# amazon-science/instruct-video-to-video

Hardware: AMD Instinct MI355X
Metric: denoised video-frames/sec (16f@256x384, 50 DDIM steps) (higher is better)
Workload: dtype fp16; 1 GPU; C2: 1 clip/step = VAE-encode + 50 DDIM steps (3-way CFG, text 7.5 / video 1.5) + VAE-decode, 16 frames @ 256x384, random-init full-width UNet+VAE; 5 independent clips in flight per GPU (stacked into every UNet launch, B = 3 x clips); frames=16, height=256, width=384, ddim_steps=50, clips_per_gpu=5, parallelism=clip-parallel x1, one all_gather, hip_graph=True, cfg_branch_streams=False, concurrent_clips=5, clip_mode=stacked, driver_mode=False, full=False

## Files before the change

### include/insv2v_hip.h

```cpp
#ifndef INSV2V_HIP_H
#define INSV2V_HIP_H

#include <stdint.h>

#ifdef __cplusplus
extern "C" {
#endif

typedef void* insv2v_stream_t;

#define INSV2V_OK 0
#define INSV2V_EINVAL (-1)
#define INSV2V_EUNSUPPORTED (-2)

#define INSV2V_ACT_NONE 0
#define INSV2V_ACT_SILU 1
#define INSV2V_ACT_GEGLU 2
#define INSV2V_ACT_QUICK_GELU 3

#define INSV2V_ACT_RELU 4
#define INSV2V_ACT_SIGMOID 5
#define INSV2V_ACT_TANH 6

#define INSV2V_MODE_LINEAR 0
#define INSV2V_MODE_CONV3X3 1

int insv2v_abi_version(void);
int insv2v_init(void);

typedef struct insv2v_gemm_desc {
    const void* a;
    const void* a2;
    const void* w;
    void* c;
    const float* bias;
    const float* row_bias;
    const void* residual;
    const float* row_stats;
    const float* col_sum;
    int64_t lda, lda2, ldw, ldc, ldr, ld_rb;
    int64_t a_bs, w_bs, c_bs, r_bs;
    void* workspace;
    int64_t workspace_bytes;
    int32_t M, N, K;
    int32_t k_split;
    int32_t rows_per_group;
    int32_t rb_mod;
    int32_t act;
    int32_t c_fp32;
    int32_t mode;
    int32_t NB, IH, IW, OH, OW, Cin;
    int32_t stride, pad_t, pad_l, upsample;
    int32_t batch;
    int32_t tile;
    int32_t split_k;
    float alpha;
    const float* gn_ab;
    int32_t gn_images_per_sample;
    int32_t gn_silu;
    float* stats_out;
    float* stats_scratch;
    int32_t stats_parts;
    float ln_eps;
    int64_t w_group_stride;
    int32_t w_group_rows;
    int32_t reserved0;
} insv2v_gemm_desc;
int insv2v_gemm(const insv2v_gemm_desc* d, insv2v_stream_t stream);
int64_t insv2v_set_operand_window(int64_t bytes);
int insv2v_gemm_stats_parts(const insv2v_gemm_desc* d);
int insv2v_conv3x3_fuses_groupnorm(const insv2v_gemm_desc* d);
#define INSV2V_PLAN_NONE 0
#define INSV2V_PLAN_TILE 1
#define INSV2V_PLAN_HALO 2
#define INSV2V_PLAN_Q8 3
#define INSV2V_PLAN_R8 4
#define INSV2V_PLAN_W4 5
typedef struct insv2v_gemm_plan_t {
    int32_t rc;
    int32_t family;
    int32_t variant;
    int32_t ring;
    int32_t tw_shift;
    int32_t cim;
    int32_t split_k;
    int32_t ln_finalize;
    int32_t splitk_reduce;
    int32_t stats_width;
    int32_t gn_fuse;
    int32_t parts;
    int32_t units_per_part;
    int32_t forced_tile;
} insv2v_gemm_plan_t;
int insv2v_gemm_plan(const insv2v_gemm_desc* d, int cus, insv2v_gemm_plan_t* out);

typedef struct insv2v_winograd_in_desc {
    const void* x;
    const void* x2;
    const float* gn_ab;
    void* v;
    int64_t ldx, ldx2;
    int64_t v_group_rows;
    int32_t NB, H, W, C, C1;
    int32_t gn_images_per_sample;
    int32_t gn_silu;
    int32_t upsample;
} insv2v_winograd_in_desc;
int insv2v_winograd_input(const insv2v_winograd_in_desc* d, insv2v_stream_t stream);
typedef struct insv2v_winograd_out_desc {
    const void* m;
    const float* bias;
    const float* row_bias;
    const void* residual;
    void* y;
    int64_t m_group_rows;
    int64_t ldr, ldy, ld_rb;
    int32_t NB, H, W, Cout;
    int32_t rows_per_group;
    int32_t upsample;
} insv2v_winograd_out_desc;
int insv2v_winograd_output(const insv2v_winograd_out_desc* d, insv2v_stream_t stream);

typedef struct insv2v_ffn_desc {
    const void* x;
    void* out;
    const void* wstream;
    int64_t ldx, ldo;
    int32_t M, C, hidden;
    float eps;
    const void* post_residual;
    int64_t ld_post;
    int32_t post;
} insv2v_ffn_desc;
int insv2v_ffn_fused(const insv2v_ffn_desc* d, insv2v_stream_t stream);
int64_t insv2v_ffn_stream_elems(int32_t C, int32_t hidden, int32_t post);

typedef struct insv2v_rowlin_desc {
    const void* x;
    void* out;
    const void* residual;
    const void* wstream;
    int64_t ldx, ldo, ldr;
    int32_t M, N, K;
    int32_t layernorm, frame_bias, rows_per_frame, frames;
    float eps;
    float* stats_out;
    float stats_eps;
    const float* gn_ab;
    int32_t gn_rows;
} insv2v_rowlin_desc;
int insv2v_rowlin(const insv2v_rowlin_desc* d, insv2v_stream_t stream);
int64_t insv2v_rowlin_stream_elems(int32_t N, int32_t K);

typedef struct insv2v_tattn_desc {
    const void* x;
    void* out;
    const void* wstream;
    int64_t ldx, ldo;
    int32_t samples, HW, C, heads, frames;
    float eps;
    float scale;
} insv2v_tattn_desc;
int insv2v_tattn_fused(const insv2v_tattn_desc* d, insv2v_stream_t stream);
int64_t insv2v_tattn_stream_elems(int32_t C, int32_t heads, int32_t frames);
int insv2v_tattn_attn(const insv2v_tattn_desc* d, insv2v_stream_t stream);
int64_t insv2v_tattn_attn_stream_elems(int32_t C, int32_t heads, int32_t frames);

typedef struct insv2v_xattn_desc {
    const void* x;
    void* out;
    const void* wstream;
    const void* kvstream;
    int64_t ldx, ldo;
    int32_t M, rows_per_sample, C, heads, ctx_len;
    float eps;
    float scale;
    const void* pre_residual;
    int64_t ld_pre;
} insv2v_xattn_desc;
int insv2v_xattn_fused(const insv2v_xattn_desc* d, insv2v_stream_t stream);
int64_t insv2v_xattn_stream_elems(int32_t C, int32_t heads, int32_t per_sample_kv);
int insv2v_xattn_attn(const insv2v_xattn_desc* d, insv2v_stream_t stream);
int64_t insv2v_xattn_attn_stream_elems(int32_t C, int32_t heads, int32_t per_sample_kv);

typedef struct insv2v_groupnorm_desc {
    const void* x;
    const void* x2;
    void* y;
    const float* gamma;
    const float* beta;
    float* partials;
    int64_t ldx, ldx2, ldy;
    int32_t nsamples, rows_per_sample, C, C1, G;
    int32_t nchunks;
    int32_t silu;
    float eps;
    float* ab;
    int32_t stats_only;
} insv2v_groupnorm_desc;
int insv2v_groupnorm(const insv2v_groupnorm_desc* d, insv2v_stream_t stream);

typedef struct insv2v_layernorm_desc {
    const void* x;
    void* y;
    const float* gamma;
    const float* beta;
    const float* pe;
    int64_t ldx, ldy;
    int32_t rows, C;
    int32_t rows_per_frame, frames, pe_start;
    float eps;
} insv2v_layernorm_desc;
int insv2v_layernorm(const insv2v_layernorm_desc* d, insv2v_stream_t stream);
int insv2v_layernorm_stats(const void* x, float* stats, int64_t ldx, int32_t rows, int32_t C, float eps,
                           insv2v_stream_t stream);

typedef struct insv2v_attention_desc {
    const void* q;
    const void* k;
    const void* v;
    void* o;
    int64_t q_rs, k_rs, v_rs, o_rs;
    int64_t q_outer, q_step, kv_outer, kv_step, o_outer, o_step;
    int32_t q_inner, kv_inner, o_inner;
    int32_t batch, heads, head_dim, seq_q, seq_k;
    float scale;
    int32_t causal;
    const void* q_bias;
    const void* k_bias;
    const void* v_bias;
    int64_t bias_rs;
} insv2v_attention_desc;
int insv2v_attention(const insv2v_attention_desc* d, insv2v_stream_t stream);

int insv2v_embed_tokens(const int64_t* ids, const void* tok, const void* pos, void* out, int32_t rows, int32_t L,
                        int32_t C, int32_t vocab, insv2v_stream_t stream);

int insv2v_softmax_rows(const void* x, void* y, int64_t ldx, int64_t ldy, int32_t rows, int32_t cols,
                        float scale, insv2v_stream_t stream);
int insv2v_softmax_rows_padded(const void* x, void* y, int64_t ldx, int64_t ldy, int32_t rows, int32_t cols, int32_t valid,
                               float scale, insv2v_stream_t stream);

int insv2v_timestep_embedding(const float* t, void* out, int32_t batch, int32_t dim, float shift,
                              insv2v_stream_t stream);

int insv2v_tap_gather(const float* y9, int64_t ld9, const float* bias, float* out, int64_t ldo, int32_t NB, int32_t H, int32_t W,
                      int32_t cout, insv2v_stream_t stream);

int insv2v_build_unet_input(const float* latent, const float* img_cond, void* out, float* t_out,
                            float timestep, int32_t nbranch, int32_t F, int32_t h, int32_t w, int32_t ldo,
                            int64_t branch_rows, int32_t t_stride, insv2v_stream_t stream);

typedef struct insv2v_step_desc {
    const float* eps_in;
    const float* latent;
    const float* latent_ref;
    const float* delta_q;
    const float* noise;
    const float* rescale_stats;
    float* latent_out;
    float* pred_x0;
    float* eps_out;
    int32_t nbranch, F, h, w, R;
    int32_t correct;
    float text_cfg, img_cfg;
    float sqrt_a, sqrt_1ma;
    float c_x0, c_eps, c_xt, c_noise;
    float guidance_rescale;
    int64_t branch_stride;
    int64_t noise_seed, noise_stream;
    int32_t noise_on;
} insv2v_step_desc;
int insv2v_cfg_step(const insv2v_step_desc* d, insv2v_stream_t stream);
typedef struct insv2v_mstep_desc {
    const float* eps_in;
    const float* latent;
    const float* latent_ref;
    const float* delta_q;
    const float* noise;
    const float* rescale_stats;
    float* latent_out;
    float* pred_x0;
    float* eps_out;
    int32_t nbranch, F, h, w, R;
    int32_t correct;
    float text_cfg, img_cfg;
    float sqrt_a, sqrt_1ma;
    float c_x0, c_eps, c_xt, c_noise;
    float guidance_rescale;
    int64_t branch_stride;
    int64_t noise_seed, noise_stream;
    int32_t noise_on;
    const float* x0_hist;
    float c_hist;
} insv2v_mstep_desc;
int insv2v_cfg_step_ms(const insv2v_mstep_desc* d, insv2v_stream_t stream);
typedef struct insv2v_maskstep_desc {
    const float* eps_in;
    const float* latent;
    const float* latent_ref;
    const float* delta_q;
    const float* noise;
    const float* rescale_stats;
    float* latent_out;
    float* pred_x0;
    float* eps_out;
    int32_t nbranch, F, h, w, R;
    int32_t correct;
    float text_cfg, img_cfg;
    float sqrt_a, sqrt_1ma;
    float c_x0, c_eps, c_xt, c_noise;
    float guidance_rescale;
    int64_t branch_stride;
    int64_t noise_seed, noise_stream;
    int32_t noise_on;
    const float* x0_hist;
    float c_hist;
    const float* mask;
    const float* src;
    const float* known_noise;
    float k_src, k_noise;
} insv2v_maskstep_desc;
int insv2v_cfg_step_mask(const insv2v_maskstep_desc* d, insv2v_stream_t stream);
int insv2v_mask_to_latent(const float* mask, float* out, int32_t N, int32_t H, int32_t W, int32_t mode, insv2v_stream_t stream);
int insv2v_composite(const float* edited, const float* original, const float* mask, float* out, int32_t N, int32_t H, int32_t W,
                     insv2v_stream_t stream);
int insv2v_add_noise(const float* z, const float* noise, float* out, int64_t n, float ka, float kb, insv2v_stream_t stream);
int insv2v_cfg_stats(const float* eps_in, float* stats, int32_t F, int32_t h, int32_t w, float text_cfg,
                     float img_cfg, int64_t branch_stride, insv2v_stream_t stream);

int insv2v_warp_image(const float* image, const float* flow, float* out, int32_t N, int32_t C, int32_t H,
                      int32_t W, insv2v_stream_t stream);
int insv2v_resize_flow(const float* flow, float* out, int32_t N, int32_t h, int32_t w, int32_t H, int32_t W,
                       insv2v_stream_t stream);
int insv2v_flow_correction(const float* eps_cfg, const float* latent, const float* latent_ref,
                           const float* flows, float* delta_q, int32_t F, int32_t R, int32_t h, int32_t w,
                           float sqrt_a, float sqrt_1ma, insv2v_stream_t stream);

int insv2v_nchw_to_nhwc_f16(const float* x, void* y, int32_t N, int32_t C, int32_t H, int32_t W, int32_t ldo,
                            float scale, insv2v_stream_t stream);
int insv2v_nhwc_to_nchw_f32(const void* x, int32_t x_is_fp32, float* y, int32_t N, int32_t C, int32_t H,
                            int32_t W, int32_t ldx, float scale, insv2v_stream_t stream);
int insv2v_posterior_sample(const float* moments, const float* noise, float* z, int32_t N, int32_t H,
                            int32_t W, int32_t ldm, float scale, insv2v_stream_t stream);
int insv2v_posterior_sample_seeded(const float* moments, float* z, int32_t N, int32_t H, int32_t W, int32_t ldm, float scale,
                                   int64_t seed, int64_t stream, int64_t offset, insv2v_stream_t hip_stream);

int insv2v_randn(float* out, int64_t n, int64_t seed, int64_t stream, int64_t offset, int32_t raw, insv2v_stream_t hip_stream);

typedef struct insv2v_im2col_desc {
    const void* x;
    const void* x2;
    void* out;
    int64_t ldx, ldx2, ldo;
    int32_t N, IH, IW, C, C1, KH, KW, stride_h, stride_w, pad_h, pad_w, OH, OW;
} insv2v_im2col_desc;
int insv2v_im2col(const insv2v_im2col_desc* d, insv2v_stream_t stream);
int insv2v_instance_norm(const void* x, void* y, float* partials, int32_t N, int32_t HW, int32_t C, int64_t ldx, int64_t ldy,
                         int32_t nchunks, float eps, int32_t relu, insv2v_stream_t stream);
#define INSV2V_EW_RELU 1
#define INSV2V_EW_ADD_RELU 2
#define INSV2V_EW_TANH 3
#define INSV2V_EW_GRU_RH 4
#define INSV2V_EW_GRU_OUT 5
int insv2v_ew(int32_t op, const void* a, const void* b, const void* c, void* out, int64_t rows, int32_t C, int64_t lda, int64_t ldb,
              int64_t ldc, int64_t ldo, insv2v_stream_t stream);
int insv2v_avgpool2x2(const float* x, float* y, int64_t n, int32_t h, int32_t w, insv2v_stream_t stream);
typedef struct insv2v_corr_lookup_desc {
    const float* pyr0;
    const float* pyr1;
    const float* pyr2;
    const float* pyr3;
    const float* coords;
    void* out;
    int64_t ldo;
    int32_t B, h, w, levels, radius;
} insv2v_corr_lookup_desc;
int insv2v_corr_lookup(const insv2v_corr_lookup_desc* d, insv2v_stream_t stream);
int insv2v_raft_flow_rows(float* coords1, const float* delta, int64_t ldd, void* rows, int64_t ldf, int32_t ncols, int32_t B, int32_t h,
                          int32_t w, insv2v_stream_t stream);
int insv2v_convex_upsample(const float* coords1, const void* mask, int64_t ldm, float* out, int32_t B, int32_t h, int32_t w,
                           insv2v_stream_t stream);

#ifdef __cplusplus
}
#endif
#endif
```

### instruct-video-to-video_amd/csrc/gemm.hip

```cpp
#include "common.h"
#include <algorithm>
#include "gemm_dma.h"
#include "gemm_plan.h"
static_assert(GEMM_BK == BK, "gemm_plan.h restates the K slice");
#include <type_traits>
#include <cstdlib>

typedef unsigned uint4r __attribute__((ext_vector_type(4)));

struct RowInfo {
    int base;
    int oh, ow;
    bool valid;
};

#ifdef INSV2V_GEMM_PROF
__device__ unsigned long long g_prof[8];
#define PROF_MARK(i) do { if (tid == 0) prof_t[i] = wall_clock64(); } while (0)
#else
#define PROF_MARK(i) do { } while (0)
#endif

template <int W>
__device__ __forceinline__ float lane_group_sum(float v) {
    static_assert(W == 4 || W == 8 || W == 16, "a DPP row is 16 lanes");
    auto dpp = [](float x, auto ctrl) {
        return __builtin_bit_cast(float, __builtin_amdgcn_update_dpp(0, __builtin_bit_cast(int, x), decltype(ctrl)::value, 0xF, 0xF, true));
    };
    v += dpp(v, std::integral_constant<int, 0xB1>{});
    v += dpp(v, std::integral_constant<int, 0x4E>{});
    if (W >= 8) v += dpp(v, std::integral_constant<int, 0x141>{});
    if (W >= 16) v += dpp(v, std::integral_constant<int, 0x140>{});
    return v;
}

__device__ __forceinline__ bool fast_output_ok(const insv2v_gemm_desc& p, const char* Cb, const half_t* Rp, int oN) {
    const bool vec_ok = ((p.ldc & 7) == 0) && (((uintptr_t)Cb & (p.c_fp32 ? 31 : 15)) == 0) &&
                        (!Rp || (((p.ldr & 7) == 0) && (((uintptr_t)Rp & 15) == 0)));
    const bool res32 = !Rp || (int64_t)p.M * p.ldr * 2 < ((int64_t)1 << 31);
    return vec_ok && !p.c_fp32 && (oN & 7) == 0 && res32;
}

template <int WM, int WN, int MI, int NI, int KG, bool HAS_LN, class RowMap>
__device__ __forceinline__ void tile_epilogue(const insv2v_gemm_desc& p, floatx16 (&acc)[NI][MI], char* smem, const float* sBias,
                                              const float* sCs, const float2* sStat, int tid, int wm, int wn, int kg, int bn0,
                                              int z, int zs, bool rows_full, RowMap grow
#ifdef INSV2V_GEMM_PROF
                                              , unsigned long long* prof_t
#endif
) {
    constexpr int NWV = WM * WN * KG, NT = NWV * 64;
    constexpr int BM = WM * MI * 32, BN = WN * NI * 32;
    const int lane = tid & 63;
    const bool geglu = p.act == INSV2V_ACT_GEGLU;
    const int oN = geglu ? (p.N >> 1) : p.N;
    const int on0 = geglu ? (bn0 >> 1) : bn0;
    constexpr int CLD = BN + 4;
    float* sC = (float*)smem;
    char* Cb = (char*)p.c + ((int64_t)z * p.c_bs + (int64_t)zs * p.M * p.ldc) * (p.c_fp32 ? 4 : 2);
    const half_t* Rp = p.residual ? (const half_t*)p.residual + z * p.r_bs : nullptr;
    if (KG > 1) {
        for (int g = 1; g < KG; ++g) {
            if (kg == g) {
#pragma unroll
                for (int j = 0; j < MI; ++j)
#pragma unroll
                    for (int i = 0; i < NI; ++i)
#pragma unroll
                        for (int q = 0; q < 4; ++q)
                            *(float4*)(sC + (wm * MI * 32 + j * 32 + (lane & 31)) * CLD + wn * NI * 32 + i * 32 + 8 * q + 4 * (lane >> 5)) =
                                make_float4(acc[i][j][4 * q], acc[i][j][4 * q + 1], acc[i][j][4 * q + 2], acc[i][j][4 * q + 3]);
            }
            __syncthreads();
            if (kg == 0) {
#pragma unroll
                for (int j = 0; j < MI; ++j)
#pragma unroll
                    for (int i = 0; i < NI; ++i)
#pragma unroll
                        for (int q = 0; q < 4; ++q) {
                            const float4 t = *(const float4*)(sC + (wm * MI * 32 + j * 32 + (lane & 31)) * CLD + wn * NI * 32 + i * 32 + 8 * q + 4 * (lane >> 5));
                            acc[i][j][4 * q] += t.x; acc[i][j][4 * q + 1] += t.y; acc[i][j][4 * q + 2] += t.z; acc[i][j][4 * q + 3] += t.w;
                        }
            }
            if (g + 1 < KG) __syncthreads();
        }
    }
    typedef unsigned uint4e __attribute__((ext_vector_type(4)));
    const srd_t rRB = make_srd(p.row_bias ? (const void*)p.row_bias : (const void*)p.w);
    const bool rb_vec = p.row_bias && (p.N & 3) == 0 && (p.ld_rb & 3) == 0 && (((uintptr_t)p.row_bias & 15) == 0);
    if (KG == 1 || kg == 0) {
#pragma unroll
    for (int j = 0; j < MI; ++j) {
        const int ml = wm * MI * 32 + j * 32 + (lane & 31);
        const int m = grow(ml);
        const float* rb = nullptr;
        unsigned rb_off = OOB_OFFSET;
        if (p.row_bias && m < p.M) {
            int grp = m / p.rows_per_group;
            if (p.rb_mod > 0) grp %= p.rb_mod;
            rb = p.row_bias + (int64_t)grp * p.ld_rb;
            rb_off = (unsigned)(grp * (int)p.ld_rb * 4);
        }
        floatx4 rbv[NI][4];
        if (rb_vec) {
#pragma unroll
            for (int i = 0; i < NI; ++i)
#pragma unroll
                for (int q = 0; q < 4; ++q) {
                    const int n = bn0 + wn * NI * 32 + i * 32 + 8 * q + 4 * (lane >> 5);
                    rbv[i][q] = __builtin_bit_cast(floatx4, (uint4e)__builtin_amdgcn_raw_buffer_load_b128(rRB, (rb && n + 3 < p.N) ? rb_off + (unsigned)(n * 4) : OOB_OFFSET, 0, 0));
                }
        }
        float ln_m = 0.f, ln_r = 1.f;
        if (HAS_LN) { const float2 st = sStat[ml]; ln_m = st.x; ln_r = st.y; }
#pragma unroll
        for (int i = 0; i < NI; ++i) {
            if (geglu && (i & 1)) continue;
#pragma unroll
            for (int q = 0; q < 4; ++q) {
                const int nl = wn * NI * 32 + i * 32 + 8 * q + 4 * (lane >> 5);
                const int n = bn0 + nl;
                float v[4];
                const float4 bt = *(const float4*)(sBias + nl), ct = HAS_LN ? *(const float4*)(sCs + nl) : make_float4(0.f, 0.f, 0.f, 0.f);
                float bsum[4] = {bt.x, bt.y, bt.z, bt.w};
                const float cs[4] = {ct.x, ct.y, ct.z, ct.w};
                if (rb_vec) {
                    const floatx4 t = rbv[i][q];
                    bsum[0] += t[0]; bsum[1] += t[1]; bsum[2] += t[2]; bsum[3] += t[3];
                } else if (rb) {
#pragma unroll
                    for (int e = 0; e < 4; ++e)
                        if (n + e < p.N) bsum[e] += rb[n + e];
                }
#pragma unroll
                for (int e = 0; e < 4; ++e) v[e] = ln_r * (acc[i][j][4 * q + e] * p.alpha - ln_m * cs[e]) + bsum[e];
                int onl = nl;
                if (geglu) {
                    const float4 gbt = *(const float4*)(sBias + nl + 32), gct = HAS_LN ? *(const float4*)(sCs + nl + 32) : make_float4(0.f, 0.f, 0.f, 0.f);
                    float gb[4] = {gbt.x, gbt.y, gbt.z, gbt.w};
                    const float gcs[4] = {gct.x, gct.y, gct.z, gct.w};
                    if (rb_vec) {
                        const floatx4 t = rbv[(i + 1) % NI][q];
                        gb[0] += t[0]; gb[1] += t[1]; gb[2] += t[2]; gb[3] += t[3];
                    } else if (rb && n + 35 < p.N) {
                        const float4 t = *(const float4*)(rb + n + 32);
                        gb[0] += t.x; gb[1] += t.y; gb[2] += t.z; gb[3] += t.w;
                    }
#pragma unroll
                    for (int e = 0; e < 4; ++e)
                        v[e] *= gelu_erf_f(ln_r * (acc[(i + 1) % NI][j][4 * q + e] * p.alpha - ln_m * gcs[e]) + gb[e]);
                    onl = (nl >> 6) * 32 + (nl & 31);
                } else if (p.act == INSV2V_ACT_SILU) {
#pragma unroll
                    for (int e = 0; e < 4; ++e) v[e] = silu_f(v[e]);
                } else if (p.act == INSV2V_ACT_QUICK_GELU) {
#pragma unroll
                    for (int e = 0; e < 4; ++e) v[e] = quick_gelu_f(v[e]);
                } else if (p.act >= INSV2V_ACT_RELU) {
#pragma unroll
                    for (int e = 0; e < 4; ++e) v[e] = act_raft_f(v[e], p.act);
                }
                *(float4*)(sC + ml * CLD + onl) = make_float4(v[0], v[1], v[2], v[3]);
            }
        }
    }
    }
    PROF_MARK(3);
    __syncthreads();
    PROF_MARK(4);
    const int OW8 = (geglu ? BN / 2 : BN) / 8;
    const bool vec_ok = ((p.ldc & 7) == 0) && (((uintptr_t)Cb & (p.c_fp32 ? 31 : 15)) == 0) &&
                        (!Rp || (((p.ldr & 7) == 0) && (((uintptr_t)Rp & 15) == 0)));
    if (fast_output_ok(p, Cb, Rp, oN)) {
        const srd_t rRes = make_srd(Rp ? (const void*)Rp : (const void*)p.w);
        auto copy_rows = [&](auto w8_tag) {
            constexpr int W8 = decltype(w8_tag)::value;
            constexpr int ITERS = (BM * W8) / NT;
            static_assert((BM * W8) % NT == 0, "staged tile must divide evenly over the workgroup");
            half8 rv[ITERS];
            bool ok[ITERS];
            int mrow[ITERS];
#pragma unroll
            for (int it = 0; it < ITERS; ++it) {
                const int idx = tid + it * NT, row = idx / W8, ch = idx % W8;
                mrow[it] = grow(row);
                ok[it] = (rows_full || mrow[it] < p.M) && on0 + ch * 8 + 8 <= oN;
                if (Rp) rv[it] = __builtin_bit_cast(half8, (uint4e)__builtin_amdgcn_raw_buffer_load_b128(
                            rRes, ok[it] ? (unsigned)((mrow[it] * (int)p.ldr + on0 + ch * 8) * 2) : OOB_OFFSET, 0, 0));
            }
#pragma unroll
            for (int it = 0; it < ITERS; ++it) {
                const int idx = tid + it * NT, row = idx / W8, ch = idx % W8;
                const float4 f0 = *(const float4*)(sC + row * CLD + ch * 8);
                const float4 f1 = *(const float4*)(sC + row * CLD + ch * 8 + 4);
                const float fv[8] = {f0.x, f0.y, f0.z, f0.w, f1.x, f1.y, f1.z, f1.w};
                half8 hv;
#pragma unroll
                for (int e = 0; e < 8; ++e) hv[e] = (half_t)(Rp ? fv[e] + (float)rv[it][e] : fv[e]);
                if (ok[it]) *(half8*)((half_t*)Cb + (int64_t)mrow[it] * p.ldc + on0 + ch * 8) = hv;
                if constexpr (W8 == 4 || W8 == 8 || W8 == 16) {
                    if (p.stats_out) {
                        float s1 = 0.f, s2 = 0.f;
#pragma unroll
                        for (int e = 0; e < 8; ++e) { const float x = ok[it] ? (float)hv[e] : 0.f; s1 += x; s2 = fmaf(x, x, s2); }
                        s1 = lane_group_sum<W8>(s1);
                        s2 = lane_group_sum<W8>(s2);
                        if (ch == 0 && (rows_full || mrow[it] < p.M))
                            *(float2*)(p.stats_out + ((int64_t)(bn0 / BN) * p.M + mrow[it]) * 2) = make_float2(s1, s2);
                    }
                }
            }
        };
        if (geglu) copy_rows(std::integral_constant<int, BN / 16>{});
        else copy_rows(std::integral_constant<int, BN / 8>{});
#ifdef INSV2V_GEMM_PROF
        wait_vmcnt<0>();
        PROF_MARK(5);
        if (tid == 0) {
            for (int i = 0; i < 5; ++i) atomicAdd(&g_prof[i], prof_t[i + 1] - prof_t[i]);
            atomicAdd(&g_prof[5], 1ull);
        }
#endif
        return;
    }
    for (int idx = tid; idx < BM * OW8; idx += NT) {
        const int row = idx / OW8, ch = idx - row * OW8;
        const int m = grow(row), on = on0 + ch * 8;
        if (m >= p.M || on >= oN) continue;
        const float4 f0 = *(const float4*)(sC + row * CLD + ch * 8);
        const float4 f1 = *(const float4*)(sC + row * CLD + ch * 8 + 4);
        float fv[8] = {f0.x, f0.y, f0.z, f0.w, f1.x, f1.y, f1.z, f1.w};
        if (p.c_fp32) {
            float* dst32 = (float*)Cb + (int64_t)m * p.ldc + on;
            if (Rp) {
#pragma unroll
                for (int e = 0; e < 8; ++e)
                    if (on + e < oN) fv[e] += (float)Rp[(int64_t)m * p.ldr + on + e];
            }
            if (vec_ok && on + 7 < oN) {
                *(float4*)dst32 = make_float4(fv[0], fv[1], fv[2], fv[3]);
                *(float4*)(dst32 + 4) = make_float4(fv[4], fv[5], fv[6], fv[7]);
            } else {
#pragma unroll
                for (int e = 0; e < 8; ++e)
                    if (on + e < oN) dst32[e] = fv[e];
            }
            continue;
        }
        half_t* dst = (half_t*)Cb + (int64_t)m * p.ldc + on;
        if (vec_ok && on + 7 < oN) {
            half8 hv;
            if (Rp) {
                const half8 rv = *(const half8*)(Rp + (int64_t)m * p.ldr + on);
#pragma unroll
                for (int e = 0; e < 8; ++e) hv[e] = (half_t)(fv[e] + (float)rv[e]);
            } else {
#pragma unroll
                for (int e = 0; e < 8; ++e) hv[e] = (half_t)fv[e];
            }
            *(half8*)dst = hv;
        } else {
#pragma unroll
            for (int e = 0; e < 8; ++e)
                if (on + e < oN) dst[e] = (half_t)(fv[e] + (Rp ? (float)Rp[(int64_t)m * p.ldr + on + e] : 0.f));
        }
    }
}

template <int WM, int WN, int MI, int NI, int MODE, int STAGES, int KG = 1>
__global__ __launch_bounds__(WM * WN * KG * 64) void gemm_kernel(insv2v_gemm_desc p) {
    constexpr int NWV = WM * WN * KG;
    constexpr int BM = WM * MI * 32, BN = WN * NI * 32;
    constexpr int LD = BK;
    constexpr int RPP = 8 * NWV;
    constexpr int RA = BM / RPP, RW = BN / RPP;
    extern __shared__ __attribute__((aligned(16))) char smem[];
    half_t* sA = (half_t*)smem;
    half_t* sW = sA + STAGES * BM * LD;
    constexpr int RING_B = STAGES * (BM + BN) * BK * 2, STAGE_B = BM * (BN + 4) * 4;
    float* sBias = (float*)(smem + (RING_B > STAGE_B ? RING_B : STAGE_B));
    float* sCs = sBias + BN;
    float2* sStat = (float2*)(sCs + BN);

    const int tid = threadIdx.x, lane = tid & 63;
#ifdef INSV2V_GEMM_PROF
    unsigned long long prof_t[6];
#endif
    PROF_MARK(0);
    const int wid = __builtin_amdgcn_readfirstlane(tid >> 6);
    const int kg = wid / (WM * WN), wl = wid % (WM * WN);
    const int wm = wl / WN, wn = wl % WN;
    const int tiles_n = (p.N + BN - 1) / BN, tiles_m = (p.M + BM - 1) / BM;
    const int bid = xcd_remap(blockIdx.x, tiles_m * tiles_n);
    constexpr int GROUP_M = 8;
    const int per_group = GROUP_M * tiles_n;
    const int gidx = bid / per_group, first_m = gidx * GROUP_M;
    const int gsz = min(GROUP_M, tiles_m - first_m), rin = bid - gidx * per_group;
    const int tn = rin / gsz, tm = first_m + rin - tn * gsz;
    const int bm0 = tm * BM, bn0 = tn * BN;
    const int z = blockIdx.y;

    const half_t* A = (const half_t*)p.a + z * p.a_bs;
    const half_t* A2 = p.a2 ? (const half_t*)p.a2 + z * p.a_bs : A;
    const half_t* Wp = (const half_t*)p.w + z * p.w_bs;
    const srd_t rA = make_srd(A), rA2 = make_srd(A2), rW = make_srd(Wp);

    const int crow = wid * 8 + (lane >> 3);
    const int cslot = lane & 7;

    RowInfo ri[RA];
    int achunk[RA];
    unsigned aoff1[RA], aoff2[RA];
#pragma unroll
    for (int i = 0; i < RA; ++i) {
        const int row = crow + RPP * i;
        achunk[i] = cslot ^ ((row >> 1) & 7);
        const int m = bm0 + row;
        ri[i].valid = m < p.M;
        if (MODE == INSV2V_MODE_LINEAR) {
            ri[i].base = m;
            ri[i].oh = ri[i].ow = 0;
            aoff1[i] = ri[i].valid ? (unsigned)(((int64_t)m * p.lda + achunk[i] * 8) * 2) : OOB_OFFSET;
            aoff2[i] = ri[i].valid ? (unsigned)(((int64_t)m * p.lda2 + achunk[i] * 8) * 2) : OOB_OFFSET;
        } else {
            int mm = ri[i].valid ? m : 0;
            int ow = mm % p.OW, t = mm / p.OW;
            int oh = t % p.OH, nb = t / p.OH;
            ri[i].base = nb * p.IH * p.IW;
            ri[i].oh = oh * p.stride - p.pad_t;
            ri[i].ow = ow * p.stride - p.pad_l;
            const int64_t pix = (int64_t)ri[i].base + (int64_t)ri[i].oh * p.IW + ri[i].ow;
            aoff1[i] = (unsigned)((pix * p.lda + achunk[i] * 8) * 2);
            aoff2[i] = (unsigned)((pix * p.lda2 + achunk[i] * 8) * 2);
        }
    }
    int wchunk[RW];
    unsigned woff[RW];
#pragma unroll
    for (int i = 0; i < RW; ++i) {
        const int row = crow + RPP * i;
        wchunk[i] = cslot ^ ((row >> 1) & 7);
        const int n = bn0 + row;
        woff[i] = n < p.N ? (unsigned)(((int64_t)n * p.ldw + wchunk[i] * 8) * 2) : OOB_OFFSET;
    }

    const int nk_total = (p.K + BK - 1) / BK;
    const int zs = blockIdx.z, nsplit = p.split_k > 1 ? p.split_k : 1;

    const int nk_per = (nk_total + nsplit - 1) / nsplit;
    const int kt0 = zs * nk_per;
    const int nk = max(0, min(nk_per, nk_total - kt0));
    const int IHu = p.upsample ? p.OH : p.IH, IWu = p.upsample ? p.OW : p.IW;

    struct Cursor {
        int k0, kh, kw, ci0;
    } cur_k = {kt0 * BK, 0, 0, 0};
    if (MODE != INSV2V_MODE_LINEAR) {
        const int tap = cur_k.k0 / p.Cin;
        cur_k.ci0 = cur_k.k0 - tap * p.Cin;
        cur_k.kh = tap / 3;
        cur_k.kw = tap - cur_k.kh * 3;
    }
    auto advance = [&]() {
        cur_k.k0 += BK;
        if (MODE != INSV2V_MODE_LINEAR) {
            cur_k.ci0 += BK;
            if (cur_k.ci0 >= p.Cin) {
                cur_k.ci0 = 0;
                if (++cur_k.kw == 3) { cur_k.kw = 0; ++cur_k.kh; }
            }
        }
    };
    auto issue_slice = [&](int buf) {
        char* a = (char*)(sA + buf * BM * LD) + wid * 1024;
        char* w = (char*)(sW + buf * BN * LD) + wid * 1024;
        const bool ktail = cur_k.k0 + BK > p.K;
        if (MODE == INSV2V_MODE_LINEAR) {
            const bool second = p.k_split > 0 && cur_k.k0 >= p.k_split;
            const int soff = (second ? cur_k.k0 - p.k_split : cur_k.k0) * 2;
#pragma unroll
            for (int i = 0; i < RA; ++i) {
                unsigned v = second ? aoff2[i] : aoff1[i];
                if (ktail && cur_k.k0 + achunk[i] * 8 >= p.K) v = OOB_OFFSET;
                dma16(second ? rA2 : rA, v, soff, a + i * (NWV * 1024));
            }
        } else {
            const bool second = p.k_split > 0 && cur_k.ci0 >= p.k_split;
            const int ld = (int)(second ? p.lda2 : p.lda);
            const int cl = second ? cur_k.ci0 - p.k_split : cur_k.ci0;
            const int tapoff = ((cur_k.kh * p.IW + cur_k.kw) * ld + cl) * 2;
#pragma unroll
            for (int i = 0; i < RA; ++i) {
                const int ih = ri[i].oh + cur_k.kh, iw = ri[i].ow + cur_k.kw;
                const bool ok = ri[i].valid && (unsigned)ih < (unsigned)IHu && (unsigned)iw < (unsigned)IWu;
                unsigned v;
                if (p.upsample)
                    v = (unsigned)((((ri[i].base + (ih >> 1) * p.IW + (iw >> 1)) * ld) + cl + achunk[i] * 8) * 2);
                else
                    v = (second ? aoff2[i] : aoff1[i]) + (unsigned)tapoff;
                dma16(second ? rA2 : rA, ok ? v : OOB_OFFSET, 0, a + i * (NWV * 1024));
            }
        }
        const int wsoff = cur_k.k0 * 2;
#pragma unroll
        for (int i = 0; i < RW; ++i) {
            unsigned v = woff[i];
            if (ktail && cur_k.k0 + wchunk[i] * 8 >= p.K) v = OOB_OFFSET;
            dma16(rW, v, wsoff, w + i * (NWV * 1024));
        }
        advance();
    };

    floatx16 acc[NI][MI];
#pragma unroll
    for (int i = 0; i < NI; ++i)
#pragma unroll
        for (int j = 0; j < MI; ++j)
#pragma unroll
            for (int r = 0; r < 16; ++r) acc[i][j][r] = 0.f;

    const int frow = lane & 31, fhalf = lane >> 5;
    auto compute = [&](int buf) {
        const half_t* a = sA + buf * BM * LD + (wm * MI * 32 + frow) * LD;
        const half_t* w = sW + buf * BN * LD + (wn * NI * 32 + frow) * LD;
        const int sw = (frow >> 1) & 7;
#pragma unroll
        for (int kq = 0; kq < BK / 16 / KG; ++kq) {
            const int kk = kg * (BK / 16 / KG) + kq;
            const int c = ((kk * 2 + fhalf) ^ sw) * 8;
            half8 fa[MI], fw[NI];
#pragma unroll
            for (int j = 0; j < MI; ++j) fa[j] = *(const half8*)(a + j * 32 * LD + c);
#pragma unroll
            for (int i = 0; i < NI; ++i) fw[i] = *(const half8*)(w + i * 32 * LD + c);
#pragma unroll
            for (int i = 0; i < NI; ++i)
#pragma unroll
                for (int j = 0; j < MI; ++j)
                    acc[i][j] = __builtin_amdgcn_mfma_f32_32x32x16_f16(fw[i], fa[j], acc[i][j], 0, 0, 0);
        }
    };

    const bool ln = p.row_stats != nullptr;
    float pre_b = 0.f, pre_c = 0.f;
    float2 pre_s = make_float2(0.f, 1.f);
    if (tid < BN && bn0 + tid < p.N) {
        if (p.bias) pre_b = p.bias[bn0 + tid];
        if (ln) pre_c = p.col_sum[bn0 + tid];
    }
    if (tid < BM && ln && bm0 + tid < p.M) {
        if (p.stats_parts > 0) {
            float s1 = 0.f, s2 = 0.f;
            for (int j = 0; j < p.stats_parts; ++j) {
                const float2 t = ((const float2*)p.row_stats)[(int64_t)j * p.M + bm0 + tid];
                s1 += t.x; s2 += t.y;
            }
            const float mean = s1 / p.K;
            pre_s = make_float2(mean, rsqrtf(fmaxf(s2 / p.K - mean * mean, 0.f) + p.ln_eps));
        } else {
            pre_s = ((const float2*)p.row_stats)[bm0 + tid];
        }
    }

    constexpr int LPT = RA + RW;
#pragma unroll
    for (int s = 0; s < STAGES; ++s)
        if (s < nk) issue_slice(s);
    if (tid < BN) { sBias[tid] = pre_b; sCs[tid] = pre_c; }
    if (tid < BM) sStat[tid] = pre_s;
    int cur = 0, nxt = STAGES - 1;
    for (int kt = 0; kt < nk; ++kt) {
        const int behind = kt == 0 ? min(STAGES - 1, nk - 1) : min(STAGES - 2, nk - 1 - kt);
        if (behind <= 0) wait_vmcnt<0>();
        else if (behind == 1) wait_vmcnt<LPT>();
        else if (behind == 2) wait_vmcnt<2 * LPT>();
        else wait_vmcnt<3 * LPT>();
        __builtin_amdgcn_s_barrier();
        asm volatile("" ::: "memory");
#ifdef INSV2V_GEMM_PROF
        if (kt == 0) PROF_MARK(1);
#endif
        if (kt > 0 && kt + STAGES - 1 < nk) issue_slice(nxt);
        compute(cur);
        cur = (cur + 1 == STAGES) ? 0 : cur + 1;
        nxt = (nxt + 1 == STAGES) ? 0 : nxt + 1;
    }
    wait_vmcnt<0>();
    __syncthreads();
    PROF_MARK(2);

    tile_epilogue<WM, WN, MI, NI, KG, true>(p, acc, smem, sBias, sCs, sStat, tid, wm, wn, kg, bn0, z, zs, bm0 + BM <= p.M,
                                            [&](int r) { return bm0 + r; }
#ifdef INSV2V_GEMM_PROF
                                            , prof_t
#endif
    );
}


template <int WM, int WN, int MI, int NI, int KG, bool GN, int WS = 2>
__global__ __launch_bounds__(WM * WN * KG * 64) void conv_halo_kernel(insv2v_gemm_desc p, int tw_shift) {
    constexpr int NWV = WM * WN * KG;
    constexpr int BM = WM * MI * 32, BN = WN * NI * 32;
    static_assert(BM == 128 || BM == 256, "the pixel patch is 128 (8x16 / 16x8) or 256 (16x16 / 32x8) output pixels");
    static_assert(WS == 2 || (WS == 3 && !GN && KG == 1), "the deep weight ring has no fused-GroupNorm / K-group form");
    constexpr int LD = BK;
    constexpr int RPP = 8 * NWV, RW = BN / RPP;
    constexpr int HPIECES = BM == 128 ? 23 : 43;
    constexpr int HP = (HPIECES + NWV - 1) / NWV;
    constexpr int HALO_B = HPIECES * 1024;
    constexpr int KQ = BK / 16 / KG;
    extern __shared__ __attribute__((aligned(16))) char smem[];
    char* sH = smem;
    half_t* sW = (half_t*)(smem + 2 * HALO_B);
    constexpr int RING_B = 2 * HALO_B + WS * BN * BK * 2, STAGE_B = BM * (BN + 4) * 4;
    float* sBias = (float*)(smem + (RING_B > STAGE_B ? RING_B : STAGE_B));
    constexpr int AB_OFF = (RING_B > STAGE_B ? RING_B : STAGE_B) + BN * 4;

    const int tid = threadIdx.x, lane = tid & 63;
#ifdef INSV2V_GEMM_PROF
    unsigned long long prof_t[6];
#endif
    PROF_MARK(0);
    const int wid = __builtin_amdgcn_readfirstlane(tid >> 6);
    const int kg = wid / (WM * WN), wl = wid % (WM * WN);
    const bool legacy_map = (tw_shift >> 8) & 1;
    tw_shift &= 255;
    const int wm = legacy_map ? wl / WN : wl % WM, wn = legacy_map ? wl % WN : wl / WM;
    const int TW = 1 << tw_shift, TH = BM >> tw_shift;
    const int tiles_x = p.OW >> tw_shift, tiles_y = p.OH / TH, tiles_img = tiles_x * tiles_y;
    const int tiles_n = (p.N + BN - 1) / BN, tiles_m = p.NB * tiles_img;
    const int bid = xcd_remap(blockIdx.x, tiles_m * tiles_n);
    constexpr int GROUP_M = 8;
    const int per_group = GROUP_M * tiles_n;
    const int gidx = bid / per_group, first_m = gidx * GROUP_M;
    const int gsz = min(GROUP_M, tiles_m - first_m), rin = bid - gidx * per_group;
    const int tn = rin / gsz, tm = first_m + rin - tn * gsz;
    const int bn0 = tn * BN;
    const int nb = tm / tiles_img, trem = tm - nb * tiles_img;
    const int ty = trem / tiles_x, tx = trem - ty * tiles_x;
    const int oy0 = ty * TH, ox0 = tx * TW;
    const int up = p.upsample ? 1 : 0;
    const int sy0 = (oy0 - 1) >> up, sx0 = (ox0 - 1) >> up;
    const int PH = (TH >> up) + 2, PW = (TW >> up) + 2, HROWS = PH * PW;

    const half_t* A = (const half_t*)p.a;
    const half_t* A2 = p.a2 ? (const half_t*)p.a2 : A;
    const srd_t rA = make_srd(A), rA2 = make_srd(A2), rW = make_srd(p.w);

    auto patch_key = [&](int hy, int hx) { return ((hx >> 1) + (tw_shift == 3 ? ((hy & 1) << 2) : 0)) & 7; };
    unsigned hoff1[HP], hoff2[HP];
    int hchunk[HP];
#pragma unroll
    for (int i = 0; i < HP; ++i) {
        const int r = (i * NWV + wid) * 8 + (lane >> 3);
        const int hy = r / PW, hx = r - hy * PW;
        const int chunk = (lane & 7) ^ patch_key(hy, hx);
        const int iy = sy0 + hy, ix = sx0 + hx;
        const bool ok = r < HROWS && (unsigned)iy < (unsigned)p.IH && (unsigned)ix < (unsigned)p.IW;
        const int64_t pix = ((int64_t)nb * p.IH + iy) * p.IW + ix;
        hoff1[i] = ok ? (unsigned)((pix * p.lda + chunk * 8) * 2) : OOB_OFFSET;
        hoff2[i] = ok ? (unsigned)((pix * p.lda2 + chunk * 8) * 2) : OOB_OFFSET;
        hchunk[i] = ok ? chunk : -1;
    }
    const int crow = wid * 8 + (lane >> 3), cslot = lane & 7;
    unsigned woff[RW];
#pragma unroll
    for (int i = 0; i < RW; ++i) {
        const int row = crow + RPP * i;
        const int n = bn0 + row;
        woff[i] = n < p.N ? (unsigned)(((int64_t)n * p.ldw + (cslot ^ ((row >> 1) & 7)) * 8) * 2) : OOB_OFFSET;
    }
    const int ncb = p.Cin / BK, nk = ncb * 9;

    auto issue_halo = [&](int i, int cb) {
        const int q = i * NWV + wid;
        if (q >= HPIECES) return;
        const int ci0 = cb * BK;
        const bool second = p.k_split > 0 && ci0 >= p.k_split;
        dma16(second ? rA2 : rA, second ? hoff2[i] : hoff1[i], (second ? ci0 - p.k_split : ci0) * 2, sH + (cb & 1) * HALO_B + q * 1024);
    };
    const unsigned lds0 = (unsigned)(uintptr_t)(__attribute__((address_space(3))) char*)smem;
    const srd_t rAB = make_srd(GN ? (const void*)p.gn_ab : p.w);
    const int gn_sample = GN ? nb / p.gn_images_per_sample : 0;
    auto issue_ab = [&](int cb) {
        if (GN && wid == 0 && lane < 32)
            dma16(rAB, (unsigned)((((int64_t)gn_sample * p.Cin + cb * BK) * 2 + lane * 4) * 4), 0, smem + AB_OFF + (cb & 1) * 512);
    };
    auto normalize = [&](int i, int cb) {
        const int q = i * NWV + wid;
        if (!GN || q >= HPIECES) return;
        const unsigned addr = lds0 + (cb & 1) * HALO_B + q * 1024 + lane * 16;
        const unsigned abaddr = lds0 + AB_OFF + (cb & 1) * 512 + (hchunk[i] < 0 ? 0 : hchunk[i]) * 64;
        uint4r v;
        floatx4 c0, c1, c2, c3;
        asm volatile("ds_read_b128 %0, %5\n\tds_read_b128 %1, %6\n\tds_read_b128 %2, %6 offset:16\n\t"
                     "ds_read_b128 %3, %6 offset:32\n\tds_read_b128 %4, %6 offset:48\n\ts_waitcnt lgkmcnt(0)"
                     : "=&v"(v), "=&v"(c0), "=&v"(c1), "=&v"(c2), "=&v"(c3) : "v"(addr), "v"(abaddr) : "memory");
        const half8 x = __builtin_bit_cast(half8, v);
        const float sc[8] = {c0[0], c0[2], c1[0], c1[2], c2[0], c2[2], c3[0], c3[2]};
        const float sh[8] = {c0[1], c0[3], c1[1], c1[3], c2[1], c2[3], c3[1], c3[3]};
        half8 y;
#pragma unroll
        for (int e = 0; e < 8; ++e) {
            float t = fmaf((float)x[e], sc[e], sh[e]);
            if (p.gn_silu) t = silu_f(t);
            y[e] = hchunk[i] < 0 ? (half_t)0.f : (half_t)t;
        }
        const uint4r o = __builtin_bit_cast(uint4r, y);
        asm volatile("ds_write_b128 %0, %1\n\ts_waitcnt lgkmcnt(0)" ::"v"(addr), "v"(o) : "memory");
    };
    auto issue_w = [&](int buf, int cb, int tap) {
        char* w = (char*)(sW + buf * BN * LD) + wid * 1024;
        const int soff = (tap * p.Cin + cb * BK) * 2;
#pragma unroll
        for (int i = 0; i < RW; ++i) dma16(rW, woff[i], soff, w + i * (NWV * 1024));
    };

    floatx16 acc[NI][MI];
#pragma unroll
    for (int i = 0; i < NI; ++i)
#pragma unroll
        for (int j = 0; j < MI; ++j)
#pragma unroll
            for (int r = 0; r < 16; ++r) acc[i][j][r] = 0.f;

    const int frow = lane & 31, fhalf = lane >> 5;
    int fpy[MI], fpx[MI];
#pragma unroll
    for (int j = 0; j < MI; ++j) {
        const int ml = wm * MI * 32 + j * 32 + frow;
        fpy[j] = ml >> tw_shift;
        fpx[j] = ml & (TW - 1);
    }
    const int wsw = (frow >> 1) & 7;
    const bool wave_live = legacy_map || bn0 + wn * NI * 32 < p.N;
    auto compute = [&](int wbuf, int cb, int kh, int kw) {
        if (!wave_live) return;
        const half_t* hb = (const half_t*)(sH + (cb & 1) * HALO_B);
        const half_t* w = sW + wbuf * BN * LD + (wn * NI * 32 + frow) * LD;
        int arow[MI], akey[MI];
#pragma unroll
        for (int j = 0; j < MI; ++j) {
            const int uy = oy0 + fpy[j] + kh - 1, ux = ox0 + fpx[j] + kw - 1;
            const int hy = (uy >> up) - sy0, hx = (ux >> up) - sx0;
            arow[j] = hy * PW + hx;
            akey[j] = patch_key(hy, hx);
        }
#pragma unroll
        for (int kq = 0; kq < KQ; ++kq) {
            const int kk = kg * KQ + kq;
            const int cl = kk * 2 + fhalf;
            half8 fa[MI], fw[NI];
#pragma unroll
            for (int j = 0; j < MI; ++j) fa[j] = *(const half8*)(hb + arow[j] * LD + ((cl ^ akey[j]) * 8));
#pragma unroll
            for (int i = 0; i < NI; ++i) fw[i] = *(const half8*)(w + i * 32 * LD + ((cl ^ wsw) * 8));
#pragma unroll
            for (int i = 0; i < NI; ++i)
#pragma unroll
                for (int j = 0; j < MI; ++j)
                    acc[i][j] = __builtin_amdgcn_mfma_f32_32x32x16_f16(fw[i], fa[j], acc[i][j], 0, 0, 0);
        }
    };

    float pre_b = 0.f;
    if (tid < BN && bn0 + tid < p.N && p.bias) pre_b = p.bias[bn0 + tid];
    issue_ab(0);
#pragma unroll
    for (int i = 0; i < HP; ++i) issue_halo(i, 0);
    issue_w(0, 0, 0);
    int cbn = 0, tapn = 1;
    if (WS == 3) {
        if (tapn == 9) { tapn = 0; ++cbn; }
        if (nk > 1) issue_w(1, cbn, tapn);
        if (++tapn == 9) { tapn = 0; ++cbn; }
    }
    if (tid < BN) sBias[tid] = pre_b;
    if (GN) {
        wait_vmcnt<0>();
        __builtin_amdgcn_s_barrier();
#pragma unroll
        for (int i = 0; i < HP; ++i) normalize(i, 0);
    }
    int cb = 0, kh = 0, kw = 0, tap = 0;
    int wslot = 0, islot = 2;
    for (int s = 0; s < nk; ++s) {
        if (WS == 3 && s + 1 < nk) wait_vmcnt<RW>();
        else wait_vmcnt<0>();
        __builtin_amdgcn_s_barrier();
        asm volatile("" ::: "memory");
#ifdef INSV2V_GEMM_PROF
        if (s == 0) PROF_MARK(1);
#endif
        if (GN && cb + 1 < ncb) {
#pragma unroll
            for (int i = 0; i < HP; ++i)
                if (tap == i + 1) normalize(i, cb + 1);
        }
        if (WS == 2 && s + 1 < nk) {
            const bool wrap = tap == 8;
            issue_w((s + 1) & 1, wrap ? cb + 1 : cb, wrap ? 0 : tap + 1);
        }
        if (tap == 0 && cb + 1 < ncb) issue_ab(cb + 1);
        if (cb + 1 < ncb) {
#pragma unroll
            for (int i = 0; i < HP; ++i)
                if (tap == i) issue_halo(i, cb + 1);
        }
        if (WS == 3) {
            if (s + 2 < nk) {
                issue_w(islot, cbn, tapn);
                if (++tapn == 9) { tapn = 0; ++cbn; }
            }
            islot = islot == 2 ? 0 : islot + 1;
        }
        compute(WS == 3 ? wslot : (s & 1), cb, kh, kw);
        if (WS == 3) wslot = wslot == 2 ? 0 : wslot + 1;
        if (++kw == 3) { kw = 0; ++kh; }
        if (++tap == 9) { tap = 0; kh = 0; ++cb; }
    }
    wait_vmcnt<0>();
    __syncthreads();
    PROF_MARK(2);
    tile_epilogue<WM, WN, MI, NI, KG, false>(p, acc, smem, sBias, nullptr, nullptr, tid, wm, wn, kg, bn0, 0, 0, true,
                                             [&](int r) { return (nb * p.OH + oy0 + (r >> tw_shift)) * p.OW + ox0 + (r & (TW - 1)); }
#ifdef INSV2V_GEMM_PROF
                                             , prof_t
#endif
    );
}

template <int WM, int WN, int MI, int NI, int KG, bool GN = false, int WS = 2>
static int launch_halo(const insv2v_gemm_desc& d, int tw_shift, hipStream_t s) {
    constexpr int BM = WM * MI * 32, BN = WN * NI * 32;
    constexpr size_t ring = 2 * (BM == 128 ? 23 : 43) * 1024 + WS * (size_t)BN * BK * sizeof(half_t);
    constexpr size_t stage = (size_t)BM * (BN + 4) * sizeof(float);
    constexpr size_t lds = (ring > stage ? ring : stage) + (size_t)BN * sizeof(float) + (GN ? 1024 : 0);
    static bool attr_set = false;
    if (const int e = set_dynamic_lds(attr_set, (const void*)conv_halo_kernel<WM, WN, MI, NI, KG, GN, WS>, lds)) return e;
    const int tiles = d.NB * (d.OH * d.OW / BM) * ((d.N + BN - 1) / BN);
    hipLaunchKernelGGL((conv_halo_kernel<WM, WN, MI, NI, KG, GN, WS>), dim3(tiles), dim3(WM * WN * KG * 64), lds, s, d, tw_shift);
    return launch_status();
}

template <int WM, int WN, int MI, int NI, int MODE, int STAGES, int KG = 1>
static int launch_cfg(const insv2v_gemm_desc& d, hipStream_t s) {
    constexpr int BM = WM * MI * 32, BN = WN * NI * 32;
    constexpr size_t lds = tile_lds_bytes(BM, BN, STAGES);
    if (lds > TILE_LDS_MAX) return INSV2V_EUNSUPPORTED;
    static bool attr_set = false;
    if (const int e = set_dynamic_lds(attr_set, (const void*)gemm_kernel<WM, WN, MI, NI, MODE, STAGES, KG>, lds)) return e;
    int tiles = ((d.M + BM - 1) / BM) * ((d.N + BN - 1) / BN);
    dim3 grid(tiles, d.batch > 0 ? d.batch : 1, d.split_k > 1 ? d.split_k : 1);
    hipLaunchKernelGGL((gemm_kernel<WM, WN, MI, NI, MODE, STAGES, KG>), grid, dim3(WM * WN * KG * 64), lds, s, d);
    return launch_status();
}

template <int MODE, int STAGES>
static int dispatch_tile(const insv2v_gemm_desc& d, int tile, hipStream_t s) {
    switch (tile) {
        case 1: return launch_cfg<2, 2, 2, 2, MODE, STAGES>(d, s);
        case 2: return launch_cfg<2, 2, 1, 2, MODE, STAGES>(d, s);
        case 3: return launch_cfg<2, 2, 2, 1, MODE, STAGES>(d, s);
        case 4: return launch_cfg<2, 2, 1, 1, MODE, STAGES>(d, s);
        case 5: return launch_cfg<4, 2, 1, 2, MODE, STAGES>(d, s);
        case 6: return launch_cfg<4, 2, 2, 2, MODE, STAGES>(d, s);
        case 7: return launch_cfg<4, 2, 1, 1, MODE, STAGES>(d, s);
        case 8: return launch_cfg<2, 2, 2, 2, MODE, STAGES, 2>(d, s);
        case 9: return launch_cfg<2, 2, 2, 1, MODE, STAGES, 2>(d, s);
    }
    return INSV2V_EINVAL;
}

__global__ __launch_bounds__(256) void splitk_reduce_kernel(insv2v_gemm_desc p, const float* ws, int nsplit) {
    const int64_t nchunk = (int64_t)p.M * (p.N / 8);
    const int64_t idx = (int64_t)blockIdx.x * 256 + threadIdx.x;
    if (idx >= nchunk) return;
    const int m = (int)(idx / (p.N / 8)), n = (int)(idx - (int64_t)m * (p.N / 8)) * 8;
    float v[8] = {0.f, 0.f, 0.f, 0.f, 0.f, 0.f, 0.f, 0.f};
    const float* src = ws + (int64_t)m * p.N + n;
    const int64_t slab = (int64_t)p.M * p.N;
    const bool res_vec = p.residual && (p.ldr & 7) == 0 && (((uintptr_t)p.residual & 15) == 0);
    half8 rh = {0, 0, 0, 0, 0, 0, 0, 0};
    if (res_vec) rh = *(const half8*)((const half_t*)p.residual + (int64_t)m * p.ldr + n);
    float4 b0 = make_float4(0.f, 0.f, 0.f, 0.f), b1 = b0, r0 = b0, r1 = b0;
    if (p.bias) {
        if (((uintptr_t)p.bias & 15) == 0) { b0 = *(const float4*)(p.bias + n); b1 = *(const float4*)(p.bias + n + 4); }
        else { b0 = make_float4(p.bias[n], p.bias[n + 1], p.bias[n + 2], p.bias[n + 3]); b1 = make_float4(p.bias[n + 4], p.bias[n + 5], p.bias[n + 6], p.bias[n + 7]); }
    }
    if (p.row_bias) {
        const float* rb = p.row_bias + (int64_t)(m / p.rows_per_group) * p.ld_rb + n;
        if ((p.ld_rb & 3) == 0 && (((uintptr_t)p.row_bias & 15) == 0)) { r0 = *(const float4*)rb; r1 = *(const float4*)(rb + 4); }
        else { r0 = make_float4(rb[0], rb[1], rb[2], rb[3]); r1 = make_float4(rb[4], rb[5], rb[6], rb[7]); }
    }
    int s = 0;
    for (; s + 4 <= nsplit; s += 4) {
        float4 a[4], b[4];
#pragma unroll
        for (int u = 0; u < 4; ++u) { a[u] = *(const float4*)(src + (s + u) * slab); b[u] = *(const float4*)(src + (s + u) * slab + 4); }
#pragma unroll
        for (int u = 0; u < 4; ++u) {
            v[0] += a[u].x; v[1] += a[u].y; v[2] += a[u].z; v[3] += a[u].w; v[4] += b[u].x; v[5] += b[u].y; v[6] += b[u].z; v[7] += b[u].w;
        }
    }
    for (; s < nsplit; ++s) {
        const float4 a = *(const float4*)(src + s * slab), b = *(const float4*)(src + s * slab + 4);
        v[0] += a.x; v[1] += a.y; v[2] += a.z; v[3] += a.w; v[4] += b.x; v[5] += b.y; v[6] += b.z; v[7] += b.w;
    }
    const float bb[8] = {b0.x, b0.y, b0.z, b0.w, b1.x, b1.y, b1.z, b1.w}, rr[8] = {r0.x, r0.y, r0.z, r0.w, r1.x, r1.y, r1.z, r1.w};
#pragma unroll
    for (int e = 0; e < 8; ++e) {
        float x = v[e] * p.alpha;
        if (p.bias) x += bb[e];
        if (p.row_bias) x += rr[e];
        if (p.act == INSV2V_ACT_SILU) x = silu_f(x);
        else if (p.act == INSV2V_ACT_QUICK_GELU) x = quick_gelu_f(x);
        else if (p.act >= INSV2V_ACT_RELU) x = act_raft_f(x, p.act);
        if (p.residual) x += res_vec ? (float)rh[e] : (float)((const half_t*)p.residual)[(int64_t)m * p.ldr + n + e];
        v[e] = x;
    }
    if (p.c_fp32) {
        float* dst = (float*)p.c + (int64_t)m * p.ldc + n;
#pragma unroll
        for (int e = 0; e < 8; ++e) dst[e] = v[e];
    } else {
        half_t* dst = (half_t*)p.c + (int64_t)m * p.ldc + n;
        if ((p.ldc & 7) == 0 && (((uintptr_t)p.c & 15) == 0)) {
            half8 h;
#pragma unroll
            for (int e = 0; e < 8; ++e) h[e] = (half_t)v[e];
            *(half8*)dst = h;
        } else {
#pragma unroll
            for (int e = 0; e < 8; ++e) dst[e] = (half_t)v[e];
        }
    }
}

__global__ __launch_bounds__(256) void ln_finalize_kernel(const float2* parts, float2* stats, int M, int nparts, int C, float eps) {
    const int m = blockIdx.x * 256 + threadIdx.x;
    if (m >= M) return;
    float s1 = 0.f, s2 = 0.f;
    for (int j = 0; j < nparts; ++j) { const float2 t = parts[(int64_t)j * M + m]; s1 += t.x; s2 += t.y; }
    const float mean = s1 / C;
    stats[m] = make_float2(mean, rsqrtf(fmaxf(s2 / C - mean * mean, 0.f) + eps));
}

const gemm_switches& insv2v_gemm_switches() {
    static const gemm_switches sw = [] {
        auto env = [](const char* name, int dflt) { const char* v = getenv(name); return v ? atoi(v) : dflt; };
        gemm_switches s;
        s.r8 = env("INSV2V_GEMM_R8", s.r8); s.r8_stats = env("INSV2V_R8_STATS", s.r8_stats); s.q8_min_n = env("INSV2V_Q8_MIN_N", s.q8_min_n); s.persistent = env("INSV2V_GEMM_PERSISTENT", s.persistent);
        s.r8_geglu = env("INSV2V_R8_GEGLU", s.r8_geglu); s.r8_cim = env("INSV2V_R8_CIM", s.r8_cim); s.halo_legacy_map = env("INSV2V_HALO_LEGACY_MAP", s.halo_legacy_map);
        s.r8_dephase = env("INSV2V_R8_DEPHASE", s.r8_dephase); s.w4_wgs = env("INSV2V_W4_WGS", s.w4_wgs); s.w4_delay = env("INSV2V_W4_DELAY", s.w4_delay);
        return s;
    }();
    return sw;
}

static int64_t g_operand_window = 0;
extern "C" int64_t insv2v_set_operand_window(int64_t bytes) {
    const int64_t prev = g_operand_window;
    g_operand_window = bytes > 0 ? bytes : 0;
    return prev;
}
static int64_t operand_window() { return g_operand_window > 0 ? g_operand_window : ((int64_t)1 << 31) - ((int64_t)1 << 20); }
int64_t insv2v_operand_window_override() { return g_operand_window; }

static insv2v_gemm_plan_t plan_here(const insv2v_gemm_desc& d, int cus = 0, bool queries_only = false) {
    return plan_gemm(d, cus > 0 ? cus : insv2v_num_cus(), operand_window(), insv2v_gemm_switches(), queries_only);
}
extern "C" int insv2v_gemm_plan(const insv2v_gemm_desc* dp, int cus, insv2v_gemm_plan_t* out) {
    if (!dp || !out) return INSV2V_EINVAL;
    *out = plan_here(*dp, cus);
    return 0;
}
extern "C" int insv2v_gemm_stats_parts(const insv2v_gemm_desc* dp) {
    const int w = dp ? plan_here(*dp, 0, true).stats_width : 0;
    return w ? (dp->N + w - 1) / w : 0;
}
extern "C" int insv2v_conv3x3_fuses_groupnorm(const insv2v_gemm_desc* dp) { return dp ? plan_here(*dp, 0, true).gn_fuse : 0; }

static void finish_stats(insv2v_gemm_desc& d, hipStream_t s) {
    hipLaunchKernelGGL(ln_finalize_kernel, dim3((d.M + 255) / 256), dim3(256), 0, s, (const float2*)d.row_stats, (float2*)d.stats_scratch, d.M,
                       d.stats_parts, d.K, d.ln_eps);
    stats_finished(d);
}

static int execute(insv2v_gemm_desc d, const insv2v_gemm_plan_t& p, hipStream_t s) {
    if (p.ln_finalize) finish_stats(d, s);
    const insv2v_gemm_desc full = d;
    if (p.split_k > 1) splitk_main_pass(d, p.split_k);
    else d.split_k = 1;
    const bool conv = d.mode == INSV2V_MODE_CONV3X3;
    int rc = INSV2V_EINVAL;
    switch (p.family) {
        case INSV2V_PLAN_Q8: return insv2v_gemm_q8(d, p.variant, s);
        case INSV2V_PLAN_R8: return insv2v_gemm_r8(d, p.variant, s);
        case INSV2V_PLAN_W4: return insv2v_gemm_w4(d, p.variant, s);
        case INSV2V_PLAN_HALO:
            switch (p.variant) {
                case 0: return d.gn_ab ? launch_halo<4, 2, 1, 2, 1, true>(d, p.tw_shift, s) : launch_halo<4, 2, 1, 2, 1>(d, p.tw_shift, s);
                case 3: return launch_halo<8, 2, 1, 2, 1, false, 3>(d, p.tw_shift, s);
                case 2: return launch_halo<2, 2, 2, 2, 1>(d, p.tw_shift, s);
                case 1: return launch_halo<2, 2, 2, 2, 2>(d, p.tw_shift, s);
            }
            return rc;
        case INSV2V_PLAN_TILE:
            switch (p.ring) {
                case 2: rc = conv ? dispatch_tile<INSV2V_MODE_CONV3X3, 2>(d, p.variant, s) : dispatch_tile<INSV2V_MODE_LINEAR, 2>(d, p.variant, s); break;
                case 3: rc = conv ? dispatch_tile<INSV2V_MODE_CONV3X3, 3>(d, p.variant, s) : dispatch_tile<INSV2V_MODE_LINEAR, 3>(d, p.variant, s); break;
                case 4: rc = conv ? dispatch_tile<INSV2V_MODE_CONV3X3, 4>(d, p.variant, s) : dispatch_tile<INSV2V_MODE_LINEAR, 4>(d, p.variant, s); break;
            }
            if (rc != 0 || !p.splitk_reduce) return rc;
            hipLaunchKernelGGL(splitk_reduce_kernel, dim3((unsigned)(((int64_t)full.M * (full.N / 8) + 255) / 256)), dim3(256), 0, s, full, (const float*)full.workspace, p.split_k);
            return launch_status();
    }
    return rc;
}

static int run(const insv2v_gemm_desc& d, hipStream_t s);
static int run_parts(insv2v_gemm_desc f, const insv2v_gemm_plan_t& p, hipStream_t s) {
    if (p.ln_finalize) finish_stats(f, s);
    const int64_t total = f.mode == INSV2V_MODE_CONV3X3 ? f.NB : f.M, per = p.units_per_part;
    for (int64_t u0 = 0; u0 < total; u0 += per)
        if (const int rc = run(window_part(f, u0, std::min(per, total - u0)), s)) return rc;
    return 0;
}
static int run(const insv2v_gemm_desc& d, hipStream_t s) {
    const insv2v_gemm_plan_t p = plan_here(d);
    return p.rc ? p.rc : p.parts > 1 ? run_parts(d, p, s) : execute(d, p, s);
}

extern "C" int insv2v_gemm(const insv2v_gemm_desc* dp, insv2v_stream_t stream) {
    if (!one_device() || !dp) return INSV2V_EINVAL;
    insv2v_gemm_desc d = *dp;
    gemm_defaults(d);
    return run(d, as_stream(stream));
}

#ifdef INSV2V_GEMM_PROF
extern "C" int insv2v_prof_read(unsigned long long* out, int reset) {
    hipError_t e = hipMemcpyFromSymbol(out, HIP_SYMBOL(g_prof), sizeof(unsigned long long) * 8);
    if (e == hipSuccess && reset) {
        unsigned long long z[8] = {0, 0, 0, 0, 0, 0, 0, 0};
        e = hipMemcpyToSymbol(HIP_SYMBOL(g_prof), z, sizeof(z));
    }
    return (int)e;
}
#endif
```

### instruct-video-to-video_amd/csrc/gemm_plan.h

```cpp
#pragma once
#include <stdint.h>
#include <algorithm>
#include "../../include/insv2v_hip.h"

constexpr int GEMM_BK = 64;
constexpr int W4_BK = 32;

struct gemm_switches {
    int r8 = 1;
    int r8_stats = 1;
    int q8_min_n = 256;
    int persistent = 1;
    int r8_geglu = 1;
    int r8_cim = 1;
    int halo_legacy_map = 0;
    int r8_dephase = 0;
    int w4_wgs = 2, w4_delay = -1;
};
const gemm_switches& insv2v_gemm_switches();

static inline void gemm_defaults(insv2v_gemm_desc& d) { if (d.batch <= 0) d.batch = 1; if (d.alpha == 0.f) d.alpha = 1.f; }
static inline bool misaligned16(const void* p) { return ((uintptr_t)p & 15) != 0; }
static inline bool beyond_2g(int64_t bytes) { return bytes >= ((int64_t)1 << 31); }

static inline bool row_bias_fits_tiles(const insv2v_gemm_desc& d, int bm) { return !d.row_bias || !((d.ld_rb & 3) || (d.rows_per_group % bm && d.M > d.rows_per_group)); }
static inline bool engine_operands_ok(const insv2v_gemm_desc& d, int bk) {
    if (d.batch > 1 || d.c_fp32 || d.split_k > 1) return false;
    if ((d.K % bk) || (d.N & 7) || (d.ldc & 7) || misaligned16(d.c)) return false;
    if (d.residual && ((d.ldr & 7) || misaligned16(d.residual))) return false;
    if (d.k_split && (d.k_split % bk)) return false;
    if (d.act != INSV2V_ACT_NONE && d.act != INSV2V_ACT_GEGLU) return false;
    if (d.row_stats && (d.M & 1)) return false;
    if (beyond_2g((int64_t)d.M * d.ldc * 2) || (d.residual && beyond_2g((int64_t)d.M * d.ldr * 2))) return false;
    if (d.act == INSV2V_ACT_GEGLU && ((d.N % 64) || d.mode == INSV2V_MODE_CONV3X3 || d.residual)) return false;
    return !(d.mode == INSV2V_MODE_CONV3X3 && (d.Cin % bk));
}
static inline int q8_refusal(const insv2v_gemm_desc& d, int variant) {
    const bool conv = d.mode == INSV2V_MODE_CONV3X3, gg = d.act == INSV2V_ACT_GEGLU, res = d.residual != nullptr;
    if (!engine_operands_ok(d, GEMM_BK) || !row_bias_fits_tiles(d, 256)) return INSV2V_EUNSUPPORTED;
    if (variant < 0 || variant > 5) return INSV2V_EINVAL;
    return (variant == 3 ? conv : variant >= 2 && (conv || gg || res)) ? INSV2V_EUNSUPPORTED : 0;
}
static inline int r8_refusal(const insv2v_gemm_desc& d, int variant) {
    const bool conv = d.mode == INSV2V_MODE_CONV3X3, gg = d.act == INSV2V_ACT_GEGLU;
    if (!engine_operands_ok(d, GEMM_BK) || !row_bias_fits_tiles(d, 256)) return INSV2V_EUNSUPPORTED;
    if ((gg || d.stats_out) && (conv || (d.N % 320) || d.k_split > 0 || variant != 0 || (gg && d.stats_out))) return INSV2V_EUNSUPPORTED;
    if ((d.bias && misaligned16(d.bias)) || (d.col_sum && misaligned16(d.col_sum)) || (d.row_bias && misaligned16(d.row_bias))) return INSV2V_EUNSUPPORTED;
    if (conv && d.M >= (1 << 24)) return INSV2V_EUNSUPPORTED;
    return (variant == 0 || variant == 2 || variant == 4 || variant == 5) ? 0 : INSV2V_EINVAL;
}
static inline bool r8_uses_cim(const insv2v_gemm_desc& d, int variant, const gemm_switches& sw) {
    return d.mode == INSV2V_MODE_CONV3X3 && sw.r8_cim && !d.stats_out && (variant == 0 || variant == 4) && d.stride == 1 && !d.upsample && d.pad_t == 1 &&
           d.pad_l == 1 && d.IH == d.OH && d.IW == d.OW;
}
static inline int w4_refusal(const insv2v_gemm_desc& d, int variant) {
    const int v = variant % 10;
    if (!engine_operands_ok(d, W4_BK) || d.K < 2 * W4_BK) return INSV2V_EUNSUPPORTED;
    if (v >= 2 && d.act == INSV2V_ACT_GEGLU) return INSV2V_EUNSUPPORTED;
    if (!row_bias_fits_tiles(d, (v == 1 || v == 3) ? 256 : 128)) return INSV2V_EUNSUPPORTED;
    if (v < 0 || v > 3) return INSV2V_EINVAL;
    return (variant / 10 == 1 && d.mode == INSV2V_MODE_CONV3X3) ? INSV2V_EUNSUPPORTED : 0;
}

static inline int tile_bm(int shape) { return shape == 6 ? 256 : (shape == 2 || shape == 4) ? 64 : 128; }
static inline int tile_bn(int shape) { return (shape == 3 || shape == 4 || shape == 7 || shape == 9) ? 64 : 128; }
constexpr size_t tile_lds_bytes(int bm, int bn, int stages) {
    const size_t ring = (size_t)stages * (bm + bn) * GEMM_BK * 2, stage = (size_t)bm * (bn + 4) * sizeof(float);
    return (ring > stage ? ring : stage) + (size_t)(2 * bn + 2 * bm) * sizeof(float);
}
constexpr size_t TILE_LDS_MAX = 160 * 1024;
static inline int pick_tile(const insv2v_gemm_desc& d) {
    const long batch = d.batch > 0 ? d.batch : 1;
    auto blocks = [&](int bm, int bn) { return (long)((d.M + bm - 1) / bm) * ((d.N + bn - 1) / bn) * batch; };
    const long b11 = blocks(128, 128);
    if (d.act == INSV2V_ACT_GEGLU) return b11 >= 200 ? 5 : 2;
    if (d.mode == INSV2V_MODE_CONV3X3) return (b11 >= 200 && d.N >= 128) ? 5 : 4;
    return blocks(128, 64) >= 200 ? 5 : 4;
}

struct pingpong_cost { double q8, r8; };
static inline pingpong_cost pingpong_costs(const insv2v_gemm_desc& d, int cus) {
    const long tm = (d.M + 255) / 256;
    auto rounds = [&](int bn) { return (double)((tm * ((d.N + bn - 1) / bn) + cus - 1) / cus) * bn; };
    return {rounds(256) * 1.03, rounds(320)};
}
static inline int pingpong_choice(const insv2v_gemm_desc& d, bool stats, int cus, const gemm_switches& sw) {
    if (!sw.r8 || d.act != INSV2V_ACT_NONE || d.batch > 1 || d.c_fp32 || d.M < 8192 || d.N < 256) return 0;
    if (stats && (!sw.r8_stats || d.mode != INSV2V_MODE_LINEAR || d.k_split || (d.N % 320))) return 0;
    if (d.mode == INSV2V_MODE_LINEAR && d.K < 256) return 0;
    if (!row_bias_fits_tiles(d, 256) || cus <= 0) return 0;
    const double old_cost = (double)((d.M + 255) / 256) * d.N / cus / 0.80;
    const pingpong_cost c = pingpong_costs(d, cus);
    if (d.N % 320 == 0 && (c.r8 <= c.q8 || stats) && c.r8 < old_cost) return 2;
    if (d.N % 256 == 0 && d.N >= sw.q8_min_n && (d.N % 320 != 0 || c.q8 < c.r8) && c.q8 < old_cost && d.K >= 1152 && !stats) return 1;
    return 0;
}
static inline int persistent_choice(const insv2v_gemm_desc& d, const gemm_switches& sw) {
    if (!sw.persistent || d.mode != INSV2V_MODE_LINEAR || d.batch > 1 || d.c_fp32 || d.k_split) return 0;
    if (!row_bias_fits_tiles(d, 256)) return 0;
    if (d.act == INSV2V_ACT_NONE && d.K >= 1280 && d.N >= 640 && (int64_t)d.M * d.N >= (int64_t)20 << 20) return 1;
    if (d.residual) return 0;
    if (d.act == INSV2V_ACT_GEGLU) return d.K <= 320 ? (d.M >= 8192 ? 2 : 0) : (d.M >= 1024 ? 1 : 0);
    if (d.act != INSV2V_ACT_NONE || d.N < 960 || d.K > 640 || d.M < 4096) return 0;
    return (d.M < 12288 && d.K == 640) ? 1 : 2;
}
static inline int split_choice(const insv2v_gemm_desc& d) {
    if (d.split_k == 1 || !d.workspace || d.batch > 1 || d.act == INSV2V_ACT_GEGLU || (d.N & 7) || d.row_stats || d.rb_mod > 0) return 1;
    const long b11 = (long)((d.M + 127) / 128) * ((d.N + 127) / 128);
    const int nk = (d.K + GEMM_BK - 1) / GEMM_BK;
    int s = d.split_k;
    if (s == 0) {
        if (b11 >= 200 || nk < 64) return 1;
        s = std::min({(int)(512 / b11), nk / 16, 8});
    }
    if (s < 2) return 1;
    if ((int64_t)s * d.M * d.N * 4 > d.workspace_bytes) return 1;
    return s;
}
static inline void splitk_main_pass(insv2v_gemm_desc& d, int nsplit) {
    d.c = d.workspace; d.ldc = d.N; d.c_fp32 = 1; d.c_bs = 0;
    d.bias = nullptr; d.row_bias = nullptr; d.residual = nullptr; d.act = INSV2V_ACT_NONE; d.alpha = 1.f;
    d.row_stats = nullptr; d.col_sum = nullptr; d.split_k = nsplit;
}
static inline int halo_tw_shift(const insv2v_gemm_desc& d) {
    if (d.mode != INSV2V_MODE_CONV3X3 || d.stride != 1 || d.pad_t != 1 || d.pad_l != 1 || (d.Cin % GEMM_BK) || d.batch > 1) return -1;
    if (d.k_split > 0 && (d.k_split % GEMM_BK)) return -1;
    if (d.row_stats || d.rb_mod > 0 || d.act == INSV2V_ACT_GEGLU) return -1;
    const int up = d.upsample ? 2 : 1;
    if (d.OH != d.IH * up || d.OW != d.IW * up) return -1;
    if (d.OH % 8 == 0 && d.OW % 16 == 0) return 4;
    if (d.OH % 16 == 0 && d.OW % 8 == 0) return 3;
    return -1;
}
static inline bool halo_fills_chip(const insv2v_gemm_desc& d) { return ((long)d.M / 128) * ((d.N + 127) / 128) >= 200; }

static inline int stats_width_of(const insv2v_gemm_desc& d, int cus, const gemm_switches& sw) {
    if (d.mode != INSV2V_MODE_LINEAR || d.c_fp32 || d.act == INSV2V_ACT_GEGLU || d.batch > 1 || (d.N & 7) || (d.ldc & 7) || misaligned16(d.c) ||
        (d.residual && ((d.ldr & 7) || misaligned16(d.residual) || beyond_2g((int64_t)d.M * d.ldr * 2))))
        return 0;
    if (d.tile >= 240 && d.tile <= 249) return (d.N % 320 || d.k_split) ? 0 : 160;
    if (d.tile >= 100) return 0;
    if (d.tile == 0 && pingpong_choice(d, true, cus, sw) == 2) return 160;
    const int shape = d.tile % 10 ? d.tile % 10 : pick_tile(d);
    return shape >= 1 && shape <= 9 ? tile_bn(shape) : 0;
}

static inline bool beyond_window(const insv2v_gemm_desc& d, int64_t window) {
    const int64_t a_rows = d.mode == INSV2V_MODE_CONV3X3 ? (int64_t)d.NB * d.IH * d.IW : (int64_t)d.M, esz = d.c_fp32 ? 4 : 2;
    const int64_t big_in = std::max(a_rows * d.lda * 2, d.k_split ? a_rows * d.lda2 * 2 : (int64_t)0);
    const int64_t big_out = std::max((int64_t)d.M * d.ldc * esz, d.residual ? (int64_t)d.M * d.ldr * 2 : (int64_t)0);
    return big_in >= window || big_out >= window;
}
static inline int64_t units_per_part(const insv2v_gemm_desc& d, int64_t window) {
    const bool conv = d.mode == INSV2V_MODE_CONV3X3;
    auto lcm = [](int64_t a, int64_t b) { int64_t x = a, y = b; while (y) { const int64_t t = x % y; x = y; y = t; } return a / x * b; };
    const int64_t opix = conv ? (int64_t)d.OH * d.OW : 1, ipix = conv ? (int64_t)d.IH * d.IW : 1;
    int64_t unit = conv ? 1 : 2;
    if (d.row_bias) {
        const int64_t grp = (int64_t)d.rows_per_group * (d.rb_mod > 0 ? d.rb_mod : 1);
        if (conv && grp % opix) return 0;
        unit = lcm(unit, conv ? grp / opix : grp);
    }
    if (conv && d.gn_ab) unit = lcm(unit, d.gn_images_per_sample);
    if (!conv && unit < 256) unit = lcm(unit, 256);
    if (d.w_group_rows > 0) unit = lcm(unit, d.w_group_rows);
    const int64_t total = conv ? d.NB : d.M, esz = d.c_fp32 ? 4 : 2;
    const int64_t in_row = std::max((int64_t)d.lda * 2, d.k_split ? (int64_t)d.lda2 * 2 : (int64_t)0) * ipix;
    const int64_t out_row = std::max((int64_t)d.ldc * esz, d.residual ? (int64_t)d.ldr * 2 : (int64_t)0) * opix;
    const int64_t per = (window - 1) / std::max(in_row, out_row) / unit * unit;
    if (per <= 0) return 0;
    const int64_t nparts = (total + per - 1) / per;
    return ((total + nparts - 1) / nparts + unit - 1) / unit * unit;
}

static inline insv2v_gemm_desc window_part(const insv2v_gemm_desc& f, int64_t u0, int64_t nu) {
    const bool conv = f.mode == INSV2V_MODE_CONV3X3;
    const int64_t opix = conv ? (int64_t)f.OH * f.OW : 1, ipix = conv ? (int64_t)f.IH * f.IW : 1, esz = f.c_fp32 ? 4 : 2;
    const int64_t r_in = u0 * ipix, r_out = u0 * opix;
    insv2v_gemm_desc d = f;
    d.a = (const char*)f.a + r_in * f.lda * 2;
    if (f.k_split) d.a2 = (const char*)f.a2 + r_in * f.lda2 * 2;
    d.c = (char*)f.c + r_out * f.ldc * esz;
    if (f.residual) d.residual = (const char*)f.residual + r_out * f.ldr * 2;
    if (f.row_stats) d.row_stats = f.row_stats + r_out * 2;
    if (f.w_group_rows > 0) d.w = (const char*)f.w + (r_out / f.w_group_rows) * f.w_group_stride * 2;
    if (f.row_bias && f.rb_mod <= 0) d.row_bias = f.row_bias + (r_out / f.rows_per_group) * f.ld_rb;
    if (conv && f.gn_ab) d.gn_ab = f.gn_ab + (u0 / f.gn_images_per_sample) * (int64_t)f.Cin * 2;
    d.M = (int32_t)(nu * opix); if (conv) d.NB = (int32_t)nu;
    return d;
}
static inline void stats_finished(insv2v_gemm_desc& d) { d.row_stats = d.stats_scratch; d.stats_parts = 0; }

static inline int validate_gemm(const insv2v_gemm_desc& d, int stats_width) {
    if (!d.a || !d.w || !d.c || d.M <= 0 || d.N <= 0 || d.K <= 0) return INSV2V_EINVAL;
    if ((d.K & 7) || (d.lda & 7) || (d.ldw & 7)) return INSV2V_EINVAL;
    if (misaligned16(d.a) || misaligned16(d.w)) return INSV2V_EINVAL;
    if (d.k_split && (!d.a2 || (d.k_split % GEMM_BK) || (d.lda2 & 7) || misaligned16(d.a2))) return INSV2V_EINVAL;
    if (d.row_bias && d.rows_per_group <= 0) return INSV2V_EINVAL;
    if (d.row_stats && (!d.col_sum || d.batch > 1)) return INSV2V_EINVAL;
    if (d.stats_parts < 0 || (d.stats_parts > 0 && (!d.row_stats || !d.stats_scratch))) return INSV2V_EINVAL;
    if (d.stats_out && stats_width == 0) return INSV2V_EUNSUPPORTED;
    if (d.act == INSV2V_ACT_GEGLU && (d.N % 64)) return INSV2V_EINVAL;
    if (d.act < 0 || d.act > INSV2V_ACT_TANH) return INSV2V_EINVAL;
    if (d.w_group_rows < 0 || (d.w_group_rows > 0 && (d.w_group_rows % 256 || d.w_group_stride <= 0))) return INSV2V_EINVAL;
    if (d.w_group_rows > 0 && (d.mode != INSV2V_MODE_LINEAR || d.batch > 1 || d.c_fp32 || d.act != INSV2V_ACT_NONE || d.residual || d.row_bias || d.row_stats ||
                               d.stats_out || d.k_split || d.split_k > 1 || d.K < 256 || (d.N % 256 && d.N % 320)))
        return INSV2V_EUNSUPPORTED;
    if (d.gn_ab && (d.mode != INSV2V_MODE_CONV3X3 || d.gn_images_per_sample <= 0 || d.upsample)) return INSV2V_EINVAL;
    if (d.mode == INSV2V_MODE_CONV3X3) {
        if (d.Cin <= 0 || (d.Cin % GEMM_BK) || d.K != 9 * d.Cin) return INSV2V_EINVAL;
        if ((long)d.NB * d.OH * d.OW != d.M || d.stride < 1) return INSV2V_EINVAL;
        if (d.upsample && (d.stride != 1 || d.pad_t != 1 || d.pad_l != 1 || (d.OH != 2 * d.IH && d.OH != 2 * d.IH - 1) || (d.OW != 2 * d.IW && d.OW != 2 * d.IW - 1)))
            return INSV2V_EINVAL;
    } else if (d.mode != INSV2V_MODE_LINEAR) {
        return INSV2V_EUNSUPPORTED;
    }
    return beyond_2g((int64_t)d.N * d.ldw * 2) ? INSV2V_EUNSUPPORTED : 0;
}

static inline int engine_tile_code(int family) { return family == INSV2V_PLAN_R8 ? 240 : family == INSV2V_PLAN_Q8 ? 230 : 210; }
static inline insv2v_gemm_plan_t plan_gemm(insv2v_gemm_desc d, int cus, int64_t window, const gemm_switches& sw, bool queries_only = false) {
    insv2v_gemm_plan_t p = {};
    p.split_k = p.parts = 1;
    gemm_defaults(d);
    const bool conv = d.mode == INSV2V_MODE_CONV3X3, split = beyond_window(d, window);
    const int stats_w = stats_width_of(d, cus, sw);
    p.stats_width = split ? 0 : stats_w;
    p.gn_fuse = d.M > 0 && d.N > 0 && conv && !d.upsample && d.split_k <= 1 && (d.tile == 0 || d.tile == 100) && halo_tw_shift(d) >= 0 &&
                (d.tile == 100 || (split_choice(d) <= 1 && halo_fills_chip(d)));
    if (queries_only) return p;
    auto refuse = [&](int rc) { p.rc = rc; p.family = INSV2V_PLAN_NONE; return p; };
    constexpr int Q8 = INSV2V_PLAN_Q8, R8 = INSV2V_PLAN_R8, W4 = INSV2V_PLAN_W4;
    auto engine = [&](int family, int variant = 0, bool finalize = true) {
        const int rc = family == R8 ? r8_refusal(d, variant) : family == Q8 ? q8_refusal(d, variant) : w4_refusal(d, variant);
        if (rc) return rc;
        p.family = family; p.variant = variant; p.forced_tile = engine_tile_code(family) + variant;
        p.ln_finalize = finalize && d.stats_parts > 0;
        p.cim = family == R8 && r8_uses_cim(d, variant, sw);
        return 0;
    };
    auto halo = [&](int cfg, int tws) { p.family = INSV2V_PLAN_HALO; p.variant = cfg; p.forced_tile = 100 + cfg; p.tw_shift = tws | (sw.halo_legacy_map ? 256 : 0); return p; };

    if (const int rc = validate_gemm(d, stats_w)) return refuse(rc);
    if (split) {
        if (d.batch > 1 || d.stats_out || d.split_k > 1) return refuse(INSV2V_EUNSUPPORTED);
        const int64_t per = units_per_part(d, window), total = conv ? d.NB : d.M;
        if (per <= 0) return refuse(INSV2V_EUNSUPPORTED);
        const bool finalize = d.stats_parts > 0;
        if (finalize) stats_finished(d);
        const insv2v_gemm_plan_t first = plan_gemm(window_part(d, 0, per), cus, window, sw);
        if (first.rc) return refuse(first.rc);
        const int32_t stats_w_ = p.stats_width, fuse = p.gn_fuse;
        p = first;
        p.stats_width = stats_w_; p.gn_fuse = fuse; p.ln_finalize = finalize;
        p.parts = (int32_t)((total + per - 1) / per);
        p.units_per_part = (int32_t)per;
        return p;
    }
    if (d.w_group_rows > 0) {
        const int64_t groups = ((int64_t)d.M + d.w_group_rows - 1) / d.w_group_rows;
        if (beyond_2g(groups * d.w_group_stride * 2)) return refuse(INSV2V_EUNSUPPORTED);
        if (cus <= 0) return refuse(INSV2V_EINVAL);
        const bool r_ok = d.N % 320 == 0, q_ok = d.N % 256 == 0;
        const pingpong_cost c = pingpong_costs(d, cus);
        const bool use_r = d.tile / 10 == 24 ? true : d.tile / 10 == 23 ? false : (r_ok && (!q_ok || c.r8 <= c.q8));
        if (use_r ? !r_ok : !q_ok) return refuse(INSV2V_EUNSUPPORTED);
        if (const int rc = engine(use_r ? R8 : Q8)) return refuse(rc);
        return p;
    }
    if (d.tile >= 200 && d.tile <= 206) return refuse(INSV2V_EUNSUPPORTED);
    if ((d.tile >= 230 && d.tile <= 249) || (d.tile >= 210 && d.tile <= 221)) {
        const int family = d.tile >= 240 ? R8 : d.tile >= 230 ? Q8 : W4;
        if (d.split_k > 1 || (d.stats_out && family != R8)) return refuse(INSV2V_EUNSUPPORTED);
        d.split_k = 1;
        if (const int rc = engine(family, d.tile - engine_tile_code(family))) return refuse(rc);
        return p;
    }
    const int nsplit = d.stats_out ? 1 : split_choice(d);
    int shape = d.tile % 10, ring = d.tile / 10;
    if (nsplit > 1) splitk_main_pass(d, nsplit);
    else d.split_k = 1;
    if (nsplit > 1 && shape == 0) shape = 5;
    const bool by_rule = nsplit <= 1 && d.tile == 0;
    if (by_rule && !d.gn_ab) {
        const int pp = pingpong_choice(d, d.stats_out != nullptr, cus, sw);
        if (pp && !engine(pp == 2 ? R8 : Q8)) return p;
        if (pp && d.stats_out) return refuse(INSV2V_EUNSUPPORTED);
    }
    if (by_rule && !d.stats_out && d.act == INSV2V_ACT_GEGLU && !conv && !d.k_split && !d.residual && sw.r8_geglu && cus > 0 && d.N % 320 == 0 &&
        d.M >= 8192 && d.K >= 640 && !d.c_fp32 && d.batch <= 1) {
        const pingpong_cost c = pingpong_costs(d, cus);
        if (c.r8 <= c.q8 && !engine(R8)) return p;
    }
    if (by_rule && !d.stats_out) {
        const int pick = persistent_choice(d, sw);
        if (pick && !engine(pick == 1 ? Q8 : W4)) return p;
    }
    if (nsplit <= 1 && (d.tile == 100 || d.tile == 0)) {
        const int tws = halo_tw_shift(d);
        if (d.tile == 100 && (tws < 0 || d.act >= INSV2V_ACT_RELU)) return refuse(INSV2V_EUNSUPPORTED);
        if (tws >= 0 && d.act < INSV2V_ACT_RELU && (d.tile == 100 || halo_fills_chip(d))) return halo(0, tws);
    }
    if (d.gn_ab) return refuse(INSV2V_EUNSUPPORTED);
    if (by_rule && conv && d.batch == 1 && !d.c_fp32 && d.M >= 10240 && d.N >= 640 && d.K >= 5760 && sw.persistent && !engine(Q8, 0, false)) return p;
    if (d.tile >= 101 && d.tile <= 103) {
        int tws = halo_tw_shift(d);
        if (d.act >= INSV2V_ACT_RELU || (nsplit <= 1 && tws < 0)) return refuse(INSV2V_EUNSUPPORTED);
        if (d.tile == 103) tws = (d.OH % 16 == 0 && d.OW % 16 == 0) ? 4 : (d.OH % 32 == 0 && d.OW % 8 == 0) ? 3 : -1;
        if (nsplit <= 1) return tws < 0 ? refuse(INSV2V_EUNSUPPORTED) : halo(d.tile - 100, tws);
    }
    if (shape == 0) shape = pick_tile(d);
    if (d.act == INSV2V_ACT_GEGLU && tile_bn(shape) == 64) shape = 2;
    if (ring == 0) ring = 2;
    if (ring < 2 || ring > 4 || shape < 1 || shape > 9) return refuse(INSV2V_EINVAL);
    if (tile_lds_bytes(tile_bm(shape), tile_bn(shape), ring) > TILE_LDS_MAX) return refuse(INSV2V_EUNSUPPORTED);
    p.family = INSV2V_PLAN_TILE; p.variant = shape; p.ring = ring; p.forced_tile = shape + 10 * ring;
    p.split_k = nsplit; p.splitk_reduce = nsplit > 1;
    return p;
}
```

### instruct-video-to-video_amd/csrc/gemm_q8.hip

```cpp
#include "common.h"
#include "gemm_dma.h"
#include "gemm_plan.h"
#include <type_traits>

namespace {

constexpr int HALF_B = 128 * 128;
constexpr int RING_B = 8 * HALF_B;
constexpr int PARK_B = 5 * 1024;
constexpr int LDS_B = RING_B + 2 * PARK_B;
constexpr int STAMP_B = 8 * 512;

#ifndef Q8_MID_SPREAD
#define Q8_MID_SPREAD 1
#endif
#define SB() __builtin_amdgcn_sched_barrier(0)
#define BARRIER() do { SB(); __builtin_amdgcn_s_barrier(); SB(); } while (0)

typedef unsigned uint4v __attribute__((ext_vector_type(4)));
__device__ __forceinline__ unsigned pack_h2(float x, float y) {
    typedef float f2_t __attribute__((ext_vector_type(2)));
    const f2_t v = {x, y};
    return __builtin_bit_cast(unsigned, __builtin_convertvector(v, half2v));
}
__device__ __forceinline__ float h_lo(unsigned u) { return (float)__builtin_bit_cast(half2v, u)[0]; }
__device__ __forceinline__ float h_hi(unsigned u) { return (float)__builtin_bit_cast(half2v, u)[1]; }

template <int I> using ic = std::integral_constant<int, I>;

template <int MODE, bool GEGLU, bool HAS_RES, int DBG = 0, int VAR = 0>
__global__ __launch_bounds__(512) void gemm_q8_kernel(insv2v_gemm_desc p) {
    extern __shared__ __attribute__((aligned(16))) char smem[];
    const int tid = threadIdx.x, lane = tid & 63;
    const int wid = __builtin_amdgcn_readfirstlane(tid >> 6);
    const int wm = wid >> 2, wn = wid & 3;
    const int G = (int)gridDim.x;

    const int tiles_n = (p.N + 255) >> 8, tiles_m = (p.M + 255) >> 8, ntiles = tiles_m * tiles_n;
    auto tile_origin = [&](int v, int& bm0, int& bn0) {
        const int bid = xcd_remap(v, ntiles);
        constexpr int GROUP_M = 8;
        const int per_group = GROUP_M * tiles_n;
        const int gidx = bid / per_group, first_m = gidx * GROUP_M;
        const int gsz = min(GROUP_M, tiles_m - first_m), rin = bid - gidx * per_group;
        const int tn = rin / gsz, tm = first_m + rin - tn * gsz;
        bm0 = tm << 8; bn0 = tn << 8;
    };

    const srd_t rA = make_srd(p.a), rA2 = make_srd(p.a2 ? p.a2 : p.a), rW = make_srd(p.w);
    const bool ln = p.row_stats != nullptr;
    const srd_t rBias = make_srd(p.bias ? (const void*)p.bias : p.w), rCs = make_srd(ln ? (const void*)p.col_sum : p.w),
                rSt = make_srd(ln ? (const void*)p.row_stats : p.w), rRb = make_srd(p.row_bias ? (const void*)p.row_bias : p.w);

    const int prow = wid * 8 + (lane >> 3);
    const int chunk8 = ((lane & 7) ^ ((prow >> 1) & 7)) * 8;
    int arow[4];
    int aoh[4], aow[4];
    unsigned aoff[4];
    unsigned woff[4];
    const int nk = p.K / BK;
    const int IHu = p.upsample ? p.OH : p.IH, IWu = p.upsample ? p.OW : p.IW;
    const int ups = p.upsample ? 1 : 0;
    struct Cursor { int v, kt, k0, kh, kw, ci0, soffA; bool second; unsigned wbase; } cur = {(int)blockIdx.x, 0, 0, 0, 0, 0, 0, false, 0u};
    auto refresh_aoff = [&]() {
        const int ld = (int)(cur.second ? p.lda2 : p.lda);
#pragma unroll
        for (int r = 0; r < 4; ++r) {
            if (MODE == INSV2V_MODE_LINEAR) {
                aoff[r] = arow[r] >= 0 ? (unsigned)((arow[r] * ld + chunk8) * 2) : OOB_OFFSET;
            } else {
                const int ih = aoh[r] + cur.kh, iw = aow[r] + cur.kw;
                const bool ok = arow[r] >= 0 && (unsigned)ih < (unsigned)IHu && (unsigned)iw < (unsigned)IWu;
                const int pix = arow[r] + (ih >> ups) * p.IW + (iw >> ups);
                aoff[r] = ok ? (unsigned)((pix * ld + chunk8) * 2) : OOB_OFFSET;
            }
        }
    };
    auto set_stage_rows = [&](int v) {
        int bm0 = 0, bn0 = 0;
        const bool live = v < ntiles;
        if (live) tile_origin(v, bm0, bn0);
        cur.wbase = (MODE == INSV2V_MODE_LINEAR && live && p.w_group_rows > 0) ? (unsigned)((int64_t)(bm0 / p.w_group_rows) * p.w_group_stride * 2) : 0u;
#pragma unroll
        for (int r = 0; r < 4; ++r) {
            const int hh = r >> 1, rr = (r & 1) * 64 + prow;
            const int m = bm0 + hh * 128 + rr;
            const bool okm = live && m < p.M;
            if (MODE == INSV2V_MODE_LINEAR) {
                arow[r] = okm ? m : -1;
                aoh[r] = aow[r] = 0;
            } else {
                const int mm = okm ? m : 0;
                const int ow = mm % p.OW, t = mm / p.OW;
                const int oh = t % p.OH, nb = t / p.OH;
                arow[r] = okm ? nb * p.IH * p.IW : -1;
                aoh[r] = oh * p.stride - p.pad_t;
                aow[r] = ow * p.stride - p.pad_l;
            }
            const int r5 = rr & 31, pr = (rr & ~31) | (((r5 >> 2) & 3) * 8 + (r5 >> 4) * 4 + (r5 & 3));
            const int n = bn0 + (GEGLU ? (pr >> 5) * 64 + hh * 32 + (pr & 31) : hh * 128 + pr);
            woff[r] = (live && n < p.N) ? (unsigned)(((int64_t)n * p.ldw + chunk8) * 2) : OOB_OFFSET;
        }
    };
    auto advance = [&]() {
        bool newtile = false, refresh = false;
        if (++cur.kt == nk) {
            cur.v += G; cur.kt = 0; cur.k0 = 0; cur.kh = cur.kw = cur.ci0 = 0; cur.soffA = 0; cur.second = false;
            newtile = true;
        } else {
            cur.k0 += BK; cur.soffA += BK * 2;
            if (MODE == INSV2V_MODE_LINEAR) {
                if (p.k_split > 0 && cur.k0 == p.k_split) { cur.second = true; cur.soffA = 0; refresh = true; }
            } else {
                cur.ci0 += BK;
                if (cur.ci0 >= p.Cin) {
                    cur.ci0 = 0; cur.soffA = 0;
                    if (++cur.kw == 3) { cur.kw = 0; ++cur.kh; }
                    cur.second = false; refresh = true;
                } else if (p.k_split > 0 && cur.ci0 == p.k_split) {
                    cur.second = true; cur.soffA = 0; refresh = true;
                }
            }
        }
        if (newtile) set_stage_rows(cur.v);
        if (newtile || refresh) refresh_aoff();
    };
    auto stage_piece = [&](auto part_c, auto buf_c, int i) {
        constexpr int PART = decltype(part_c)::value, BUF = decltype(buf_c)::value;
        char* dst = smem + (PART * 2 + BUF) * HALF_B + wid * 1024 + i * 8192;
        if (PART >= 2) dma16(rW, woff[(PART - 2) * 2 + i], cur.k0 * 2 + (int)cur.wbase, dst);
        else dma16(cur.second ? rA2 : rA, aoff[PART * 2 + i], cur.soffA, dst);
    };
    auto stage = [&](auto part_c, auto buf_c) { stage_piece(part_c, buf_c, 0); stage_piece(part_c, buf_c, 1); };
    auto row_group = [&](int m) { int g = m / p.rows_per_group; if (p.rb_mod > 0) g %= p.rb_mod; return g; };
    auto stage_park = [&](int pb, int bm0, int bn0) {
        char* dst = smem + RING_B + pb * PARK_B + wid * 1024;
        if (wid == 0) {
            const int n = bn0 + lane * 4;
            dma16(rBias, (p.bias && n < p.N) ? (unsigned)(n * 4) : OOB_OFFSET, 0, dst);
        } else if (wid == 1) {
            const int n = bn0 + lane * 4;
            dma16(rCs, (ln && n < p.N) ? (unsigned)(n * 4) : OOB_OFFSET, 0, dst);
        } else if (wid == 2 || wid == 3) {
            const int m = bm0 + (wid - 2) * 128 + lane * 2;
            dma16(rSt, (ln && m < p.M) ? (unsigned)(m * 8) : OOB_OFFSET, 0, dst);
        } else if (wid == 4) {
            const int n = bn0 + lane * 4;
            const int g = p.row_bias ? row_group(bm0) : 0;
            dma16(rRb, (p.row_bias && n < p.N) ? (unsigned)((g * (int)p.ld_rb + n) * 4) : OOB_OFFSET, 0, dst);
        }
    };

    const int l15 = lane & 15, lq = lane >> 4, fsw = l15 >> 1;
    const char* aRd[2];
    const char* wRd[2];
#pragma unroll
    for (int kb = 0; kb < 2; ++kb) {
        const int co = ((kb * 4 + lq) ^ fsw) * 16;
        aRd[kb] = smem + (wm * 64 + l15) * 128 + co;
        wRd[kb] = smem + 4 * HALF_B + (wn * 32 + l15) * 128 + co;
    }

    half8 fa[4][2], fw0[2][2], fw1[2][2];
    floatx4 acc[2][2][4][2];
    auto zero_acc = [&]() {
#pragma unroll
        for (int i = 0; i < 2; ++i)
#pragma unroll
            for (int j = 0; j < 2; ++j)
#pragma unroll
                for (int tb = 0; tb < 4; ++tb)
#pragma unroll
                    for (int cb = 0; cb < 2; ++cb) acc[i][j][tb][cb] = floatx4{0.f, 0.f, 0.f, 0.f};
    };
    auto read_a = [&](auto buf_c, auto jq_c) {
        constexpr int B = decltype(buf_c)::value, JQ = decltype(jq_c)::value;
#pragma unroll
        for (int tb = 0; tb < 4; ++tb)
#pragma unroll
            for (int kb = 0; kb < 2; ++kb) fa[tb][kb] = *(const half8*)(aRd[kb] + (JQ * 2 + B) * HALF_B + tb * 16 * 128);
    };
    auto read_w = [&](auto buf_c, auto iq_c, half8 (&fw)[2][2]) {
        constexpr int B = decltype(buf_c)::value, IQ = decltype(iq_c)::value;
#pragma unroll
        for (int cb = 0; cb < 2; ++cb)
#pragma unroll
            for (int kb = 0; kb < 2; ++kb) fw[cb][kb] = *(const half8*)(wRd[kb] + (IQ * 2 + B) * HALF_B + cb * 16 * 128);
    };
    int stamp_i = 0;
    const unsigned stamp_lds = (unsigned)(uintptr_t)(__attribute__((address_space(3))) char*)smem + LDS_B + wid * 512;
    auto stamp_begin = [&](unsigned long long& t0) {
        if (DBG == 4) asm volatile("s_memtime %0\n\ts_waitcnt lgkmcnt(0)" : "=s"(t0)::"memory");
    };
    auto stamp_end = [&](unsigned long long t0) {
        if (DBG == 4) {
            unsigned long long t1;
            asm volatile("s_memtime %0\n\ts_waitcnt lgkmcnt(0)" : "=s"(t1)::"memory");
            if (stamp_i < 32) {
                const unsigned a = stamp_lds + stamp_i * 16;
                asm volatile("ds_write_b64 %0, %1\n\tds_write_b64 %0, %2 offset:8" ::"v"(a), "v"(t0), "v"(t1) : "memory");
            }
            ++stamp_i;
        }
    };
    auto mma = [&](floatx4 (&c)[4][2], const half8 (&fw)[2][2], auto part_c, auto buf_c) {
        unsigned long long t0 = 0;
        stamp_begin(t0);
        __builtin_amdgcn_s_setprio(1);
#if Q8_MID_SPREAD
        if (VAR == 1) { stage_piece(part_c, buf_c, 0); stage_piece(part_c, buf_c, 1); }
#endif
#pragma unroll
        for (int kb = 0; kb < 2; ++kb)
#pragma unroll
            for (int tb = 0; tb < 4; ++tb)
#pragma unroll
                for (int cb = 0; cb < 2; ++cb) {
                    c[tb][cb] = __builtin_amdgcn_mfma_f32_16x16x32_f16(fw[cb][kb], fa[tb][kb], c[tb][cb], 0, 0, 0);
#if !Q8_MID_SPREAD
                    const int idx = kb * 8 + tb * 2 + cb;
                    if (VAR == 1 && (idx == 3 || idx == 9)) { SB(); stage_piece(part_c, buf_c, idx == 3 ? 0 : 1); SB(); }
#endif
                }
#if Q8_MID_SPREAD
        if (VAR == 1) {
#pragma unroll
            for (int i = 0; i < 16; ++i) {
                __builtin_amdgcn_sched_group_barrier(0x008, 1, 0);
                __builtin_amdgcn_sched_group_barrier(0x002, 2, 0);
                __builtin_amdgcn_sched_group_barrier(0x004, 1, 0);
                __builtin_amdgcn_sched_group_barrier(0x020, 1, 0);
            }
        }
#endif
        __builtin_amdgcn_s_setprio(0);
        stamp_end(t0);
    };

    const unsigned lds0 = (unsigned)(uintptr_t)(__attribute__((address_space(3))) char*)smem;
    const srd_t rC = make_srd(p.c), rR = make_srd(p.residual ? p.residual : p.c);
    auto park6 = [&](unsigned a, floatx4& b0, floatx4& b1, floatx4& r0, floatx4& r1, floatx4& c0, floatx4& c1) {
        asm volatile("ds_read_b128 %0, %6\n\tds_read_b128 %1, %6 offset:16\n\tds_read_b128 %2, %6 offset:4096\n\t"
                     "ds_read_b128 %3, %6 offset:4112\n\tds_read_b128 %4, %6 offset:1024\n\tds_read_b128 %5, %6 offset:1040\n\t"
                     "s_waitcnt lgkmcnt(0)"
                     : "=&v"(b0), "=&v"(b1), "=&v"(r0), "=&v"(r1), "=&v"(c0), "=&v"(c1) : "v"(a) : "memory");
    };
    auto stat4 = [&](unsigned a, float2& s0, float2& s1, float2& s2, float2& s3) {
        asm volatile("ds_read_b64 %0, %4\n\tds_read_b64 %1, %4 offset:128\n\tds_read_b64 %2, %4 offset:256\n\t"
                     "ds_read_b64 %3, %4 offset:384\n\ts_waitcnt lgkmcnt(0)"
                     : "=&v"(s0), "=&v"(s1), "=&v"(s2), "=&v"(s3) : "v"(a) : "memory");
    };
    auto epilogue = [&](int bm0, int bn0, int pb) {
        if (DBG == 2 || DBG == 4) {
            float s = 0.f;
#pragma unroll
            for (int i = 0; i < 2; ++i)
#pragma unroll
                for (int j = 0; j < 2; ++j)
#pragma unroll
                    for (int tb = 0; tb < 4; ++tb)
#pragma unroll
                        for (int cb = 0; cb < 2; ++cb)
#pragma unroll
                            for (int r = 0; r < 4; ++r) s += acc[i][j][tb][cb][r];
            if (s == 12345.678f) ((half_t*)p.c)[tid] = (half_t)s;
            return;
        }
        const unsigned park = lds0 + RING_B + pb * PARK_B;
        constexpr int NIQ = GEGLU ? 1 : 2;
        const int oN = GEGLU ? (p.N >> 1) : p.N;
        const int e15 = lane & 15, eg = lane >> 4;
        auto chan0 = [&](int iq) { return GEGLU ? wn * 64 : iq * 128 + wn * 32; };
        auto ocol0 = [&](int iq) { return GEGLU ? (bn0 >> 1) + wn * 32 : bn0 + chan0(iq); };
        constexpr bool LINM = MODE == INSV2V_MODE_LINEAR;
        float ra[LINM ? 8 : 1], rm[LINM ? 8 : 1];
        unsigned offc[8], offr[8];
        {
            if (!LINM) { ra[0] = p.alpha; rm[0] = 0.f; }
#pragma unroll
            for (int jq = 0; jq < 2; ++jq) {
                float2 st[4];
                if (LINM) stat4(park + 2048 + (jq * 128 + wm * 64 + e15) * 8, st[0], st[1], st[2], st[3]);
#pragma unroll
                for (int tb = 0; tb < 4; ++tb) {
                    const int rbk = jq * 4 + tb;
                    const int m = bm0 + jq * 128 + wm * 64 + tb * 16 + e15;
                    if (LINM) {
                        const float mean = ln ? st[tb].x : 0.f, rstd = ln ? st[tb].y : 1.f;
                        ra[rbk] = rstd * p.alpha; rm[rbk] = -rstd * mean;
                    }
                    offc[rbk] = m < p.M ? (unsigned)(m * (int)p.ldc * 2 + eg * 16) : OOB_OFFSET;
                    offr[rbk] = m < p.M ? (unsigned)(m * (int)p.ldr * 2 + eg * 16) : OOB_OFFSET;
                }
            }
        }
        uint4v rv[8];
        auto load_res = [&](int iq) {
            const int on = ocol0(iq);
            const bool okc = on + eg * 8 + 8 <= oN;
#pragma unroll
            for (int rbk = 0; rbk < 8; ++rbk) rv[rbk] = __builtin_amdgcn_raw_buffer_load_b128(rR, okc ? offr[rbk] : OOB_OFFSET, on * 2, 0);
            asm volatile("s_waitcnt vmcnt(0)" ::: "memory");
            SB();
        };
#pragma unroll
        for (int iq = 0; iq < NIQ; ++iq) {
            if (HAS_RES) load_res(iq);
            float bs[8], cs[8], gbs[8], gcs[8];
            {
                floatx4 tb_[2], tr[2], tc[2], gb[2], gr[2], gc[2];
                const unsigned a = park + (chan0(iq) + 8 * eg) * 4;
                park6(a, tb_[0], tb_[1], tr[0], tr[1], tc[0], tc[1]);
                if (GEGLU) park6(a + 128, gb[0], gb[1], gr[0], gr[1], gc[0], gc[1]);
#pragma unroll
                for (int h = 0; h < 2; ++h)
#pragma unroll
                    for (int e = 0; e < 4; ++e) {
                        bs[4 * h + e] = tb_[h][e] + tr[h][e]; cs[4 * h + e] = tc[h][e];
                        if (GEGLU) { gbs[4 * h + e] = gb[h][e] + gr[h][e]; gcs[4 * h + e] = gc[h][e]; }
                    }
            }
            const int on = ocol0(iq);
            const bool okc = on + eg * 8 + 8 <= oN;
#pragma unroll
            for (int rbk = 0; rbk < 8; ++rbk) {
                const int jq = rbk >> 2, tb = rbk & 3, ri = LINM ? rbk : 0;
                float v[8];
#pragma unroll
                for (int h = 0; h < 2; ++h)
#pragma unroll
                    for (int e = 0; e < 4; ++e) {
                        float x = fmaf(ra[ri], acc[iq][jq][tb][h][e], fmaf(rm[ri], cs[4 * h + e], bs[4 * h + e]));
                        if (GEGLU) x *= gelu_erf_f(fmaf(ra[ri], acc[1][jq][tb][h][e], fmaf(rm[ri], gcs[4 * h + e], gbs[4 * h + e])));
                        v[4 * h + e] = x;
                    }
                if (HAS_RES) {
                    const uint4v r = rv[rbk];
                    v[0] += h_lo(r[0]); v[1] += h_hi(r[0]); v[2] += h_lo(r[1]); v[3] += h_hi(r[1]);
                    v[4] += h_lo(r[2]); v[5] += h_hi(r[2]); v[6] += h_lo(r[3]); v[7] += h_hi(r[3]);
                }
                const uint4v out = {pack_h2(v[0], v[1]), pack_h2(v[2], v[3]), pack_h2(v[4], v[5]), pack_h2(v[6], v[7])};
                __builtin_amdgcn_raw_buffer_store_b128(out, rC, okc ? offc[rbk] : OOB_OFFSET, on * 2, 0);
                asm volatile("s_nop 7" ::"v"(out));
            }
        }
    };

    int cbm0, cbn0;
    int cv = blockIdx.x, cpb = 0;
    tile_origin(cv, cbm0, cbn0);
    set_stage_rows(cv);
    refresh_aoff();
    stage_park(0, cbm0, cbn0);
    stage(ic<2>{}, ic<0>{}); stage(ic<0>{}, ic<0>{}); stage(ic<3>{}, ic<0>{}); stage(ic<1>{}, ic<0>{});
    advance();
    stage(ic<2>{}, ic<1>{}); stage(ic<0>{}, ic<1>{}); stage(ic<3>{}, ic<1>{});
    wait_vmcnt<6>();
    BARRIER();
    zero_acc();

    auto tile_step = [&](auto buf_c, bool first, int nbm0, int nbn0, int npb) {
        constexpr int B = decltype(buf_c)::value;
        read_w(ic<B>{}, ic<0>{}, fw0);
        SB();
        read_a(ic<B>{}, ic<0>{});
        SB();
        if (first) stage_park(npb, nbm0, nbn0);
        if (VAR == 0) { stage(ic<1>{}, ic<B ^ 1>{}); advance(); }
        asm volatile("s_waitcnt lgkmcnt(8)" ::: "memory");
        BARRIER();
        mma(acc[0][0], fw0, ic<1>{}, ic<B ^ 1>{});
        BARRIER();
        read_w(ic<B>{}, ic<1>{}, fw1);
        if (VAR == 0) stage(ic<2>{}, ic<B>{}); else advance();
        BARRIER();
        mma(acc[1][0], fw1, ic<2>{}, ic<B>{});
        BARRIER();
        read_a(ic<B>{}, ic<1>{});
        if (VAR == 0) stage(ic<0>{}, ic<B>{});
        BARRIER();
        mma(acc[1][1], fw1, ic<0>{}, ic<B>{});
        BARRIER();
        if (VAR == 0) { stage(ic<3>{}, ic<B>{}); wait_vmcnt<6>(); } else wait_vmcnt<4>();
        BARRIER();
        mma(acc[0][1], fw0, ic<3>{}, ic<B>{});
        BARRIER();
    };
    int par = 0;
    for (; cv < ntiles; cv += G) {
        tile_origin(cv, cbm0, cbn0);
        if (wm == 1) BARRIER();
        bool first = cv != (int)blockIdx.x;
        int t = 0;
        if (par) { tile_step(ic<1>{}, first, cbm0, cbn0, cpb); first = false; t = 1; par = 0; }
        for (; t + 1 < nk; t += 2) {
            tile_step(ic<0>{}, first, cbm0, cbn0, cpb);
            first = false;
            tile_step(ic<1>{}, false, cbm0, cbn0, cpb);
        }
        if (t < nk) { tile_step(ic<0>{}, first, cbm0, cbn0, cpb); par = 1; }
        if (DBG != 3) { if (wm == 0) BARRIER(); }
        epilogue(cbm0, cbn0, cpb);
        if (DBG == 3) { if (wm == 0) BARRIER(); }
        zero_acc();
        cpb ^= 1;
    }
    if (DBG == 4 && blockIdx.x < 8 && p.workspace) {
        asm volatile("s_waitcnt lgkmcnt(0)" ::: "memory");
        const unsigned long long v = *(const unsigned long long*)(smem + LDS_B + wid * 512 + lane * 8);
        ((unsigned long long*)p.workspace)[((int)blockIdx.x * 8 + wid) * 64 + lane] = v;
    }
}

template <int MODE, bool GEGLU, bool HAS_RES, int DBG = 0, int VAR = 0>
int launch_q8(const insv2v_gemm_desc& d, hipStream_t s) {
    static bool attr_set = false;
    if (const int e = set_dynamic_lds(attr_set, (const void*)gemm_q8_kernel<MODE, GEGLU, HAS_RES, DBG, VAR>, LDS_B + STAMP_B)) return e;
    const int num_cu = insv2v_num_cus();
    if (num_cu <= 0) return INSV2V_EINVAL;
    const int tiles = ((d.M + 255) / 256) * ((d.N + 255) / 256);
    hipLaunchKernelGGL((gemm_q8_kernel<MODE, GEGLU, HAS_RES, DBG, VAR>), dim3(tiles < num_cu ? tiles : num_cu), dim3(512), LDS_B + (DBG == 4 ? STAMP_B : 0), s, d);
    return launch_status();
}

}

int insv2v_gemm_q8(const insv2v_gemm_desc& d, int variant, hipStream_t s) {
    if (const int rc = q8_refusal(d, variant)) return rc;
    const bool conv = d.mode == INSV2V_MODE_CONV3X3, gg = d.act == INSV2V_ACT_GEGLU, res = d.residual != nullptr;
    constexpr int L = INSV2V_MODE_LINEAR, C = INSV2V_MODE_CONV3X3;
    switch (variant) {
        case 0:
            if (conv) return res ? launch_q8<C, false, true, 0, 1>(d, s) : launch_q8<C, false, false, 0, 1>(d, s);
            if (gg) return launch_q8<L, true, false, 0, 1>(d, s);
            return res ? launch_q8<L, false, true, 0, 1>(d, s) : launch_q8<L, false, false, 0, 1>(d, s);
        case 1:
            if (conv) return res ? launch_q8<C, false, true, 0, 0>(d, s) : launch_q8<C, false, false, 0, 0>(d, s);
            if (gg) return launch_q8<L, true, false, 0, 0>(d, s);
            return res ? launch_q8<L, false, true, 0, 0>(d, s) : launch_q8<L, false, false, 0, 0>(d, s);
        case 2: return launch_q8<L, false, false, 2, 1>(d, s);
        case 3:
            if (gg) return launch_q8<L, true, false, 3, 1>(d, s);
            return res ? launch_q8<L, false, true, 3, 1>(d, s) : launch_q8<L, false, false, 3, 1>(d, s);
        case 4: return launch_q8<L, false, false, 4, 1>(d, s);
        case 5: return launch_q8<L, false, false, 4, 0>(d, s);
    }
    return INSV2V_EINVAL;
}
```

### instruct-video-to-video_amd/csrc/gemm_r8.hip

```cpp
#include "common.h"
#include "gemm_dma.h"
#include "gemm_plan.h"
#include <type_traits>

namespace {

constexpr int BM = 256, BN = 320;
constexpr int AH_B = 128 * 128;
constexpr int WB_B = 64 * 128;
constexpr int W_BASE = 4 * AH_B;
constexpr int RING_B = 4 * AH_B + 10 * WB_B;
constexpr int PK_BIAS = 0, PK_CS = 2048, PK_ST = 4096, PK_RB = 6144, PARK_B = 8192;
constexpr int LDS_B = RING_B + 2 * PARK_B;

#ifndef R8_MID_SPREAD
#define R8_MID_SPREAD 1
#endif
#define SB() __builtin_amdgcn_sched_barrier(0)
#define BARRIER() do { SB(); __builtin_amdgcn_s_barrier(); SB(); } while (0)

typedef unsigned uint4v __attribute__((ext_vector_type(4)));
typedef unsigned uint2v __attribute__((ext_vector_type(2)));
__device__ __forceinline__ unsigned pack_h2(float x, float y) {
    typedef float f2_t __attribute__((ext_vector_type(2)));
    const f2_t v = {x, y};
    return __builtin_bit_cast(unsigned, __builtin_convertvector(v, half2v));
}
__device__ __forceinline__ float h_lo(unsigned u) { return (float)__builtin_bit_cast(half2v, u)[0]; }
__device__ __forceinline__ float h_hi(unsigned u) { return (float)__builtin_bit_cast(half2v, u)[1]; }

template <int I> using ic = std::integral_constant<int, I>;

template <int MODE, bool HAS_RES, int DBG = 0, bool SPLIT = true, bool STATS = false, bool GEGLU = false, bool CIM = false>
__global__ __launch_bounds__(512) void gemm_r8_kernel(insv2v_gemm_desc p, int dephase) {
    extern __shared__ __attribute__((aligned(16))) char smem[];
    const int tid = threadIdx.x, lane = tid & 63;
    const int wid = __builtin_amdgcn_readfirstlane(tid >> 6);
    const int wm = wid >> 1, wn = wid & 1, grp = wid >> 2;
    const int G = (int)gridDim.x;
    constexpr bool LIN = MODE == INSV2V_MODE_LINEAR;

    const int tiles_n = (p.N + BN - 1) / BN, tiles_m = (p.M + BM - 1) / BM, ntiles = tiles_m * tiles_n;
    if (dephase > 0 && ntiles > G) {
        const int n0 = ntiles % G;
        if (n0 != 0 && (int)blockIdx.x >= n0) {
            const float tile_cycles = (float)(p.K / BK) * 3700.f + (HAS_RES ? 30000.f : 10000.f);
            const float frac = (float)((int)blockIdx.x - n0 + 1) / (float)(G - n0 + 1) * (float)dephase * 0.001f;
            const unsigned long long wait = (unsigned long long)(frac * tile_cycles);
            unsigned long long t0, t1;
            asm volatile("s_memtime %0\n\ts_waitcnt lgkmcnt(0)" : "=s"(t0)::"memory");
            do {
                __builtin_amdgcn_s_sleep(64);
                asm volatile("s_memtime %0\n\ts_waitcnt lgkmcnt(0)" : "=s"(t1)::"memory");
            } while (t1 - t0 < wait);
        }
    }
    auto tile_origin = [&](int v, int& bm0, int& bn0) {
        const int bid = xcd_remap(v, ntiles);
        constexpr int GROUP_M = 8;
        const int per_group = GROUP_M * tiles_n;
        const int gidx = bid / per_group, first_m = gidx * GROUP_M;
        const int gsz = min(GROUP_M, tiles_m - first_m), rin = bid - gidx * per_group;
        const int tn = rin / gsz, tm = first_m + rin - tn * gsz;
        bm0 = tm * BM; bn0 = tn * BN;
    };

    const srd_t rA = make_srd(p.a), rA2 = make_srd(p.a2 ? p.a2 : p.a), rW = make_srd(p.w);
    const bool ln = p.row_stats != nullptr;

    const int prow = wid * 8 + (lane >> 3);
    const int chunk8 = ((lane & 7) ^ ((prow >> 1) & 7)) * 8;
    unsigned aoff[4];
    unsigned amask[2] = {0, 0};
    unsigned woff;
    unsigned amax = 0;
    const unsigned wmax = (unsigned)(((int64_t)(p.N - 1) * p.ldw + chunk8) * 2);
    const int nk = p.K / BK;
    const int IHu = p.upsample ? p.OH : p.IH, IWu = p.upsample ? p.OW : p.IW;
    const int ups = p.upsample ? 1 : 0;
    struct Cursor { int v, kt, k0, kh, kw, ci0, soffA, abm0; bool second; int tap, dpix; unsigned wbase; } cur = {(int)blockIdx.x, 0, 0, 0, 0, 0, 0, 0, false, 0, 0, 0u};
    if (CIM) cur.dpix = -p.IW - 1;
    auto refresh_aoff = [&]() {
        const int ld = (int)((SPLIT && cur.second) ? p.lda2 : p.lda);
        if (LIN) {
            aoff[0] = ((unsigned)(cur.abm0 + prow) * (unsigned)ld + (unsigned)chunk8) * 2u;
            amax = ((unsigned)(p.M - 1) * (unsigned)ld + (unsigned)chunk8) * 2u;
        } else {
            const float rOW = 1.0f / (float)p.OW, rOH = 1.0f / (float)p.OH;
#pragma unroll
            for (int r = 0; r < 4; ++r) {
                const int m = cur.abm0 + (r >> 1) * 128 + (r & 1) * 64 + prow;
                const bool okm = m < p.M;
                const int mm = okm ? m : 0;
                int t = (int)((float)mm * rOW);
                int ow = mm - t * p.OW;
                if (ow < 0) { ow += p.OW; --t; } else if (ow >= p.OW) { ow -= p.OW; ++t; }
                int nb = (int)((float)t * rOH);
                int oh = t - nb * p.OH;
                if (oh < 0) { oh += p.OH; --nb; } else if (oh >= p.OH) { oh -= p.OH; ++nb; }
                if (CIM) {
                    aoff[r] = (unsigned)(nb * p.IH * p.IW + oh * p.IW + ow);
                    const unsigned vh = (okm && oh > 0 ? 1u : 0u) | (okm ? 2u : 0u) | (okm && oh + 1 < p.IH ? 4u : 0u);
                    const unsigned vw = (ow > 0 ? 1u : 0u) | 2u | (ow + 1 < p.IW ? 4u : 0u);
                    const unsigned bits = ((vh & 1u) ? vw : 0u) | ((vh & 2u) ? vw << 3 : 0u) | ((vh & 4u) ? vw << 6 : 0u);
                    if (r & 1) amask[r >> 1] |= bits << 9; else amask[r >> 1] = bits;
                } else {
                    const int ih = oh * p.stride - p.pad_t + cur.kh, iw = ow * p.stride - p.pad_l + cur.kw;
                    const bool ok = okm && (unsigned)ih < (unsigned)IHu && (unsigned)iw < (unsigned)IWu;
                    const int pix = nb * p.IH * p.IW + (ih >> ups) * p.IW + (iw >> ups);
                    aoff[r] = ok ? (unsigned)((pix * ld + chunk8) * 2) : OOB_OFFSET;
                }
            }
        }
    };
    auto set_stage_rows = [&](int v) {
        int bm0 = 0, bn0 = 0;
        const bool live = v < ntiles;
        if (live) tile_origin(v, bm0, bn0);
        else { bm0 = p.M + BM; bn0 = p.N + BN; }
        cur.abm0 = bm0;
        cur.wbase = (LIN && live && p.w_group_rows > 0) ? (unsigned)((int64_t)(bm0 / p.w_group_rows) * p.w_group_stride * 2) : 0u;
        const int c32 = (wid & 3) * 8 + (lane >> 3);
        const int pc = ((c32 >> 2) & 3) * 8 + (c32 >> 4) * 4 + (c32 & 3);
        const int n = GEGLU ? bn0 + (c32 >> 4) * 32 + (c32 & 15) : bn0 + (wid >> 2) * 160 + pc;
        woff = ((unsigned)n * (unsigned)p.ldw + (unsigned)chunk8) * 2u;
    };
    auto advance = [&]() {
        bool newtile = false, refresh = false;
        if (++cur.kt == nk) {
            cur.v += G; cur.kt = 0; cur.k0 = 0; cur.kh = cur.kw = cur.ci0 = 0; cur.soffA = 0; cur.second = false;
            if (CIM) { cur.tap = 0; cur.dpix = -p.IW - 1; }
            newtile = true;
        } else if (CIM) {
            if (++cur.tap == 9) { cur.tap = 0; cur.ci0 += BK; }
            const int kh = (cur.tap * 11) >> 5, kw = cur.tap - 3 * kh;
            cur.dpix = (kh - 1) * p.IW + kw - 1;
            cur.second = SPLIT && p.k_split > 0 && cur.ci0 >= p.k_split;
            cur.soffA = (cur.ci0 - (cur.second ? p.k_split : 0)) * 2;
            cur.k0 = cur.tap * p.Cin + cur.ci0;
        } else {
            cur.k0 += BK; cur.soffA += BK * 2;
            if (LIN) {
                if (SPLIT && p.k_split > 0 && cur.k0 == p.k_split) { cur.second = true; cur.soffA = 0; refresh = true; }
            } else {
                cur.ci0 += BK;
                if (cur.ci0 >= p.Cin) {
                    cur.ci0 = 0; cur.soffA = 0;
                    if (++cur.kw == 3) { cur.kw = 0; ++cur.kh; }
                    cur.second = false; refresh = true;
                } else if (SPLIT && p.k_split > 0 && cur.ci0 == p.k_split) {
                    cur.second = true; cur.soffA = 0; refresh = true;
                }
            }
        }
        if (newtile) set_stage_rows(cur.v);
        if (newtile || refresh) refresh_aoff();
    };
    auto stage_a = [&](auto h_c, auto buf_c, int i) {
        constexpr int H = decltype(h_c)::value, BUF = decltype(buf_c)::value;
        char* dst = smem + (H * 2 + BUF) * AH_B + i * 8192 + wid * 1024;
        if (LIN) {
            const int ld = (int)((SPLIT && cur.second) ? p.lda2 : p.lda);
            dma16((SPLIT && cur.second) ? rA2 : rA, min(aoff[0] + (unsigned)((H * 128 + i * 64) * ld * 2), amax), cur.soffA, dst);
        } else if (CIM) {
            constexpr int R = H * 2;
            const unsigned ld2 = (unsigned)((SPLIT && cur.second) ? p.lda2 : p.lda) * 2u;
            const bool ok = (amask[H] >> (i * 9 + cur.tap)) & 1u;
            const unsigned off = __umul24(aoff[R + i] + (unsigned)cur.dpix, ld2) + (unsigned)(chunk8 * 2);
            dma16((SPLIT && cur.second) ? rA2 : rA, ok ? off : OOB_OFFSET, cur.soffA, dst);
        } else {
            dma16((SPLIT && cur.second) ? rA2 : rA, aoff[H * 2 + i], cur.soffA, dst);
        }
    };
    auto stage_w = [&](auto pb_c, auto buf_c) {
        constexpr int PB = decltype(pb_c)::value, BUF = decltype(buf_c)::value;
        char* dst = smem + W_BASE + (PB * 2 + BUF) * WB_B + wid * 1024;
        if (GEGLU) {
            const int t = (wid >> 2) * 5 + PB;
            dma16(rW, min(woff + (unsigned)(((t >> 1) * 64 + (t & 1) * 16) * (int)p.ldw * 2), wmax), cur.k0 * 2 + (int)cur.wbase, dst);
        } else {
            dma16(rW, min(woff + (unsigned)(PB * 32 * (int)p.ldw * 2), wmax), cur.k0 * 2 + (int)cur.wbase, dst);
        }
    };
    auto row_group = [&](int m) { int g = m / p.rows_per_group; if (p.rb_mod > 0) g %= p.rb_mod; return g; };
    auto stage_park = [&](int pb, int bm0, int bn0) {
        char* park = smem + RING_B + pb * PARK_B;
        const srd_t rBias = make_srd(p.bias ? (const void*)p.bias : p.w), rCs = make_srd(ln ? (const void*)p.col_sum : p.w),
                    rSt = make_srd(ln ? (const void*)p.row_stats : p.w), rRb = make_srd(p.row_bias ? (const void*)p.row_bias : p.w);
        const int hi = wid & 1;
        const int n = bn0 + hi * 256 + lane * 4;
        const bool okn = n < p.N && (hi == 0 || lane < 16);
        if (wid < 2) {
            dma16(rBias, (p.bias && okn) ? (unsigned)(n * 4) : OOB_OFFSET, 0, park + PK_BIAS + hi * 1024);
        } else if (wid < 4) {
            dma16(rCs, (ln && okn) ? (unsigned)(n * 4) : OOB_OFFSET, 0, park + PK_CS + hi * 1024);
        } else if (wid < 6) {
            const int m = bm0 + hi * 128 + lane * 2;
            dma16(rSt, (ln && m < p.M) ? (unsigned)(m * 8) : OOB_OFFSET, 0, park + PK_ST + hi * 1024);
        } else {
            const int g = p.row_bias ? row_group(bm0) : 0;
            dma16(rRb, (p.row_bias && okn) ? (unsigned)((g * (int)p.ld_rb + n) * 4) : OOB_OFFSET, 0, park + PK_RB + hi * 1024);
        }
    };

    const int l15 = lane & 15, lq = lane >> 4, fsw = l15 >> 1;
    const char* aRd[2];
    const char* wRd[2];
#pragma unroll
    for (int kb = 0; kb < 2; ++kb) {
        const int co = ((kb * 4 + lq) ^ fsw) * 16;
        aRd[kb] = smem + grp * 2 * AH_B + ((wm & 1) * 64 + l15) * 128 + co;
        wRd[kb] = smem + W_BASE + (wn * 32 + l15) * 128 + co;
    }

    half8 fa[4][2], fw[2][2];
    floatx4 acc[5][4][2];
    auto zero_acc = [&]() {
#pragma unroll
        for (int i = 0; i < 5; ++i)
#pragma unroll
            for (int tb = 0; tb < 4; ++tb)
#pragma unroll
                for (int cb = 0; cb < 2; ++cb) acc[i][tb][cb] = floatx4{0.f, 0.f, 0.f, 0.f};
    };
    auto read_a = [&](auto buf_c) {
        constexpr int B = decltype(buf_c)::value;
#pragma unroll
        for (int tb = 0; tb < 4; ++tb)
#pragma unroll
            for (int kb = 0; kb < 2; ++kb) fa[tb][kb] = *(const half8*)(aRd[kb] + B * AH_B + tb * 16 * 128);
    };
    auto read_w = [&](auto buf_c, auto pb_c) {
        constexpr int B = decltype(buf_c)::value, PB = decltype(pb_c)::value;
        if (PB < 4) {
#pragma unroll
            for (int cb = 0; cb < 2; ++cb)
#pragma unroll
                for (int kb = 0; kb < 2; ++kb) fw[cb][kb] = *(const half8*)(wRd[kb] + (PB * 2 + B) * WB_B + cb * 16 * 128);
        } else {
            int far;
            asm volatile("s_mov_b32 %0, 0x10000" : "=s"(far));
#pragma unroll
            for (int cb = 0; cb < 2; ++cb)
#pragma unroll
                for (int kb = 0; kb < 2; ++kb) fw[cb][kb] = *(const half8*)(wRd[kb] + far + B * WB_B + cb * 16 * 128);
        }
    };
    unsigned dbg_seg[5] = {0, 0, 0, 0, 0}, dbg_gap[5] = {0, 0, 0, 0, 0}, dbg_last = 0, dbg_n = 0;
    auto mma = [&](auto pb_c, auto&& mid) {
        constexpr int PB = decltype(pb_c)::value;
        unsigned long long tb_ = 0;
        if (DBG == 5) {
            asm volatile("s_memtime %0\n\ts_waitcnt lgkmcnt(0)" : "=s"(tb_)::"memory");
            if (dbg_n) dbg_gap[(PB + 4) % 5] += (unsigned)tb_ - dbg_last;
            dbg_last = (unsigned)tb_;
        }
        __builtin_amdgcn_s_setprio(1);
#if R8_MID_SPREAD
        mid(0); mid(1);
#endif
#pragma unroll
        for (int kb = 0; kb < 2; ++kb)
#pragma unroll
            for (int tb = 0; tb < 4; ++tb)
#pragma unroll
                for (int cb = 0; cb < 2; ++cb) {
                    acc[PB][tb][cb] = __builtin_amdgcn_mfma_f32_16x16x32_f16(fw[cb][kb], fa[tb][kb], acc[PB][tb][cb], 0, 0, 0);
#if !R8_MID_SPREAD
                    if (kb * 8 + tb * 2 + cb == 3) { SB(); mid(0); SB(); }
                    if (kb * 8 + tb * 2 + cb == 9) { SB(); mid(1); SB(); }
#endif
                }
#if R8_MID_SPREAD
#pragma unroll
        for (int i = 0; i < 16; ++i) {
            __builtin_amdgcn_sched_group_barrier(0x008, 1, 0);
            __builtin_amdgcn_sched_group_barrier(0x002, 2, 0);
            __builtin_amdgcn_sched_group_barrier(0x004, 1, 0);
            __builtin_amdgcn_sched_group_barrier(0x020, 1, 0);
        }
#endif
        __builtin_amdgcn_s_setprio(0);
        if (DBG == 5) {
            unsigned long long te;
            asm volatile("s_memtime %0\n\ts_waitcnt lgkmcnt(0)" : "=s"(te)::"memory");
            dbg_seg[PB] += (unsigned)te - (unsigned)tb_;
            if (PB == 4) ++dbg_n;
        }
    };

    const unsigned lds0 = (unsigned)(uintptr_t)(__attribute__((address_space(3))) char*)smem;
    auto park6 = [&](unsigned a, floatx4& b0, floatx4& b1, floatx4& r0, floatx4& r1, floatx4& c0, floatx4& c1) {
        if constexpr (GEGLU)
            asm volatile("ds_read_b128 %0, %6\n\tds_read_b128 %1, %6 offset:128\n\tds_read_b128 %2, %6 offset:6144\n\t"
                         "ds_read_b128 %3, %6 offset:6272\n\tds_read_b128 %4, %6 offset:2048\n\tds_read_b128 %5, %6 offset:2176\n\t"
                         "s_waitcnt lgkmcnt(0)"
                         : "=&v"(b0), "=&v"(b1), "=&v"(r0), "=&v"(r1), "=&v"(c0), "=&v"(c1) : "v"(a) : "memory");
        else
            asm volatile("ds_read_b128 %0, %6\n\tds_read_b128 %1, %6 offset:16\n\tds_read_b128 %2, %6 offset:6144\n\t"
                         "ds_read_b128 %3, %6 offset:6160\n\tds_read_b128 %4, %6 offset:2048\n\tds_read_b128 %5, %6 offset:2064\n\t"
                         "s_waitcnt lgkmcnt(0)"
                         : "=&v"(b0), "=&v"(b1), "=&v"(r0), "=&v"(r1), "=&v"(c0), "=&v"(c1) : "v"(a) : "memory");
    };
    auto stat4 = [&](unsigned a, float2& s0, float2& s1, float2& s2, float2& s3) {
        asm volatile("ds_read_b64 %0, %4\n\tds_read_b64 %1, %4 offset:128\n\tds_read_b64 %2, %4 offset:256\n\tds_read_b64 %3, %4 offset:384\n\t"
                     "s_waitcnt lgkmcnt(0)" : "=&v"(s0), "=&v"(s1), "=&v"(s2), "=&v"(s3) : "v"(a) : "memory");
    };
    auto epilogue = [&](int bm0, int bn0, int pb) {
        if (DBG == 2 || DBG == 5) {
            float s = 0.f;
#pragma unroll
            for (int i = 0; i < 5; ++i)
#pragma unroll
                for (int tb = 0; tb < 4; ++tb)
#pragma unroll
                    for (int cb = 0; cb < 2; ++cb)
#pragma unroll
                        for (int r = 0; r < 4; ++r) s += acc[i][tb][cb][r];
            if (s == 12345.678f) ((half_t*)p.c)[tid] = (half_t)s;
            return;
        }
        unsigned elane;
        asm volatile("v_mbcnt_lo_u32_b32 %0, -1, 0\n\tv_mbcnt_hi_u32_b32 %0, -1, %0" : "=v"(elane));
        const int e15 = (int)(elane & 15), eg = (int)(elane >> 4);
        const srd_t rC = make_srd(p.c), rR = make_srd(p.residual ? p.residual : p.c);
        const unsigned park = lds0 + RING_B + pb * PARK_B;
        float ra[LIN ? 4 : 1], rm[LIN ? 4 : 1];
        unsigned offc[4], offr[4];
        {
            float2 st[4];
            if (LIN) stat4(park + PK_ST + (wm * 64 + e15) * 8, st[0], st[1], st[2], st[3]);
            else { ra[0] = p.alpha; rm[0] = 0.f; }
#pragma unroll
            for (int tb = 0; tb < 4; ++tb) {
                const int m = bm0 + wm * 64 + tb * 16 + e15;
                if (LIN) {
                    const float mean = ln ? st[tb].x : 0.f, rstd = ln ? st[tb].y : 1.f;
                    ra[tb] = rstd * p.alpha; rm[tb] = -rstd * mean;
                }
                offc[tb] = m < p.M ? (unsigned)(m * (int)p.ldc * 2 + eg * (GEGLU ? 8 : 16)) : OOB_OFFSET;
                offr[tb] = m < p.M ? (unsigned)(m * (int)p.ldr * 2 + eg * 16) : OOB_OFFSET;
            }
        }
        if constexpr (GEGLU) {
#pragma unroll
            for (int pbk = 0; pbk < 5; ++pbk) {
                const int t = wn * 5 + pbk;
                const int nl = (t >> 1) * 64 + (t & 1) * 16 + 4 * eg;
                float bh[4], ch[4], bg[4], cg[4];
                {
                    floatx4 tb_[2], tr[2], tc[2];
                    park6(park + nl * 4, tb_[0], tb_[1], tr[0], tr[1], tc[0], tc[1]);
#pragma unroll
                    for (int e = 0; e < 4; ++e) { bh[e] = tb_[0][e] + tr[0][e]; ch[e] = tc[0][e]; bg[e] = tb_[1][e] + tr[1][e]; cg[e] = tc[1][e]; }
                }
                const int on = (bn0 >> 1) + t * 16;
                const bool okc = on + eg * 4 + 4 <= (p.N >> 1);
#pragma unroll
                for (int tb = 0; tb < 4; ++tb) {
                    float v[4];
#pragma unroll
                    for (int e = 0; e < 4; ++e) {
                        const float x = fmaf(ra[LIN ? tb : 0], acc[pbk][tb][0][e], fmaf(rm[LIN ? tb : 0], ch[e], bh[e]));
                        const float g = fmaf(ra[LIN ? tb : 0], acc[pbk][tb][1][e], fmaf(rm[LIN ? tb : 0], cg[e], bg[e]));
                        v[e] = x * gelu_erf_f(g);
                    }
                    const uint2v out = {pack_h2(v[0], v[1]), pack_h2(v[2], v[3])};
                    __builtin_amdgcn_raw_buffer_store_b64(out, rC, okc ? offc[tb] : OOB_OFFSET, on * 2, 0);
                    asm volatile("s_nop 7" ::"v"(out));
                }
            }
            return;
        }
        uint4v rv[2][4];
        auto load_res = [&](auto pbk_c, auto slot_c) {
            constexpr int PBK = decltype(pbk_c)::value, SLOT = decltype(slot_c)::value;
            const int on = bn0 + wn * 160 + PBK * 32;
            const bool okc = on + eg * 8 + 8 <= p.N;
#pragma unroll
            for (int tb = 0; tb < 4; ++tb) rv[SLOT][tb] = __builtin_amdgcn_raw_buffer_load_b128(rR, okc ? offr[tb] : OOB_OFFSET, on * 2, 0);
        };
        if (HAS_RES) {
            load_res(ic<0>{}, ic<0>{}); load_res(ic<1>{}, ic<1>{});
            asm volatile("s_waitcnt vmcnt(0)" ::: "memory");
            SB();
        }
        float st1[4] = {0.f, 0.f, 0.f, 0.f}, st2[4] = {0.f, 0.f, 0.f, 0.f};
#pragma unroll
        for (int pbk = 0; pbk < 5; ++pbk) {
            const int slot = pbk & 1;
            if (HAS_RES && (pbk == 2 || pbk == 4)) { asm volatile("s_waitcnt vmcnt(0)" ::: "memory"); SB(); }
            const int cl = wn * 160 + pbk * 32 + 8 * eg;
            float bs[8], cs[8];
            {
                floatx4 tb_[2], tr[2], tc[2];
                park6(park + cl * 4, tb_[0], tb_[1], tr[0], tr[1], tc[0], tc[1]);
#pragma unroll
                for (int h = 0; h < 2; ++h)
#pragma unroll
                    for (int e = 0; e < 4; ++e) { bs[4 * h + e] = tb_[h][e] + tr[h][e]; cs[4 * h + e] = tc[h][e]; }
            }
            const int on = bn0 + wn * 160 + pbk * 32;
            const bool okc = on + eg * 8 + 8 <= p.N;
#pragma unroll
            for (int tb = 0; tb < 4; ++tb) {
                float v[8];
#pragma unroll
                for (int h = 0; h < 2; ++h)
#pragma unroll
                    for (int e = 0; e < 4; ++e) v[4 * h + e] = fmaf(ra[LIN ? tb : 0], acc[pbk][tb][h][e], fmaf(rm[LIN ? tb : 0], cs[4 * h + e], bs[4 * h + e]));
                if (HAS_RES) {
                    const uint4v r = rv[slot][tb];
                    v[0] += h_lo(r[0]); v[1] += h_hi(r[0]); v[2] += h_lo(r[1]); v[3] += h_hi(r[1]);
                    v[4] += h_lo(r[2]); v[5] += h_hi(r[2]); v[6] += h_lo(r[3]); v[7] += h_hi(r[3]);
                }
                if (STATS) {
#pragma unroll
                    for (int e = 0; e < 8; ++e) { st1[tb] += v[e]; st2[tb] = fmaf(v[e], v[e], st2[tb]); }
                }
                const uint4v out = {pack_h2(v[0], v[1]), pack_h2(v[2], v[3]), pack_h2(v[4], v[5]), pack_h2(v[6], v[7])};
                __builtin_amdgcn_raw_buffer_store_b128(out, rC, okc ? offc[tb] : OOB_OFFSET, on * 2, 0);
                asm volatile("s_nop 7" ::"v"(out));
            }
            if (HAS_RES) {
                SB();
                if (pbk == 0) load_res(ic<2>{}, ic<0>{});
                if (pbk == 1) load_res(ic<3>{}, ic<1>{});
                if (pbk == 2) load_res(ic<4>{}, ic<0>{});
                SB();
            }
        }
        if (STATS) {
            const int part = bn0 / 160 + wn;
#pragma unroll
            for (int tb = 0; tb < 4; ++tb) {
                const int m = bm0 + wm * 64 + tb * 16 + e15;
                float s1 = st1[tb] + __shfl_xor(st1[tb], 16, 64), s2 = st2[tb] + __shfl_xor(st2[tb], 16, 64);
                s1 += __shfl_xor(s1, 32, 64); s2 += __shfl_xor(s2, 32, 64);
                if (eg == 0 && m < p.M) *(float2*)(p.stats_out + ((int64_t)part * p.M + m) * 2) = make_float2(s1, s2);
            }
        }
    };

    int cbm0, cbn0;
    int cv = blockIdx.x, cpb = 0;
    tile_origin(cv, cbm0, cbn0);
    set_stage_rows(cv);
    refresh_aoff();
    stage_park(0, cbm0, cbn0);
    stage_a(ic<0>{}, ic<0>{}, 0); stage_a(ic<0>{}, ic<0>{}, 1); stage_a(ic<1>{}, ic<0>{}, 0); stage_a(ic<1>{}, ic<0>{}, 1);
    stage_w(ic<0>{}, ic<0>{}); stage_w(ic<1>{}, ic<0>{}); stage_w(ic<2>{}, ic<0>{}); stage_w(ic<3>{}, ic<0>{}); stage_w(ic<4>{}, ic<0>{});
    advance();
    stage_a(ic<0>{}, ic<1>{}, 0); stage_a(ic<0>{}, ic<1>{}, 1); stage_a(ic<1>{}, ic<1>{}, 0); stage_a(ic<1>{}, ic<1>{}, 1);
    stage_w(ic<0>{}, ic<1>{}); stage_w(ic<1>{}, ic<1>{});
    wait_vmcnt<6>();
    BARRIER();
    zero_acc();

    auto tile_step = [&](auto buf_c, bool first, int nbm0, int nbn0, int npb) {
        constexpr int B = decltype(buf_c)::value;
        read_w(ic<B>{}, ic<0>{});
        SB();
        read_a(ic<B>{});
        SB();
        if (first) stage_park(npb, nbm0, nbn0);
        BARRIER();
        mma(ic<0>{}, [&](int i) { if (i == 0) stage_w(ic<2>{}, ic<B ^ 1>{}); else stage_w(ic<3>{}, ic<B ^ 1>{}); });
        BARRIER();
        read_w(ic<B>{}, ic<1>{});
        BARRIER();
        mma(ic<1>{}, [&](int i) { if (i == 0) stage_w(ic<4>{}, ic<B ^ 1>{}); });
        BARRIER();
        read_w(ic<B>{}, ic<2>{});
        advance();
        BARRIER();
        mma(ic<2>{}, [&](int i) { stage_a(ic<0>{}, ic<B>{}, i); });
        BARRIER();
        read_w(ic<B>{}, ic<3>{});
        BARRIER();
        mma(ic<3>{}, [&](int i) { stage_a(ic<1>{}, ic<B>{}, i); });
        BARRIER();
        read_w(ic<B>{}, ic<4>{});
        wait_vmcnt<4>();
        BARRIER();
        mma(ic<4>{}, [&](int i) { if (i == 0) stage_w(ic<0>{}, ic<B>{}); else stage_w(ic<1>{}, ic<B>{}); });
        BARRIER();
    };
    int par = 0;
    unsigned long long cyc_loop = 0, cyc_join = 0, cyc_epi = 0, ntl = 0, ts0 = 0, ts1 = 0, ts2 = 0, ts3 = 0;
    auto stamp = [&](unsigned long long& t) { if (DBG == 4) asm volatile("s_memtime %0\n\ts_waitcnt lgkmcnt(0)" : "=s"(t)::"memory"); };
    for (; cv < ntiles; cv += G) {
        tile_origin(cv, cbm0, cbn0);
        stamp(ts0);
        if (grp == 1) BARRIER();
        bool first = cv != (int)blockIdx.x;
        int t = 0;
        if (par) { tile_step(ic<1>{}, first, cbm0, cbn0, cpb); first = false; t = 1; par = 0; }
        for (; t + 1 < nk; t += 2) {
            tile_step(ic<0>{}, first, cbm0, cbn0, cpb);
            first = false;
            tile_step(ic<1>{}, false, cbm0, cbn0, cpb);
        }
        if (t < nk) { tile_step(ic<0>{}, first, cbm0, cbn0, cpb); par = 1; }
        stamp(ts1);
        if (grp == 0) BARRIER();
        stamp(ts2);
        epilogue(cbm0, cbn0, cpb);
        stamp(ts3);
        if (DBG == 4) { cyc_loop += ts1 - ts0; cyc_join += ts2 - ts1; cyc_epi += ts3 - ts2; ++ntl; }
        zero_acc();
        cpb ^= 1;
    }
    if (DBG == 5 && p.workspace && blockIdx.x < 64 && lane == 0) {
        unsigned* o = (unsigned*)p.workspace + ((int)blockIdx.x * 8 + wid) * 12;
#pragma unroll
        for (int i = 0; i < 5; ++i) { o[i] = dbg_seg[i]; o[5 + i] = dbg_gap[i]; }
        o[10] = dbg_n; o[11] = 0;
    }
    if (DBG == 4 && p.workspace && blockIdx.x < 64 && lane == 0) {
        unsigned long long* o = (unsigned long long*)p.workspace + ((int)blockIdx.x * 8 + wid) * 4;
        o[0] = cyc_loop; o[1] = cyc_join; o[2] = cyc_epi; o[3] = ntl;
    }
}

template <int MODE, bool HAS_RES, int DBG = 0, bool SPLIT = true, bool STATS = false, bool GEGLU = false, bool CIM = false>
int launch_r8(const insv2v_gemm_desc& d, hipStream_t s) {
    static bool attr_set = false;
    if (const int e = set_dynamic_lds(attr_set, (const void*)gemm_r8_kernel<MODE, HAS_RES, DBG, SPLIT, STATS, GEGLU, CIM>, LDS_B)) return e;
    const int num_cu = insv2v_num_cus();
    if (num_cu <= 0) return INSV2V_EINVAL;
    const int tiles = ((d.M + BM - 1) / BM) * ((d.N + BN - 1) / BN);
    const int dephase = insv2v_gemm_switches().r8_dephase;
    hipLaunchKernelGGL((gemm_r8_kernel<MODE, HAS_RES, DBG, SPLIT, STATS, GEGLU, CIM>), dim3(tiles < num_cu ? tiles : num_cu), dim3(512), LDS_B, s, d, dephase);
    return launch_status();
}

}

int insv2v_gemm_r8(const insv2v_gemm_desc& d, int variant, hipStream_t s) {
    if (const int rc = r8_refusal(d, variant)) return rc;
    const bool conv = d.mode == INSV2V_MODE_CONV3X3, res = d.residual != nullptr;
    constexpr int L = INSV2V_MODE_LINEAR, C = INSV2V_MODE_CONV3X3;
    if (d.act == INSV2V_ACT_GEGLU) return launch_r8<L, false, 0, false, false, true>(d, s);
    if (d.stats_out) return res ? launch_r8<L, true, 0, false, true>(d, s) : launch_r8<L, false, 0, false, true>(d, s);
    if (r8_uses_cim(d, variant, insv2v_gemm_switches())) {
        if (variant == 4) return res ? launch_r8<C, true, 4, true, false, false, true>(d, s) : launch_r8<C, false, 4, true, false, false, true>(d, s);
        if (d.k_split > 0) return res ? launch_r8<C, true, 0, true, false, false, true>(d, s) : launch_r8<C, false, 0, true, false, false, true>(d, s);
        return res ? launch_r8<C, true, 0, false, false, false, true>(d, s) : launch_r8<C, false, 0, false, false, false, true>(d, s);
    }
    switch (variant) {
        case 0:
            if (d.k_split > 0) {
                if (conv) return res ? launch_r8<C, true>(d, s) : launch_r8<C, false>(d, s);
                return res ? launch_r8<L, true>(d, s) : launch_r8<L, false>(d, s);
            }
            if (conv) return res ? launch_r8<C, true, 0, false>(d, s) : launch_r8<C, false, 0, false>(d, s);
            return res ? launch_r8<L, true, 0, false>(d, s) : launch_r8<L, false, 0, false>(d, s);
        case 2: return conv ? launch_r8<C, false, 2>(d, s) : launch_r8<L, false, 2>(d, s);
        case 5: return conv ? launch_r8<C, false, 5>(d, s) : launch_r8<L, false, 5>(d, s);
        case 4:
            if (conv) return res ? launch_r8<C, true, 4>(d, s) : launch_r8<C, false, 4>(d, s);
            return res ? launch_r8<L, true, 4>(d, s) : launch_r8<L, false, 4>(d, s);
    }
    return INSV2V_EINVAL;
}
```

### instruct-video-to-video_amd/insv2v/_lib.py

```python
import ctypes as C
import os

import torch

ABI_VERSION = 14
_HERE = os.path.dirname(os.path.abspath(__file__))
LIB_PATH = os.environ.get("INSV2V_LIB", os.path.join(_HERE, "libinsv2v_hip.so"))

c_i32, c_i64, c_f32, c_p = C.c_int32, C.c_int64, C.c_float, C.c_void_p


class GemmDesc(C.Structure):
    _fields_ = [("a", c_p), ("a2", c_p), ("w", c_p), ("c", c_p), ("bias", c_p), ("row_bias", c_p), ("residual", c_p),
                ("row_stats", c_p), ("col_sum", c_p),
                ("lda", c_i64), ("lda2", c_i64), ("ldw", c_i64), ("ldc", c_i64), ("ldr", c_i64), ("ld_rb", c_i64),
                ("a_bs", c_i64), ("w_bs", c_i64), ("c_bs", c_i64), ("r_bs", c_i64),
                ("workspace", c_p), ("workspace_bytes", c_i64),
                ("M", c_i32), ("N", c_i32), ("K", c_i32), ("k_split", c_i32), ("rows_per_group", c_i32),
                ("rb_mod", c_i32), ("act", c_i32), ("c_fp32", c_i32), ("mode", c_i32),
                ("NB", c_i32), ("IH", c_i32), ("IW", c_i32), ("OH", c_i32), ("OW", c_i32), ("Cin", c_i32),
                ("stride", c_i32), ("pad_t", c_i32), ("pad_l", c_i32), ("upsample", c_i32),
                ("batch", c_i32), ("tile", c_i32), ("split_k", c_i32), ("alpha", c_f32),
                ("gn_ab", c_p), ("gn_images_per_sample", c_i32), ("gn_silu", c_i32),
                ("stats_out", c_p), ("stats_scratch", c_p), ("stats_parts", c_i32), ("ln_eps", c_f32),
                ("w_group_stride", c_i64), ("w_group_rows", c_i32), ("reserved0", c_i32)]


class GemmPlan(C.Structure):
    _fields_ = [(n, c_i32) for n in ("rc", "family", "variant", "ring", "tw_shift", "cim", "split_k", "ln_finalize", "splitk_reduce", "stats_width",
                                     "gn_fuse", "parts", "units_per_part", "forced_tile")]


class WinogradInDesc(C.Structure):
    _fields_ = [("x", c_p), ("x2", c_p), ("gn_ab", c_p), ("v", c_p), ("ldx", c_i64), ("ldx2", c_i64), ("v_group_rows", c_i64),
                ("NB", c_i32), ("H", c_i32), ("W", c_i32), ("C", c_i32), ("C1", c_i32), ("gn_images_per_sample", c_i32), ("gn_silu", c_i32), ("upsample", c_i32)]


class WinogradOutDesc(C.Structure):
    _fields_ = [("m", c_p), ("bias", c_p), ("row_bias", c_p), ("residual", c_p), ("y", c_p), ("m_group_rows", c_i64),
                ("ldr", c_i64), ("ldy", c_i64), ("ld_rb", c_i64), ("NB", c_i32), ("H", c_i32), ("W", c_i32), ("Cout", c_i32), ("rows_per_group", c_i32), ("upsample", c_i32)]


class FfnDesc(C.Structure):
    _fields_ = [("x", c_p), ("out", c_p), ("wstream", c_p), ("ldx", c_i64), ("ldo", c_i64),
                ("M", c_i32), ("C", c_i32), ("hidden", c_i32), ("eps", c_f32), ("post_residual", c_p), ("ld_post", c_i64), ("post", c_i32)]


class RowLinDesc(C.Structure):
    _fields_ = [("x", c_p), ("out", c_p), ("residual", c_p), ("wstream", c_p), ("ldx", c_i64), ("ldo", c_i64), ("ldr", c_i64),
                ("M", c_i32), ("N", c_i32), ("K", c_i32), ("layernorm", c_i32), ("frame_bias", c_i32), ("rows_per_frame", c_i32),
                ("frames", c_i32), ("eps", c_f32), ("stats_out", c_p), ("stats_eps", c_f32), ("gn_ab", c_p), ("gn_rows", c_i32)]


class TattnDesc(C.Structure):
    _fields_ = [("x", c_p), ("out", c_p), ("wstream", c_p), ("ldx", c_i64), ("ldo", c_i64),
                ("samples", c_i32), ("HW", c_i32), ("C", c_i32), ("heads", c_i32), ("frames", c_i32), ("eps", c_f32), ("scale", c_f32)]


class XattnDesc(C.Structure):
    _fields_ = [("x", c_p), ("out", c_p), ("wstream", c_p), ("kvstream", c_p), ("ldx", c_i64), ("ldo", c_i64),
                ("M", c_i32), ("rows_per_sample", c_i32), ("C", c_i32), ("heads", c_i32), ("ctx_len", c_i32), ("eps", c_f32), ("scale", c_f32),
                ("pre_residual", c_p), ("ld_pre", c_i64)]


class GroupNormDesc(C.Structure):
    _fields_ = [("x", c_p), ("x2", c_p), ("y", c_p), ("gamma", c_p), ("beta", c_p), ("partials", c_p),
                ("ldx", c_i64), ("ldx2", c_i64), ("ldy", c_i64),
                ("nsamples", c_i32), ("rows_per_sample", c_i32), ("C", c_i32), ("C1", c_i32), ("G", c_i32),
                ("nchunks", c_i32), ("silu", c_i32), ("eps", c_f32), ("ab", c_p), ("stats_only", c_i32)]


class LayerNormDesc(C.Structure):
    _fields_ = [("x", c_p), ("y", c_p), ("gamma", c_p), ("beta", c_p), ("pe", c_p),
                ("ldx", c_i64), ("ldy", c_i64), ("rows", c_i32), ("C", c_i32),
                ("rows_per_frame", c_i32), ("frames", c_i32), ("pe_start", c_i32), ("eps", c_f32)]


class AttentionDesc(C.Structure):
    _fields_ = [("q", c_p), ("k", c_p), ("v", c_p), ("o", c_p),
                ("q_rs", c_i64), ("k_rs", c_i64), ("v_rs", c_i64), ("o_rs", c_i64),
                ("q_outer", c_i64), ("q_step", c_i64), ("kv_outer", c_i64), ("kv_step", c_i64),
                ("o_outer", c_i64), ("o_step", c_i64),
                ("q_inner", c_i32), ("kv_inner", c_i32), ("o_inner", c_i32),
                ("batch", c_i32), ("heads", c_i32), ("head_dim", c_i32), ("seq_q", c_i32), ("seq_k", c_i32),
                ("scale", c_f32), ("causal", c_i32), ("q_bias", c_p), ("k_bias", c_p), ("v_bias", c_p), ("bias_rs", c_i64)]


class StepDesc(C.Structure):
    _fields_ = [("eps_in", c_p), ("latent", c_p), ("latent_ref", c_p), ("delta_q", c_p), ("noise", c_p),
                ("rescale_stats", c_p), ("latent_out", c_p), ("pred_x0", c_p), ("eps_out", c_p),
                ("nbranch", c_i32), ("F", c_i32), ("h", c_i32), ("w", c_i32), ("R", c_i32), ("correct", c_i32),
                ("text_cfg", c_f32), ("img_cfg", c_f32), ("sqrt_a", c_f32), ("sqrt_1ma", c_f32),
                ("c_x0", c_f32), ("c_eps", c_f32), ("c_xt", c_f32), ("c_noise", c_f32), ("guidance_rescale", c_f32),
                ("branch_stride", c_i64), ("noise_seed", c_i64), ("noise_stream", c_i64), ("noise_on", c_i32)]


class MStepDesc(C.Structure):
    _fields_ = StepDesc._fields_ + [("x0_hist", c_p), ("c_hist", c_f32)]


class MaskStepDesc(C.Structure):
    _fields_ = MStepDesc._fields_ + [("mask", c_p), ("src", c_p), ("known_noise", c_p), ("k_src", c_f32), ("k_noise", c_f32)]


class Im2colDesc(C.Structure):
    _fields_ = [("x", c_p), ("x2", c_p), ("out", c_p), ("ldx", c_i64), ("ldx2", c_i64), ("ldo", c_i64),
                ("N", c_i32), ("IH", c_i32), ("IW", c_i32), ("C", c_i32), ("C1", c_i32), ("KH", c_i32), ("KW", c_i32),
                ("stride_h", c_i32), ("stride_w", c_i32), ("pad_h", c_i32), ("pad_w", c_i32), ("OH", c_i32), ("OW", c_i32)]


class CorrLookupDesc(C.Structure):
    _fields_ = [("pyr0", c_p), ("pyr1", c_p), ("pyr2", c_p), ("pyr3", c_p), ("coords", c_p), ("out", c_p), ("ldo", c_i64),
                ("B", c_i32), ("h", c_i32), ("w", c_i32), ("levels", c_i32), ("radius", c_i32)]


SIGNATURES = {
    "insv2v_abi_version": (c_i32, []),
    "insv2v_init": (c_i32, []),
    "insv2v_gemm": (c_i32, [C.POINTER(GemmDesc), c_p]),
    "insv2v_gemm_stats_parts": (c_i32, [C.POINTER(GemmDesc)]),
    "insv2v_gemm_plan": (c_i32, [C.POINTER(GemmDesc), c_i32, C.POINTER(GemmPlan)]),
    "insv2v_set_operand_window": (c_i64, [c_i64]),
    "insv2v_conv3x3_fuses_groupnorm": (c_i32, [C.POINTER(GemmDesc)]),
    "insv2v_winograd_input": (c_i32, [C.POINTER(WinogradInDesc), c_p]),
    "insv2v_winograd_output": (c_i32, [C.POINTER(WinogradOutDesc), c_p]),
    "insv2v_ffn_fused": (c_i32, [C.POINTER(FfnDesc), c_p]),
    "insv2v_ffn_stream_elems": (c_i64, [c_i32, c_i32, c_i32]),
    "insv2v_rowlin": (c_i32, [C.POINTER(RowLinDesc), c_p]),
    "insv2v_rowlin_stream_elems": (c_i64, [c_i32, c_i32]),
    "insv2v_tattn_fused": (c_i32, [C.POINTER(TattnDesc), c_p]),
    "insv2v_tattn_stream_elems": (c_i64, [c_i32, c_i32, c_i32]),
    "insv2v_tattn_attn": (c_i32, [C.POINTER(TattnDesc), c_p]),
    "insv2v_tattn_attn_stream_elems": (c_i64, [c_i32, c_i32, c_i32]),
    "insv2v_xattn_fused": (c_i32, [C.POINTER(XattnDesc), c_p]),
    "insv2v_xattn_stream_elems": (c_i64, [c_i32, c_i32, c_i32]),
    "insv2v_xattn_attn": (c_i32, [C.POINTER(XattnDesc), c_p]),
    "insv2v_xattn_attn_stream_elems": (c_i64, [c_i32, c_i32, c_i32]),
    "insv2v_groupnorm": (c_i32, [C.POINTER(GroupNormDesc), c_p]),
    "insv2v_layernorm": (c_i32, [C.POINTER(LayerNormDesc), c_p]),
    "insv2v_layernorm_stats": (c_i32, [c_p, c_p, c_i64, c_i32, c_i32, c_f32, c_p]),
    "insv2v_attention": (c_i32, [C.POINTER(AttentionDesc), c_p]),
    "insv2v_embed_tokens": (c_i32, [c_p, c_p, c_p, c_p, c_i32, c_i32, c_i32, c_i32, c_p]),
    "insv2v_softmax_rows": (c_i32, [c_p, c_p, c_i64, c_i64, c_i32, c_i32, c_f32, c_p]),
    "insv2v_softmax_rows_padded": (c_i32, [c_p, c_p, c_i64, c_i64, c_i32, c_i32, c_i32, c_f32, c_p]),
    "insv2v_timestep_embedding": (c_i32, [c_p, c_p, c_i32, c_i32, c_f32, c_p]),
    "insv2v_build_unet_input": (c_i32, [c_p, c_p, c_p, c_p, c_f32, c_i32, c_i32, c_i32, c_i32, c_i32, c_i64, c_i32, c_p]),
    "insv2v_cfg_step": (c_i32, [C.POINTER(StepDesc), c_p]),
    "insv2v_cfg_step_ms": (c_i32, [C.POINTER(MStepDesc), c_p]),
    "insv2v_cfg_step_mask": (c_i32, [C.POINTER(MaskStepDesc), c_p]),
    "insv2v_mask_to_latent": (c_i32, [c_p, c_p, c_i32, c_i32, c_i32, c_i32, c_p]),
    "insv2v_composite": (c_i32, [c_p, c_p, c_p, c_p, c_i32, c_i32, c_i32, c_p]),
    "insv2v_add_noise": (c_i32, [c_p, c_p, c_p, c_i64, c_f32, c_f32, c_p]),
    "insv2v_cfg_stats": (c_i32, [c_p, c_p, c_i32, c_i32, c_i32, c_f32, c_f32, c_i64, c_p]),
    "insv2v_warp_image": (c_i32, [c_p, c_p, c_p, c_i32, c_i32, c_i32, c_i32, c_p]),
    "insv2v_tap_gather": (c_i32, [c_p, c_i64, c_p, c_p, c_i64, c_i32, c_i32, c_i32, c_i32, c_p]),
    "insv2v_resize_flow": (c_i32, [c_p, c_p, c_i32, c_i32, c_i32, c_i32, c_i32, c_p]),
    "insv2v_flow_correction": (c_i32, [c_p, c_p, c_p, c_p, c_p, c_i32, c_i32, c_i32, c_i32, c_f32, c_f32, c_p]),
    "insv2v_nchw_to_nhwc_f16": (c_i32, [c_p, c_p, c_i32, c_i32, c_i32, c_i32, c_i32, c_f32, c_p]),
    "insv2v_nhwc_to_nchw_f32": (c_i32, [c_p, c_i32, c_p, c_i32, c_i32, c_i32, c_i32, c_i32, c_f32, c_p]),
    "insv2v_posterior_sample": (c_i32, [c_p, c_p, c_p, c_i32, c_i32, c_i32, c_i32, c_f32, c_p]),
    "insv2v_posterior_sample_seeded": (c_i32, [c_p, c_p, c_i32, c_i32, c_i32, c_i32, c_f32, c_i64, c_i64, c_i64, c_p]),
    "insv2v_randn": (c_i32, [c_p, c_i64, c_i64, c_i64, c_i64, c_i32, c_p]),
    "insv2v_im2col": (c_i32, [C.POINTER(Im2colDesc), c_p]),
    "insv2v_instance_norm": (c_i32, [c_p, c_p, c_p, c_i32, c_i32, c_i32, c_i64, c_i64, c_i32, c_f32, c_i32, c_p]),
    "insv2v_ew": (c_i32, [c_i32, c_p, c_p, c_p, c_p, c_i64, c_i32, c_i64, c_i64, c_i64, c_i64, c_p]),
    "insv2v_avgpool2x2": (c_i32, [c_p, c_p, c_i64, c_i32, c_i32, c_p]),
    "insv2v_corr_lookup": (c_i32, [C.POINTER(CorrLookupDesc), c_p]),
    "insv2v_raft_flow_rows": (c_i32, [c_p, c_p, c_i64, c_p, c_i64, c_i32, c_i32, c_i32, c_i32, c_p]),
    "insv2v_convex_upsample": (c_i32, [c_p, c_p, c_i64, c_p, c_i32, c_i32, c_i32, c_p]),
}

_lib = None


class HipKernelError(RuntimeError):
    pass


def load():
    global _lib
    if _lib is not None:
        return _lib
    if not os.path.exists(LIB_PATH):
        raise HipKernelError(
            f"{LIB_PATH} not found: build it with `python instruct-video-to-video_amd/build.py` "
            "(or __graft_entry__.build()). There is no CPU fallback for the insv2v hot path.")
    lib = C.CDLL(LIB_PATH)
    for name, (res, args) in SIGNATURES.items():
        fn = getattr(lib, name)
        fn.restype, fn.argtypes = res, args
    if lib.insv2v_abi_version() != ABI_VERSION:
        raise HipKernelError("libinsv2v_hip.so ABI version mismatch; rebuild the library")
    _lib = lib
    return lib


def check(status, what):
    if status != 0:
        kind = {-1: "invalid argument", -2: "unsupported configuration"}.get(status, f"hipError {status}")
        raise HipKernelError(f"{what}: {kind}")
```

Measured before the change: 16.60 frames/s.

## Split last-wave R8 GEMM tiles into smaller M sub-tiles to balance tail

```diff
diff --git a/include/insv2v_hip.h b/include/insv2v_hip.h
--- a/include/insv2v_hip.h
+++ b/include/insv2v_hip.h
@@ -93,6 +93,15 @@
     int32_t forced_tile;
 } insv2v_gemm_plan_t;
 int insv2v_gemm_plan(const insv2v_gemm_desc* d, int cus, insv2v_gemm_plan_t* out);
+typedef struct insv2v_gemm_tail_t {
+    int32_t bn;
+    int32_t grid;
+    int32_t full_tiles;
+    int32_t sub_h;
+    int32_t sub_tiles;
+} insv2v_gemm_tail_t;
+int insv2v_gemm_tail(const insv2v_gemm_desc* d, int cus, insv2v_gemm_tail_t* out);
+int insv2v_gemm_set_tail(int mode, int grid);
 
 typedef struct insv2v_winograd_in_desc {
     const void* x;
diff --git a/instruct-video-to-video_amd/csrc/gemm.hip b/instruct-video-to-video_amd/csrc/gemm.hip
--- a/instruct-video-to-video_amd/csrc/gemm.hip
+++ b/instruct-video-to-video_amd/csrc/gemm.hip
@@ -855,6 +855,8 @@
         s.r8 = env("INSV2V_GEMM_R8", s.r8); s.r8_stats = env("INSV2V_R8_STATS", s.r8_stats); s.q8_min_n = env("INSV2V_Q8_MIN_N", s.q8_min_n); s.persistent = env("INSV2V_GEMM_PERSISTENT", s.persistent);
         s.r8_geglu = env("INSV2V_R8_GEGLU", s.r8_geglu); s.r8_cim = env("INSV2V_R8_CIM", s.r8_cim); s.halo_legacy_map = env("INSV2V_HALO_LEGACY_MAP", s.halo_legacy_map);
         s.r8_dephase = env("INSV2V_R8_DEPHASE", s.r8_dephase); s.w4_wgs = env("INSV2V_W4_WGS", s.w4_wgs); s.w4_delay = env("INSV2V_W4_DELAY", s.w4_delay);
+        s.tail = env("INSV2V_GEMM_TAIL", s.tail);
+        if (s.tail != 0 && s.tail != 64 && s.tail != 128) s.tail = 1;
         return s;
     }();
     return sw;
@@ -869,12 +871,42 @@
 static int64_t operand_window() { return g_operand_window > 0 ? g_operand_window : ((int64_t)1 << 31) - ((int64_t)1 << 20); }
 int64_t insv2v_operand_window_override() { return g_operand_window; }
 
+static int g_tail_mode = 1, g_tail_grid = 0;
+extern "C" int insv2v_gemm_set_tail(int mode, int grid) {
+    const int prev = g_tail_mode | g_tail_grid << 8;
+    if (mode >= 0) g_tail_mode = (mode == 0 || mode == 64 || mode == 128) ? mode : 1;
+    if (grid >= 0) g_tail_grid = grid < (1 << 20) ? grid : 0;
+    return prev;
+}
+gemm_switches insv2v_gemm_tail_switches(int* grid) {
+    gemm_switches sw = insv2v_gemm_switches();
+    if (sw.tail) sw.tail = g_tail_mode;
+    if (grid) *grid = g_tail_grid;
+    return sw;
+}
+
 static insv2v_gemm_plan_t plan_here(const insv2v_gemm_desc& d, int cus = 0, bool queries_only = false) {
     return plan_gemm(d, cus > 0 ? cus : insv2v_num_cus(), operand_window(), insv2v_gemm_switches(), queries_only);
 }
 extern "C" int insv2v_gemm_plan(const insv2v_gemm_desc* dp, int cus, insv2v_gemm_plan_t* out) {
     if (!dp || !out) return INSV2V_EINVAL;
     *out = plan_here(*dp, cus);
+    return 0;
+}
+extern "C" int insv2v_gemm_tail(const insv2v_gemm_desc* dp, int cus, insv2v_gemm_tail_t* out) {
+    if (!dp || !out) return INSV2V_EINVAL;
+    *out = {};
+    insv2v_gemm_desc d = *dp;
+    gemm_defaults(d);
+    const insv2v_gemm_plan_t p = plan_here(d, cus);
+    if (p.rc || (p.family != INSV2V_PLAN_R8 && p.family != INSV2V_PLAN_Q8)) return 0;
+    if (p.parts > 1) d = window_part(d, 0, p.units_per_part);
+    int grid = 0;
+    const gemm_switches sw = insv2v_gemm_tail_switches(&grid);
+    if (grid <= 0) grid = cus > 0 ? cus : insv2v_num_cus();
+    const int bn = p.family == INSV2V_PLAN_R8 ? 320 : 256;
+    const tail_sched t = tail_of_launch(d, bn, grid, sw);
+    *out = {bn, grid, t.full_tiles, t.sub_h, t.sub_tiles};
     return 0;
 }
 extern "C" int insv2v_gemm_stats_parts(const insv2v_gemm_desc* dp) {
diff --git a/instruct-video-to-video_amd/csrc/gemm_plan.h b/instruct-video-to-video_amd/csrc/gemm_plan.h
--- a/instruct-video-to-video_amd/csrc/gemm_plan.h
+++ b/instruct-video-to-video_amd/csrc/gemm_plan.h
@@ -16,8 +16,10 @@
     int halo_legacy_map = 0;
     int r8_dephase = 0;
     int w4_wgs = 2, w4_delay = -1;
+    int tail = 1;
 };
 const gemm_switches& insv2v_gemm_switches();
+gemm_switches insv2v_gemm_tail_switches(int* grid);
 
 static inline void gemm_defaults(insv2v_gemm_desc& d) { if (d.batch <= 0) d.batch = 1; if (d.alpha == 0.f) d.alpha = 1.f; }
 static inline bool misaligned16(const void* p) { return ((uintptr_t)p & 15) != 0; }
@@ -84,6 +86,32 @@
     auto rounds = [&](int bn) { return (double)((tm * ((d.N + bn - 1) / bn) + cus - 1) / cus) * bn; };
     return {rounds(256) * 1.03, rounds(320)};
 }
+struct tail_sched { int32_t full_tiles, sub_h, sub_tiles; };
+constexpr double TAIL_T128 = 0.75, TAIL_T64 = 0.65;
+static inline double tail_cost(int r, int sub_h, int grid) {
+    const long subs = (long)r * (256 / sub_h);
+    return (double)((subs + grid - 1) / grid) * (sub_h == 256 ? 1.0 : sub_h == 128 ? TAIL_T128 : TAIL_T64);
+}
+static inline tail_sched tail_schedule(int M, int N, int bn, int grid, const gemm_switches& sw) {
+    const long tiles = (long)((M + 255) / 256) * ((N + bn - 1) / bn);
+    if (grid <= 0) return {(int32_t)tiles, 256, 0};
+    const int full = (int)(tiles / grid * grid), r = (int)(tiles - full);
+    int h = 256;
+    if (r > 0 && bn == 320 && sw.tail) {
+        if (sw.tail == 128 || sw.tail == 64) h = sw.tail;
+        else {
+            double best = tail_cost(r, 256, grid);
+            if (tail_cost(r, 128, grid) < best) { best = tail_cost(r, 128, grid); h = 128; }
+            if (TAIL_T64 < 1.0 && tail_cost(r, 64, grid) < best) h = 64;
+        }
+    }
+    return {full, h, r * (256 / h)};
+}
+static inline tail_sched tail_of_launch(const insv2v_gemm_desc& d, int bn, int grid, gemm_switches sw) {
+    if (d.stats_out && d.residual) sw.tail = 0;
+    return tail_schedule(d.M, d.N, bn, grid, sw);
+}
+
 static inline int pingpong_choice(const insv2v_gemm_desc& d, bool stats, int cus, const gemm_switches& sw) {
     if (!sw.r8 || d.act != INSV2V_ACT_NONE || d.batch > 1 || d.c_fp32 || d.M < 8192 || d.N < 256) return 0;
     if (stats && (!sw.r8_stats || d.mode != INSV2V_MODE_LINEAR || d.k_split || (d.N % 320))) return 0;
diff --git a/instruct-video-to-video_amd/csrc/gemm_q8.hip b/instruct-video-to-video_amd/csrc/gemm_q8.hip
--- a/instruct-video-to-video_amd/csrc/gemm_q8.hip
+++ b/instruct-video-to-video_amd/csrc/gemm_q8.hip
@@ -419,7 +419,10 @@
     const int num_cu = insv2v_num_cus();
     if (num_cu <= 0) return INSV2V_EINVAL;
     const int tiles = ((d.M + 255) / 256) * ((d.N + 255) / 256);
-    hipLaunchKernelGGL((gemm_q8_kernel<MODE, GEGLU, HAS_RES, DBG, VAR>), dim3(tiles < num_cu ? tiles : num_cu), dim3(512), LDS_B + (DBG == 4 ? STAMP_B : 0), s, d);
+    int grid = 0;
+    insv2v_gemm_tail_switches(&grid);
+    if (grid <= 0) grid = num_cu;
+    hipLaunchKernelGGL((gemm_q8_kernel<MODE, GEGLU, HAS_RES, DBG, VAR>), dim3(tiles < grid ? tiles : grid), dim3(512), LDS_B + (DBG == 4 ? STAMP_B : 0), s, d);
     return launch_status();
 }
 
diff --git a/instruct-video-to-video_amd/csrc/gemm_r8.hip b/instruct-video-to-video_amd/csrc/gemm_r8.hip
--- a/instruct-video-to-video_amd/csrc/gemm_r8.hip
+++ b/instruct-video-to-video_amd/csrc/gemm_r8.hip
@@ -31,8 +31,9 @@
 
 template <int I> using ic = std::integral_constant<int, I>;
 
-template <int MODE, bool HAS_RES, int DBG = 0, bool SPLIT = true, bool STATS = false, bool GEGLU = false, bool CIM = false>
-__global__ __launch_bounds__(512) void gemm_r8_kernel(insv2v_gemm_desc p, int dephase) {
+template <int MODE, bool HAS_RES, int DBG = 0, bool SPLIT = true, bool STATS = false, bool GEGLU = false, bool CIM = false, int TAIL = 0>
+__global__ __launch_bounds__(512) void gemm_r8_kernel(insv2v_gemm_desc p, int dephase, int full_tiles, int nvirt) {
+    constexpr int sub_sh = TAIL;
     extern __shared__ __attribute__((aligned(16))) char smem[];
     const int tid = threadIdx.x, lane = tid & 63;
     const int wid = __builtin_amdgcn_readfirstlane(tid >> 6);
@@ -56,13 +57,15 @@
         }
     }
     auto tile_origin = [&](int v, int& bm0, int& bn0) {
+        int slice = 0;
+        if (TAIL != 0 && v >= full_tiles) { const int j = v - full_tiles; slice = j & ((1 << sub_sh) - 1); v = full_tiles + (j >> sub_sh); }
         const int bid = xcd_remap(v, ntiles);
         constexpr int GROUP_M = 8;
         const int per_group = GROUP_M * tiles_n;
         const int gidx = bid / per_group, first_m = gidx * GROUP_M;
         const int gsz = min(GROUP_M, tiles_m - first_m), rin = bid - gidx * per_group;
         const int tn = rin / gsz, tm = first_m + rin - tn * gsz;
-        bm0 = tm * BM; bn0 = tn * BN;
+        bm0 = tm * BM + slice * (BM >> sub_sh); bn0 = tn * BN;
     };
 
     const srd_t rA = make_srd(p.a), rA2 = make_srd(p.a2 ? p.a2 : p.a), rW = make_srd(p.w);
@@ -78,19 +81,20 @@
     const int nk = p.K / BK;
     const int IHu = p.upsample ? p.OH : p.IH, IWu = p.upsample ? p.OW : p.IW;
     const int ups = p.upsample ? 1 : 0;
-    struct Cursor { int v, kt, k0, kh, kw, ci0, soffA, abm0; bool second; int tap, dpix; unsigned wbase; } cur = {(int)blockIdx.x, 0, 0, 0, 0, 0, 0, 0, false, 0, 0, 0u};
+    struct Cursor { int v, kt, k0, kh, kw, ci0, soffA, abm0; bool second; int tap, dpix; unsigned wbase; int rsh; } cur = {(int)blockIdx.x, 0, 0, 0, 0, 0, 0, 0, false, 0, 0, 0u, 0};
     if (CIM) cur.dpix = -p.IW - 1;
     auto refresh_aoff = [&]() {
         const int ld = (int)((SPLIT && cur.second) ? p.lda2 : p.lda);
+        const bool dead = TAIL != 0 && prow >= (64 >> cur.rsh);
         if (LIN) {
-            aoff[0] = ((unsigned)(cur.abm0 + prow) * (unsigned)ld + (unsigned)chunk8) * 2u;
-            amax = ((unsigned)(p.M - 1) * (unsigned)ld + (unsigned)chunk8) * 2u;
+            aoff[0] = dead ? OOB_OFFSET : ((unsigned)(cur.abm0 + prow) * (unsigned)ld + (unsigned)chunk8) * 2u;
+            amax = dead ? OOB_OFFSET : ((unsigned)(p.M - 1) * (unsigned)ld + (unsigned)chunk8) * 2u;
         } else {
             const float rOW = 1.0f / (float)p.OW, rOH = 1.0f / (float)p.OH;
 #pragma unroll
             for (int r = 0; r < 4; ++r) {
-                const int m = cur.abm0 + (r >> 1) * 128 + (r & 1) * 64 + prow;
-                const bool okm = m < p.M;
+                const int m = cur.abm0 + ((r * 64) >> cur.rsh) + prow;
+                const bool okm = m < p.M && !dead;
                 const int mm = okm ? m : 0;
                 int t = (int)((float)mm * rOW);
                 int ow = mm - t * p.OW;
@@ -115,10 +119,11 @@
     };
     auto set_stage_rows = [&](int v) {
         int bm0 = 0, bn0 = 0;
-        const bool live = v < ntiles;
+        const bool live = v < (TAIL != 0 ? nvirt : ntiles);
         if (live) tile_origin(v, bm0, bn0);
         else { bm0 = p.M + BM; bn0 = p.N + BN; }
         cur.abm0 = bm0;
+        if (TAIL != 0) cur.rsh = (live && v >= full_tiles) ? sub_sh : 0;
         cur.wbase = (LIN && live && p.w_group_rows > 0) ? (unsigned)((int64_t)(bm0 / p.w_group_rows) * p.w_group_stride * 2) : 0u;
         const int c32 = (wid & 3) * 8 + (lane >> 3);
         const int pc = ((c32 >> 2) & 3) * 8 + (c32 >> 4) * 4 + (c32 & 3);
@@ -161,7 +166,7 @@
         char* dst = smem + (H * 2 + BUF) * AH_B + i * 8192 + wid * 1024;
         if (LIN) {
             const int ld = (int)((SPLIT && cur.second) ? p.lda2 : p.lda);
-            dma16((SPLIT && cur.second) ? rA2 : rA, min(aoff[0] + (unsigned)((H * 128 + i * 64) * ld * 2), amax), cur.soffA, dst);
+            dma16((SPLIT && cur.second) ? rA2 : rA, min(aoff[0] + (unsigned)(((H * 128 + i * 64) >> cur.rsh) * ld * 2), amax), cur.soffA, dst);
         } else if (CIM) {
             constexpr int R = H * 2;
             const unsigned ld2 = (unsigned)((SPLIT && cur.second) ? p.lda2 : p.lda) * 2u;
@@ -223,10 +228,10 @@
 #pragma unroll
                 for (int cb = 0; cb < 2; ++cb) acc[i][tb][cb] = floatx4{0.f, 0.f, 0.f, 0.f};
     };
-    auto read_a = [&](auto buf_c) {
-        constexpr int B = decltype(buf_c)::value;
-#pragma unroll
-        for (int tb = 0; tb < 4; ++tb)
+    auto read_a = [&](auto buf_c, auto ntb_c) __attribute__((always_inline)) {
+        constexpr int B = decltype(buf_c)::value, NTB = decltype(ntb_c)::value;
+#pragma unroll
+        for (int tb = 0; tb < NTB; ++tb)
 #pragma unroll
             for (int kb = 0; kb < 2; ++kb) fa[tb][kb] = *(const half8*)(aRd[kb] + B * AH_B + tb * 16 * 128);
     };
@@ -247,8 +252,8 @@
         }
     };
     unsigned dbg_seg[5] = {0, 0, 0, 0, 0}, dbg_gap[5] = {0, 0, 0, 0, 0}, dbg_last = 0, dbg_n = 0;
-    auto mma = [&](auto pb_c, auto&& mid) {
-        constexpr int PB = decltype(pb_c)::value;
+    auto mma = [&](auto pb_c, auto ntb_c, auto&& mid) __attribute__((always_inline)) {
+        constexpr int PB = decltype(pb_c)::value, NTB = decltype(ntb_c)::value;
         unsigned long long tb_ = 0;
         if (DBG == 5) {
             asm volatile("s_memtime %0\n\ts_waitcnt lgkmcnt(0)" : "=s"(tb_)::"memory");
@@ -262,18 +267,18 @@
 #pragma unroll
         for (int kb = 0; kb < 2; ++kb)
 #pragma unroll
-            for (int tb = 0; tb < 4; ++tb)
+            for (int tb = 0; tb < NTB; ++tb)
 #pragma unroll
                 for (int cb = 0; cb < 2; ++cb) {
                     acc[PB][tb][cb] = __builtin_amdgcn_mfma_f32_16x16x32_f16(fw[cb][kb], fa[tb][kb], acc[PB][tb][cb], 0, 0, 0);
 #if !R8_MID_SPREAD
-                    if (kb * 8 + tb * 2 + cb == 3) { SB(); mid(0); SB(); }
-                    if (kb * 8 + tb * 2 + cb == 9) { SB(); mid(1); SB(); }
+                    if ((kb * NTB + tb) * 2 + cb == NTB - 1) { SB(); mid(0); SB(); }
+                    if ((kb * NTB + tb) * 2 + cb == NTB * 2 + 1) { SB(); mid(1); SB(); }
 #endif
                 }
 #if R8_MID_SPREAD
 #pragma unroll
-        for (int i = 0; i < 16; ++i) {
+        for (int i = 0; i < 4 * NTB; ++i) {
             __builtin_amdgcn_sched_group_barrier(0x008, 1, 0);
             __builtin_amdgcn_sched_group_barrier(0x002, 2, 0);
             __builtin_amdgcn_sched_group_barrier(0x004, 1, 0);
@@ -306,13 +311,14 @@
         asm volatile("ds_read_b64 %0, %4\n\tds_read_b64 %1, %4 offset:128\n\tds_read_b64 %2, %4 offset:256\n\tds_read_b64 %3, %4 offset:384\n\t"
                      "s_waitcnt lgkmcnt(0)" : "=&v"(s0), "=&v"(s1), "=&v"(s2), "=&v"(s3) : "v"(a) : "memory");
     };
-    auto epilogue = [&](int bm0, int bn0, int pb) {
+    auto epilogue = [&](int bm0, int bn0, int pb, auto ntb_c) __attribute__((always_inline)) {
+        constexpr int NTB = decltype(ntb_c)::value, WROWS = NTB * 16;
         if (DBG == 2 || DBG == 5) {
             float s = 0.f;
 #pragma unroll
             for (int i = 0; i < 5; ++i)
 #pragma unroll
-                for (int tb = 0; tb < 4; ++tb)
+                for (int tb = 0; tb < NTB; ++tb)
 #pragma unroll
                     for (int cb = 0; cb < 2; ++cb)
 #pragma unroll
@@ -329,11 +335,11 @@
         unsigned offc[4], offr[4];
         {
             float2 st[4];
-            if (LIN) stat4(park + PK_ST + (wm * 64 + e15) * 8, st[0], st[1], st[2], st[3]);
+            if (LIN) stat4(park + PK_ST + (wm * WROWS + e15) * 8, st[0], st[1], st[2], st[3]);
             else { ra[0] = p.alpha; rm[0] = 0.f; }
 #pragma unroll
-            for (int tb = 0; tb < 4; ++tb) {
-                const int m = bm0 + wm * 64 + tb * 16 + e15;
+            for (int tb = 0; tb < NTB; ++tb) {
+                const int m = bm0 + wm * WROWS + tb * 16 + e15;
                 if (LIN) {
                     const float mean = ln ? st[tb].x : 0.f, rstd = ln ? st[tb].y : 1.f;
                     ra[tb] = rstd * p.alpha; rm[tb] = -rstd * mean;
@@ -357,7 +363,7 @@
                 const int on = (bn0 >> 1) + t * 16;
                 const bool okc = on + eg * 4 + 4 <= (p.N >> 1);
 #pragma unroll
-                for (int tb = 0; tb < 4; ++tb) {
+                for (int tb = 0; tb < NTB; ++tb) {
                     float v[4];
 #pragma unroll
                     for (int e = 0; e < 4; ++e) {
@@ -378,7 +384,7 @@
             const int on = bn0 + wn * 160 + PBK * 32;
             const bool okc = on + eg * 8 + 8 <= p.N;
 #pragma unroll
-            for (int tb = 0; tb < 4; ++tb) rv[SLOT][tb] = __builtin_amdgcn_raw_buffer_load_b128(rR, okc ? offr[tb] : OOB_OFFSET, on * 2, 0);
+            for (int tb = 0; tb < NTB; ++tb) rv[SLOT][tb] = __builtin_amdgcn_raw_buffer_load_b128(rR, okc ? offr[tb] : OOB_OFFSET, on * 2, 0);
         };
         if (HAS_RES) {
             load_res(ic<0>{}, ic<0>{}); load_res(ic<1>{}, ic<1>{});
@@ -403,7 +409,7 @@
             const int on = bn0 + wn * 160 + pbk * 32;
             const bool okc = on + eg * 8 + 8 <= p.N;
 #pragma unroll
-            for (int tb = 0; tb < 4; ++tb) {
+            for (int tb = 0; tb < NTB; ++tb) {
                 float v[8];
 #pragma unroll
                 for (int h = 0; h < 2; ++h)
@@ -433,8 +439,8 @@
         if (STATS) {
             const int part = bn0 / 160 + wn;
 #pragma unroll
-            for (int tb = 0; tb < 4; ++tb) {
-                const int m = bm0 + wm * 64 + tb * 16 + e15;
+            for (int tb = 0; tb < NTB; ++tb) {
+                const int m = bm0 + wm * WROWS + tb * 16 + e15;
                 float s1 = st1[tb] + __shfl_xor(st1[tb], 16, 64), s2 = st2[tb] + __shfl_xor(st2[tb], 16, 64);
                 s1 += __shfl_xor(s1, 32, 64); s2 += __shfl_xor(s2, 32, 64);
                 if (eg == 0 && m < p.M) *(float2*)(p.stats_out + ((int64_t)part * p.M + m) * 2) = make_float2(s1, s2);
@@ -457,59 +463,65 @@
     BARRIER();
     zero_acc();
 
-    auto tile_step = [&](auto buf_c, bool first, int nbm0, int nbn0, int npb) {
+    auto tile_step = [&](auto buf_c, auto ntb_c, bool first, int nbm0, int nbn0, int npb) __attribute__((always_inline)) {
         constexpr int B = decltype(buf_c)::value;
+        constexpr ic<decltype(ntb_c)::value> NT{};
         read_w(ic<B>{}, ic<0>{});
         SB();
-        read_a(ic<B>{});
+        read_a(ic<B>{}, NT);
         SB();
         if (first) stage_park(npb, nbm0, nbn0);
         BARRIER();
-        mma(ic<0>{}, [&](int i) { if (i == 0) stage_w(ic<2>{}, ic<B ^ 1>{}); else stage_w(ic<3>{}, ic<B ^ 1>{}); });
+        mma(ic<0>{}, NT, [&](int i) { if (i == 0) stage_w(ic<2>{}, ic<B ^ 1>{}); else stage_w(ic<3>{}, ic<B ^ 1>{}); });
         BARRIER();
         read_w(ic<B>{}, ic<1>{});
         BARRIER();
-        mma(ic<1>{}, [&](int i) { if (i == 0) stage_w(ic<4>{}, ic<B ^ 1>{}); });
+        mma(ic<1>{}, NT, [&](int i) { if (i == 0) stage_w(ic<4>{}, ic<B ^ 1>{}); });
         BARRIER();
         read_w(ic<B>{}, ic<2>{});
         advance();
         BARRIER();
-        mma(ic<2>{}, [&](int i) { stage_a(ic<0>{}, ic<B>{}, i); });
+        mma(ic<2>{}, NT, [&](int i) { stage_a(ic<0>{}, ic<B>{}, i); });
         BARRIER();
         read_w(ic<B>{}, ic<3>{});
         BARRIER();
-        mma(ic<3>{}, [&](int i) { stage_a(ic<1>{}, ic<B>{}, i); });
+        mma(ic<3>{}, NT, [&](int i) { stage_a(ic<1>{}, ic<B>{}, i); });
         BARRIER();
         read_w(ic<B>{}, ic<4>{});
         wait_vmcnt<4>();
         BARRIER();
-        mma(ic<4>{}, [&](int i) { if (i == 0) stage_w(ic<0>{}, ic<B>{}); else stage_w(ic<1>{}, ic<B>{}); });
+        mma(ic<4>{}, NT, [&](int i) { if (i == 0) stage_w(ic<0>{}, ic<B>{}); else stage_w(ic<1>{}, ic<B>{}); });
         BARRIER();
     };
     int par = 0;
     unsigned long long cyc_loop = 0, cyc_join = 0, cyc_epi = 0, ntl = 0, ts0 = 0, ts1 = 0, ts2 = 0, ts3 = 0;
     auto stamp = [&](unsigned long long& t) { if (DBG == 4) asm volatile("s_memtime %0\n\ts_waitcnt lgkmcnt(0)" : "=s"(t)::"memory"); };
-    for (; cv < ntiles; cv += G) {
+    auto run_tile = [&](auto ntb_c) __attribute__((always_inline)) {
+        constexpr ic<decltype(ntb_c)::value> NT{};
         tile_origin(cv, cbm0, cbn0);
         stamp(ts0);
         if (grp == 1) BARRIER();
         bool first = cv != (int)blockIdx.x;
         int t = 0;
-        if (par) { tile_step(ic<1>{}, first, cbm0, cbn0, cpb); first = false; t = 1; par = 0; }
+        if (par) { tile_step(ic<1>{}, NT, first, cbm0, cbn0, cpb); first = false; t = 1; par = 0; }
         for (; t + 1 < nk; t += 2) {
-            tile_step(ic<0>{}, first, cbm0, cbn0, cpb);
+            tile_step(ic<0>{}, NT, first, cbm0, cbn0, cpb);
             first = false;
-            tile_step(ic<1>{}, false, cbm0, cbn0, cpb);
-        }
-        if (t < nk) { tile_step(ic<0>{}, first, cbm0, cbn0, cpb); par = 1; }
+            tile_step(ic<1>{}, NT, false, cbm0, cbn0, cpb);
+        }
+        if (t < nk) { tile_step(ic<0>{}, NT, first, cbm0, cbn0, cpb); par = 1; }
         stamp(ts1);
         if (grp == 0) BARRIER();
         stamp(ts2);
-        epilogue(cbm0, cbn0, cpb);
+        epilogue(cbm0, cbn0, cpb, NT);
         stamp(ts3);
         if (DBG == 4) { cyc_loop += ts1 - ts0; cyc_join += ts2 - ts1; cyc_epi += ts3 - ts2; ++ntl; }
         zero_acc();
         cpb ^= 1;
+    };
+    for (; cv < (TAIL != 0 ? full_tiles : ntiles); cv += G) run_tile(ic<4>{});
+    if constexpr (TAIL > 0) {
+        for (; cv < nvirt; cv += G) run_tile(ic<(4 >> TAIL)>{});
     }
     if (DBG == 5 && p.workspace && blockIdx.x < 64 && lane == 0) {
         unsigned* o = (unsigned*)p.workspace + ((int)blockIdx.x * 8 + wid) * 12;
@@ -523,16 +535,30 @@
     }
 }
 
+template <int MODE, bool HAS_RES, int DBG, bool SPLIT, bool STATS, bool GEGLU, bool CIM, int TAIL>
+int launch_r8_tail(const insv2v_gemm_desc& d, int grid, const tail_sched& t, hipStream_t s) {
+    static bool attr_set = false;
+    if (const int e = set_dynamic_lds(attr_set, (const void*)gemm_r8_kernel<MODE, HAS_RES, DBG, SPLIT, STATS, GEGLU, CIM, TAIL>, LDS_B)) return e;
+    const int dephase = insv2v_gemm_switches().r8_dephase;
+    const int nvirt = t.full_tiles + t.sub_tiles;
+    hipLaunchKernelGGL((gemm_r8_kernel<MODE, HAS_RES, DBG, SPLIT, STATS, GEGLU, CIM, TAIL>), dim3(nvirt < grid ? nvirt : grid), dim3(512), LDS_B, s, d, dephase,
+                       TAIL ? t.full_tiles : nvirt, nvirt);
+    return launch_status();
+}
 template <int MODE, bool HAS_RES, int DBG = 0, bool SPLIT = true, bool STATS = false, bool GEGLU = false, bool CIM = false>
 int launch_r8(const insv2v_gemm_desc& d, hipStream_t s) {
-    static bool attr_set = false;
-    if (const int e = set_dynamic_lds(attr_set, (const void*)gemm_r8_kernel<MODE, HAS_RES, DBG, SPLIT, STATS, GEGLU, CIM>, LDS_B)) return e;
     const int num_cu = insv2v_num_cus();
     if (num_cu <= 0) return INSV2V_EINVAL;
-    const int tiles = ((d.M + BM - 1) / BM) * ((d.N + BN - 1) / BN);
-    const int dephase = insv2v_gemm_switches().r8_dephase;
-    hipLaunchKernelGGL((gemm_r8_kernel<MODE, HAS_RES, DBG, SPLIT, STATS, GEGLU, CIM>), dim3(tiles < num_cu ? tiles : num_cu), dim3(512), LDS_B, s, d, dephase);
-    return launch_status();
+    int grid = 0;
+    gemm_switches sw = insv2v_gemm_tail_switches(&grid);
+    if (grid <= 0) grid = num_cu;
+    if (DBG != 0) sw.tail = 0;
+    const tail_sched t = tail_of_launch(d, BN, grid, sw);
+    if constexpr (DBG == 0 && !(STATS && HAS_RES)) {
+        if (t.sub_h == 128) return launch_r8_tail<MODE, HAS_RES, DBG, SPLIT, STATS, GEGLU, CIM, 1>(d, grid, t, s);
+        if (t.sub_h == 64) return launch_r8_tail<MODE, HAS_RES, DBG, SPLIT, STATS, GEGLU, CIM, 2>(d, grid, t, s);
+    }
+    return launch_r8_tail<MODE, HAS_RES, DBG, SPLIT, STATS, GEGLU, CIM, 0>(d, grid, t, s);
 }
 
 }
diff --git a/instruct-video-to-video_amd/insv2v/_lib.py b/instruct-video-to-video_amd/insv2v/_lib.py
--- a/instruct-video-to-video_amd/insv2v/_lib.py
+++ b/instruct-video-to-video_amd/insv2v/_lib.py
@@ -31,6 +31,10 @@
                                      "gn_fuse", "parts", "units_per_part", "forced_tile")]
 
 
+class GemmTail(C.Structure):
+    _fields_ = [(n, c_i32) for n in ("bn", "grid", "full_tiles", "sub_h", "sub_tiles")]
+
+
 class WinogradInDesc(C.Structure):
     _fields_ = [("x", c_p), ("x2", c_p), ("gn_ab", c_p), ("v", c_p), ("ldx", c_i64), ("ldx2", c_i64), ("v_group_rows", c_i64),
                 ("NB", c_i32), ("H", c_i32), ("W", c_i32), ("C", c_i32), ("C1", c_i32), ("gn_images_per_sample", c_i32), ("gn_silu", c_i32), ("upsample", c_i32)]
@@ -120,6 +124,8 @@
     "insv2v_gemm": (c_i32, [C.POINTER(GemmDesc), c_p]),
     "insv2v_gemm_stats_parts": (c_i32, [C.POINTER(GemmDesc)]),
     "insv2v_gemm_plan": (c_i32, [C.POINTER(GemmDesc), c_i32, C.POINTER(GemmPlan)]),
+    "insv2v_gemm_tail": (c_i32, [C.POINTER(GemmDesc), c_i32, C.POINTER(GemmTail)]),
+    "insv2v_gemm_set_tail": (c_i32, [c_i32, c_i32]),
     "insv2v_set_operand_window": (c_i64, [c_i64]),
     "insv2v_conv3x3_fuses_groupnorm": (c_i32, [C.POINTER(GemmDesc)]),
     "insv2v_winograd_input": (c_i32, [C.POINTER(WinogradInDesc), c_p]),
```

After: 16.62 frames/s (median of 6 runs). About the same (+0.1%).
